# hongsukchoi/Pose2Mesh_RELEASE

Hardware: NVIDIA H100
Metric: SMPL meshes/sec (higher is better)
Workload: dtype f32 (wgmma fp16x3 split, fp32 accumulate)

## Files before the change

### include/p2m_b200.h

```cpp
#ifndef P2M_B200_H_
#define P2M_B200_H_

#include <stddef.h>
#include <stdint.h>

#ifdef __cplusplus
extern "C" {
#endif

typedef struct p2m_model p2m_model_t;
typedef void* p2m_stream_t;

enum p2m_status {
  P2M_OK = 0,
  P2M_ERR_INVALID = 1,
  P2M_ERR_CUDA = 2,
  P2M_ERR_WORKSPACE = 3,
  P2M_ERR_NOGPU = 4
};

enum p2m_precision {
  P2M_PREC_FP32_SIMT = 0,
  P2M_PREC_FP16X3_TC = 1
};

typedef struct {
  int32_t n_levels;
  const int32_t* level_size;
  const int32_t* const* rowptr;
  const int32_t* const* colidx;
  const float* const* values;
  int32_t n_blocks;
  const int32_t* block_len;
  const int32_t* block_chans;
  int32_t device;
} p2m_model_desc_t;

typedef struct {
  float* fc_w;
  float* fc_b;
  float* const* cl_w;
  float* const* cl_b;
  float* const* bn_w;
  float* const* bn_b;
  float* const* bn_rm;
  float* const* bn_rv;
  int64_t* const* bn_nbt;
} p2m_params_t;

int p2m_model_create(const p2m_model_desc_t* desc, p2m_model_t** out);
void p2m_model_destroy(p2m_model_t* m);
int p2m_model_num_layers(const p2m_model_t* m);
int p2m_model_layer_info(const p2m_model_t* m, int layer, int32_t out[6]);
int p2m_model_set_precision(p2m_model_t* m, int precision);
int p2m_model_set_profiling(p2m_model_t* m, int enable);
int p2m_model_layer_times_ms(p2m_model_t* m, float* out_ms, int n);
int p2m_debug_kernel_status(p2m_model_t* m, int32_t* out);
int p2m_debug_set_trace(p2m_model_t* m, void* dev_buf);
int p2m_debug_set_fuse_head(p2m_model_t* m, int enable);
int p2m_debug_set_elide_padding(p2m_model_t* m, int enable);
int p2m_debug_set_dedup_padding(p2m_model_t* m, int enable);
int p2m_debug_conv_path(const p2m_model_t* m, int level, int fin, int fout, int32_t out[9]);
int p2m_debug_conv_tiling(const p2m_model_t* m, int level, int fin, int fout, int32_t out[3]);
int p2m_debug_layer_route(const p2m_model_t* m, int layer, int batch, int need_dx, int32_t out[9]);

typedef struct {
  float* const* z;
  float* const* a;
  float* const* y;
  float* fc_out;
  float* const* g_a;
  float* const* g_z;
  float* const* dx;
  float* fc_dx;
} p2m_capture_t;
int p2m_debug_set_capture(p2m_model_t* m, const p2m_capture_t* capture);

#define P2M_BN_BATCH_UPDATE 0
#define P2M_BN_BATCH 1
#define P2M_BN_RUNNING 2
typedef struct {
  int32_t stats;
  int32_t cumulative;
  double momentum;
  double eps;
} p2m_bn_opts_t;

size_t p2m_meshnet_workspace_bytes(const p2m_model_t* m, int batch, int training);
size_t p2m_meshnet_backward_scratch_bytes(const p2m_model_t* m, int batch);

int p2m_meshnet_forward(p2m_model_t* m, const p2m_params_t* params, const float* x, float* y, int batch,
                        int training, void* workspace, size_t workspace_bytes, p2m_stream_t stream);

int p2m_model_set_output_gather(p2m_model_t* m, const int32_t* vertex_of_slot, int n_slots);
int p2m_meshnet_forward_vertices(p2m_model_t* m, const p2m_params_t* params, const float* x, float* y_vertices,
                                 int batch, void* workspace, size_t workspace_bytes, p2m_stream_t stream);

int p2m_meshnet_backward(p2m_model_t* m, const p2m_params_t* params, const p2m_params_t* grads, const float* x,
                         const float* dy, float* dx, int batch, void* workspace, size_t workspace_bytes,
                         void* scratch, size_t scratch_bytes, p2m_stream_t stream);

size_t p2m_meshnet_workspace_bytes_opts(const p2m_model_t* m, int batch, int training, const p2m_bn_opts_t* bn);
int p2m_meshnet_forward_opts(p2m_model_t* m, const p2m_params_t* params, const p2m_bn_opts_t* bn, const float* x,
                             float* y, int batch, int training, void* workspace, size_t workspace_bytes,
                             p2m_stream_t stream);
int p2m_meshnet_backward_opts(p2m_model_t* m, const p2m_params_t* params, const p2m_params_t* grads,
                              const p2m_bn_opts_t* bn, const float* x, const float* dy, float* dx, int batch,
                              void* workspace, size_t workspace_bytes, void* scratch, size_t scratch_bytes,
                              p2m_stream_t stream);

size_t p2m_meshnet_host_io_bytes(const p2m_model_t* m, int batch);
int p2m_meshnet_forward_host(p2m_model_t* m, const p2m_params_t* params, const float* x_host, float* y_host,
                             int batch, void* workspace, size_t workspace_bytes, p2m_stream_t stream);
int p2m_meshnet_forward_vertices_host(p2m_model_t* m, const p2m_params_t* params, const float* x_host,
                                      float* y_vertices_host, int batch, void* workspace, size_t workspace_bytes,
                                      p2m_stream_t stream);

typedef struct {
  int32_t level, batch, fin, fout;
  const float* x;
  const float* weight;
  const float* bias;
  int32_t bn_mode;
  const float* bn_weight;
  const float* bn_bias;
  float* bn_running_mean;
  float* bn_running_var;
  int64_t* bn_num_batches_tracked;
  float* save_mean;
  float* save_invstd;
  int32_t relu;
  float* y;
} p2m_conv_fwd_args_t;

size_t p2m_cheb_conv_workspace_bytes(const p2m_model_t* m, int level, int batch, int fin, int fout);
int p2m_cheb_conv_fwd(p2m_model_t* m, const p2m_conv_fwd_args_t* a, void* workspace, size_t workspace_bytes,
                      p2m_stream_t stream);

typedef struct {
  int32_t level, batch, fin, fout;
  const float* x;
  const float* weight;
  const float* dz;
  float* dx;
  float* dweight;
  float* dbias;
} p2m_conv_bwd_args_t;
int p2m_cheb_conv_bwd(p2m_model_t* m, const p2m_conv_bwd_args_t* a, void* workspace, size_t workspace_bytes,
                      p2m_stream_t stream);


typedef struct {
  const float* w1_w; const float* w1_b;
  const float* w2_w; const float* w2_b;
  const float* bn1_w; const float* bn1_b; const float* bn1_rm; const float* bn1_rv;
  const float* bn2_w; const float* bn2_b; const float* bn2_rm; const float* bn2_rv;
} p2m_posenet_stage_t;
typedef struct {
  int32_t num_joint, hidden, num_stage;
  const float* w1_w; const float* w1_b;
  const float* w2_w; const float* w2_b;
  const p2m_posenet_stage_t* stages;
} p2m_posenet_params_t;
size_t p2m_posenet_workspace_bytes(int batch, int hidden);
int p2m_posenet_forward(const p2m_posenet_params_t* params, const float* pose2d, float* pose3d, float* pose_combine,
                        int batch, void* workspace, size_t workspace_bytes, p2m_stream_t stream);

typedef struct {
  int64_t* bn1_nbt; int64_t* bn2_nbt;
} p2m_posenet_train_stage_t;
typedef struct {
  const p2m_posenet_train_stage_t* stages;
} p2m_posenet_train_t;
typedef struct {
  float* w1_w; float* w1_b; float* w2_w; float* w2_b;
  float* bn1_w; float* bn1_b; float* bn2_w; float* bn2_b;
} p2m_posenet_stage_grads_t;
typedef struct {
  float* w1_w; float* w1_b; float* w2_w; float* w2_b;
  const p2m_posenet_stage_grads_t* stages;
} p2m_posenet_grads_t;
size_t p2m_posenet_train_workspace_bytes(int batch, int num_joint, int hidden, int num_stage);
size_t p2m_posenet_train_saved_bytes(int batch, int num_joint, int hidden, int num_stage);
int p2m_posenet_train_forward(const p2m_posenet_params_t* params, const p2m_posenet_train_t* extra, const float* pose2d,
                              int batch, float p_dropout, const int64_t* seed, float* pose3d, float* pose_combine,
                              void* saved, size_t saved_bytes, void* workspace, size_t workspace_bytes,
                              p2m_stream_t stream);
int p2m_posenet_backward(const p2m_posenet_params_t* params, const float* pose2d, int batch, float p_dropout,
                         const int64_t* seed, const void* saved, size_t saved_bytes, const float* d_pose3d,
                         const p2m_posenet_grads_t* grads, float* d_pose2d, void* workspace, size_t workspace_bytes,
                         p2m_stream_t stream);

int p2m_posenet_forward_opts(const p2m_posenet_params_t* params, const p2m_bn_opts_t* bn, const float* pose2d,
                             float* pose3d, float* pose_combine, int batch, void* workspace, size_t workspace_bytes,
                             p2m_stream_t stream);
int p2m_posenet_train_forward_opts(const p2m_posenet_params_t* params, const p2m_posenet_train_t* extra,
                                   const p2m_bn_opts_t* bn, const float* p_dropout, const float* pose2d, int batch,
                                   const int64_t* seed, float* pose3d, float* pose_combine, void* saved,
                                   size_t saved_bytes, void* workspace, size_t workspace_bytes, p2m_stream_t stream);
int p2m_posenet_backward_opts(const p2m_posenet_params_t* params, const p2m_bn_opts_t* bn, const float* p_dropout,
                              const float* pose2d, int batch, const int64_t* seed, const void* saved,
                              size_t saved_bytes, const float* d_pose3d, const p2m_posenet_grads_t* grads,
                              float* d_pose2d, void* workspace, size_t workspace_bytes, p2m_stream_t stream);

typedef struct {
  float* const* g_y;
  float* const* a2;
  float* const* g_a2;
  float* const* g_z2;
  float* const* a1;
  float* const* g_a1;
  float* const* g_bn1;
  float* const* scale;
  float* g_y0;
} p2m_posenet_capture_t;
int p2m_debug_posenet_backward_capture(const p2m_posenet_params_t* params, const p2m_bn_opts_t* bn,
// ... 212 lines not shown
```

### pose2mesh_release_b200/_lib.py

```python
from __future__ import annotations

import ctypes as C
import os
import threading

import torch

_HERE = os.path.dirname(os.path.abspath(__file__))
LIB_PATH = os.path.join(_HERE, "libp2m_b200.so")

P2M_PREC_FP32_SIMT = 0
P2M_PREC_FP16X3_TC = 1
PRECISIONS = {"fp32": P2M_PREC_FP32_SIMT, "fp16x3": P2M_PREC_FP16X3_TC}


def default_precision() -> int:
    name = os.environ.get("P2M_PRECISION", "fp16x3").strip().lower()
    if name not in PRECISIONS:
        raise RuntimeError(f"P2M_PRECISION={name!r}: expected one of {sorted(PRECISIONS)}")
    return PRECISIONS[name]

c_float_p = C.POINTER(C.c_float)
c_int32_p = C.POINTER(C.c_int32)
c_int64_p = C.POINTER(C.c_int64)
# ... 14 lines not shown


class Params(C.Structure):
    _fields_ = [
        ("fc_w", C.c_void_p),
        ("fc_b", C.c_void_p),
        ("cl_w", C.POINTER(C.c_void_p)),
        ("cl_b", C.POINTER(C.c_void_p)),
        ("bn_w", C.POINTER(C.c_void_p)),
        ("bn_b", C.POINTER(C.c_void_p)),
        ("bn_rm", C.POINTER(C.c_void_p)),
        ("bn_rv", C.POINTER(C.c_void_p)),
        ("bn_nbt", C.POINTER(C.c_void_p)),
    ]


P2M_BN_BATCH_UPDATE = 0
P2M_BN_BATCH = 1
P2M_BN_RUNNING = 2


class BnOpts(C.Structure):
    _fields_ = [("stats", C.c_int32), ("cumulative", C.c_int32), ("momentum", C.c_double), ("eps", C.c_double)]


class ConvFwdArgs(C.Structure):
    _fields_ = [
        ("level", C.c_int32), ("batch", C.c_int32), ("fin", C.c_int32), ("fout", C.c_int32),
        ("x", C.c_void_p), ("weight", C.c_void_p), ("bias", C.c_void_p),
        ("bn_mode", C.c_int32),
        ("bn_weight", C.c_void_p), ("bn_bias", C.c_void_p),
        ("bn_running_mean", C.c_void_p), ("bn_running_var", C.c_void_p),
        ("bn_num_batches_tracked", C.c_void_p),
        ("save_mean", C.c_void_p), ("save_invstd", C.c_void_p),
        ("relu", C.c_int32),
        ("y", C.c_void_p),
    ]


class ConvBwdArgs(C.Structure):
    _fields_ = [
        ("level", C.c_int32), ("batch", C.c_int32), ("fin", C.c_int32), ("fout", C.c_int32),
        ("x", C.c_void_p), ("weight", C.c_void_p), ("dz", C.c_void_p),
        ("dx", C.c_void_p), ("dweight", C.c_void_p), ("dbias", C.c_void_p),
    ]


class Capture(C.Structure):
    _fields_ = [
        ("z", C.POINTER(C.c_void_p)), ("a", C.POINTER(C.c_void_p)), ("y", C.POINTER(C.c_void_p)),
        ("fc_out", C.c_void_p),
        ("g_a", C.POINTER(C.c_void_p)), ("g_z", C.POINTER(C.c_void_p)), ("dx", C.POINTER(C.c_void_p)),
        ("fc_dx", C.c_void_p),
    ]


class Pose2MeshLossArgs(C.Structure):
    _fields_ = [(n, C.c_int32) for n in ("batch", "n_padded", "n_vertex", "n_face", "n_reg_joint", "n_lift_joint")] + [
        (n, C.c_void_p) for n in ("cam_mesh", "lift_pose", "gt_mesh", "gt_reg3dpose", "gt_lift3dpose", "mesh_valid",
                                  "reg3dpose_valid", "lift3dpose_valid", "faces", "joint_regressor", "perm_reverse",
                                  "weights", "edge", "pred_pose", "scratch", "loss", "terms", "grad_loss",
                                  "d_cam_mesh", "d_lift_pose")]


P2M_POSE2MESH_MAX_REG_JOINT = 24


class PoseNetStage(C.Structure):
    _fields_ = [(n, C.c_void_p) for n in ("w1_w", "w1_b", "w2_w", "w2_b", "bn1_w", "bn1_b", "bn1_rm", "bn1_rv",
                                          "bn2_w", "bn2_b", "bn2_rm", "bn2_rv")]


class PoseNetParams(C.Structure):
    _fields_ = [("num_joint", C.c_int32), ("hidden", C.c_int32), ("num_stage", C.c_int32),
                ("w1_w", C.c_void_p), ("w1_b", C.c_void_p), ("w2_w", C.c_void_p), ("w2_b", C.c_void_p),
                ("stages", C.POINTER(PoseNetStage))]


class PoseNetTrainStage(C.Structure):
    _fields_ = [("bn1_nbt", C.c_void_p), ("bn2_nbt", C.c_void_p)]


class PoseNetTrain(C.Structure):
    _fields_ = [("stages", C.POINTER(PoseNetTrainStage))]


class PoseNetStageGrads(C.Structure):
    _fields_ = [(n, C.c_void_p) for n in ("w1_w", "w1_b", "w2_w", "w2_b", "bn1_w", "bn1_b", "bn2_w", "bn2_b")]


class PoseNetGrads(C.Structure):
    _fields_ = [("w1_w", C.c_void_p), ("w1_b", C.c_void_p), ("w2_w", C.c_void_p), ("w2_b", C.c_void_p),
                ("stages", C.POINTER(PoseNetStageGrads))]


class PoseNetCapture(C.Structure):
    _fields_ = [(n, C.POINTER(C.c_void_p)) for n in ("g_y", "a2", "g_a2", "g_z2", "a1", "g_a1", "g_bn1", "scale")] + [
        ("g_y0", C.c_void_p)]


class BodyModelDesc(C.Structure):
    _fields_ = [
        ("n_vertex", C.c_int32), ("n_joint", C.c_int32), ("n_betas", C.c_int32), ("n_out_joints", C.c_int32),
        ("v_template", c_float_p), ("shapedirs", c_float_p), ("posedirs", c_float_p), ("J_regressor", c_float_p),
        ("weights", c_float_p), ("parents", c_int32_p), ("model_betas", c_float_p), ("pose_mean", c_float_p),
        ("joint_map", c_int32_p), ("scale", C.c_float), ("device", C.c_int32),
    ]


P2M_BETAS_ZERO_MEANS_MODEL = 0
P2M_BETAS_AS_GIVEN = 1

P2M_FRAME_ROTATE_ROOT = 1
P2M_FRAME_CLAMP_BETAS = 2
P2M_FRAME_ZERO_BETAS_MODEL = 4
P2M_FRAME_LAYER_TRANS_T = 8
P2M_FRAME_LAYER_TRANS = 16
P2M_FRAME_H36M_COMPENSATE = 32
P2M_FRAME_ADD_T = 64
P2M_FRAME_TO_MM = 128

P2M_JOINTS_HUMAN36 = 0
P2M_JOINTS_COCO = 1
P2M_JOINTS_SMPL = 2
P2M_JOINTS_MANO = 3
P2M_DATASET_HUMAN36M = 0
P2M_DATASET_COCO = 1
P2M_DATASET_MUCO = 2
P2M_DATASET_AMASS = 3
P2M_DATASET_PW3D = 4
P2M_DATASET_SURREAL = 5
P2M_DATASET_FREIHAND = 6

P2M_CAM_INPUT_F64 = 0
P2M_CAM_INPUT_INT = 1
P2M_CAM_INPUT_F32 = 2

P2M_DTYPE_F32 = 0
P2M_DTYPE_F64 = 1

P2M_NOISE_NONE = 0
P2M_NOISE_COCO = 1
P2M_NOISE_H36M = 2
P2M_AREA_TIGHT = 0
P2M_AREA_CROP = 1


class H36MError(C.Structure):
    _fields_ = [("mean", C.c_double * 2), ("std", C.c_double * 2), ("weight", C.c_double)]


EXPORTS = [
    "p2m_model_create", "p2m_model_destroy", "p2m_model_num_layers", "p2m_model_layer_info",
    "p2m_model_set_precision", "p2m_debug_kernel_status", "p2m_debug_set_trace", "p2m_debug_set_fuse_head", "p2m_debug_set_elide_padding", "p2m_debug_set_dedup_padding", "p2m_debug_conv_path", "p2m_debug_conv_tiling", "p2m_debug_layer_route", "p2m_debug_set_capture", "p2m_model_set_profiling", "p2m_model_layer_times_ms", "p2m_meshnet_workspace_bytes", "p2m_meshnet_backward_scratch_bytes",
    "p2m_meshnet_forward", "p2m_meshnet_backward", "p2m_meshnet_workspace_bytes_opts", "p2m_meshnet_forward_opts",
    "p2m_meshnet_backward_opts", "p2m_model_set_output_gather", "p2m_meshnet_forward_vertices", "p2m_meshnet_host_io_bytes", "p2m_meshnet_forward_host", "p2m_meshnet_forward_vertices_host",
    "p2m_cheb_conv_workspace_bytes", "p2m_cheb_conv_fwd", "p2m_cheb_conv_bwd", "p2m_graph_match_level", "p2m_posenet_workspace_bytes", "p2m_posenet_forward",
    "p2m_posenet_train_workspace_bytes", "p2m_posenet_train_saved_bytes", "p2m_posenet_train_forward", "p2m_posenet_backward",
    "p2m_posenet_forward_opts", "p2m_posenet_train_forward_opts", "p2m_posenet_backward_opts",
    "p2m_debug_posenet_backward_capture",
    "p2m_regress_joints", "p2m_regress_joints_backward", "p2m_normalize_pose2d", "p2m_mesh_losses", "p2m_coord_loss",
    "p2m_pose2mesh_loss", "p2m_pose2mesh_loss_backward",
    "p2m_rigid_align", "p2m_point_errors", "p2m_fit_camera", "p2m_crop_cam_to_orig",
    "p2m_one_euro_smooth", "p2m_accel_error", "p2m_segment_mean",
    "p2m_nearest_distances", "p2m_align_w_scale", "p2m_pck_accumulate",
    "p2m_render_workspace_bytes", "p2m_render_meshes",
    "p2m_body_model_create", "p2m_body_model_destroy", "p2m_body_model_workspace_bytes", "p2m_body_model_forward",
    "p2m_body_model_backward_workspace_bytes", "p2m_body_model_backward",
    "p2m_camera_frame_workspace_bytes", "p2m_camera_frame_coords", "p2m_h36m_regressors_create",
    "p2m_h36m_regressors_destroy", "p2m_h36m_targets", "p2m_synthesize_pose", "p2m_h36m_syn_error",
    "p2m_training_pose2d", "p2m_augm_params", "p2m_training_pose2d_augmented", "p2m_sample_targets",
    "p2m_layer_joint_targets",
    "p2m_last_error", "p2m_version", "p2m_launch_count", "p2m_launch_count_reset",
]

_lib = None
_lock = threading.Lock()


def load() -> C.CDLL:
    global _lib
    if _lib is not None:
        return _lib
    with _lock:
        if _lib is not None:
            return _lib
        if not os.path.exists(LIB_PATH):
            raise RuntimeError(
                f"{LIB_PATH} not found: build it with `python -m pose2mesh_release_b200.build` "
                "(or __graft_entry__.build()).  pose2mesh_release_b200 has no CPU / eager fallback.")
        lib = C.CDLL(LIB_PATH)
        vp, i32, i64, sz = C.c_void_p, C.c_int32, C.c_int64, C.c_size_t
        lib.p2m_model_create.argtypes = [C.POINTER(ModelDesc), C.POINTER(vp)]
        lib.p2m_model_create.restype = C.c_int
        lib.p2m_model_destroy.argtypes = [vp]
        lib.p2m_model_destroy.restype = None
        lib.p2m_model_num_layers.argtypes = [vp]
        lib.p2m_model_num_layers.restype = C.c_int
        lib.p2m_model_layer_info.argtypes = [vp, C.c_int, c_int32_p]
        lib.p2m_model_layer_info.restype = C.c_int
        lib.p2m_model_set_precision.argtypes = [vp, C.c_int]
        lib.p2m_model_set_precision.restype = C.c_int
        lib.p2m_model_set_profiling.argtypes = [vp, C.c_int]
        lib.p2m_model_set_profiling.restype = C.c_int
        lib.p2m_model_layer_times_ms.argtypes = [vp, c_float_p, C.c_int]
        lib.p2m_model_layer_times_ms.restype = C.c_int
        lib.p2m_debug_set_fuse_head.argtypes = [vp, C.c_int]
        lib.p2m_debug_set_fuse_head.restype = C.c_int
        lib.p2m_debug_set_elide_padding.argtypes = [vp, C.c_int]
        lib.p2m_debug_set_elide_padding.restype = C.c_int
        lib.p2m_debug_set_dedup_padding.argtypes = [vp, C.c_int]
        lib.p2m_debug_set_dedup_padding.restype = C.c_int
        lib.p2m_debug_set_trace.argtypes = [vp, vp]
        lib.p2m_debug_set_trace.restype = C.c_int
        lib.p2m_debug_conv_path.argtypes = [vp, C.c_int, C.c_int, C.c_int, c_int32_p]
        lib.p2m_debug_conv_path.restype = C.c_int
        lib.p2m_debug_conv_tiling.argtypes = [vp, C.c_int, C.c_int, C.c_int, c_int32_p]
        lib.p2m_debug_conv_tiling.restype = C.c_int
        lib.p2m_debug_layer_route.argtypes = [vp, C.c_int, C.c_int, C.c_int, c_int32_p]
        lib.p2m_debug_layer_route.restype = C.c_int
        lib.p2m_debug_set_capture.argtypes = [vp, C.POINTER(Capture)]
        lib.p2m_debug_set_capture.restype = C.c_int
        lib.p2m_debug_kernel_status.argtypes = [vp, c_int32_p]
        lib.p2m_debug_kernel_status.restype = C.c_int
        lib.p2m_meshnet_workspace_bytes.argtypes = [vp, C.c_int, C.c_int]
        lib.p2m_meshnet_workspace_bytes.restype = sz
        lib.p2m_meshnet_backward_scratch_bytes.argtypes = [vp, C.c_int]
        lib.p2m_meshnet_backward_scratch_bytes.restype = sz
        lib.p2m_meshnet_host_io_bytes.argtypes = [vp, C.c_int]
        lib.p2m_meshnet_host_io_bytes.restype = sz
        lib.p2m_meshnet_forward.argtypes = [vp, C.POINTER(Params), vp, vp, C.c_int, C.c_int, vp, sz, vp]
        lib.p2m_meshnet_forward.restype = C.c_int
        lib.p2m_model_set_output_gather.argtypes = [vp, c_int32_p, C.c_int]
        lib.p2m_model_set_output_gather.restype = C.c_int
        lib.p2m_meshnet_forward_vertices.argtypes = [vp, C.POINTER(Params), vp, vp, C.c_int, vp, sz, vp]
        lib.p2m_meshnet_forward_vertices.restype = C.c_int
        lib.p2m_meshnet_forward_host.argtypes = [vp, C.POINTER(Params), vp, vp, C.c_int, vp, sz, vp]
        lib.p2m_meshnet_forward_host.restype = C.c_int
        lib.p2m_meshnet_forward_vertices_host.argtypes = [vp, C.POINTER(Params), vp, vp, C.c_int, vp, sz, vp]
        lib.p2m_meshnet_forward_vertices_host.restype = C.c_int
        lib.p2m_meshnet_backward.argtypes = [vp, C.POINTER(Params), C.POINTER(Params), vp, vp, vp, C.c_int, vp, sz,
                                             vp, sz, vp]
        lib.p2m_meshnet_backward.restype = C.c_int
        bn_p = C.POINTER(BnOpts)
        lib.p2m_meshnet_workspace_bytes_opts.argtypes = [vp, C.c_int, C.c_int, bn_p]
        lib.p2m_meshnet_workspace_bytes_opts.restype = sz
        lib.p2m_meshnet_forward_opts.argtypes = [vp, C.POINTER(Params), bn_p, vp, vp, C.c_int, C.c_int, vp, sz, vp]
        lib.p2m_meshnet_forward_opts.restype = C.c_int
        lib.p2m_meshnet_backward_opts.argtypes = [vp, C.POINTER(Params), C.POINTER(Params), bn_p, vp, vp, vp, C.c_int,
                                                  vp, sz, vp, sz, vp]
        lib.p2m_meshnet_backward_opts.restype = C.c_int
        lib.p2m_cheb_conv_workspace_bytes.argtypes = [vp, C.c_int, C.c_int, C.c_int, C.c_int]
        lib.p2m_cheb_conv_workspace_bytes.restype = sz
        lib.p2m_cheb_conv_fwd.argtypes = [vp, C.POINTER(ConvFwdArgs), vp, sz, vp]
        lib.p2m_cheb_conv_fwd.restype = C.c_int
        lib.p2m_cheb_conv_bwd.argtypes = [vp, C.POINTER(ConvBwdArgs), vp, sz, vp]
        lib.p2m_cheb_conv_bwd.restype = C.c_int
        lib.p2m_posenet_workspace_bytes.argtypes = [C.c_int, C.c_int]
        lib.p2m_posenet_workspace_bytes.restype = sz
        lib.p2m_posenet_forward.argtypes = [C.POINTER(PoseNetParams), vp, vp, vp, C.c_int, vp, sz, vp]
        lib.p2m_posenet_forward.restype = C.c_int
        for fn in (lib.p2m_posenet_train_workspace_bytes, lib.p2m_posenet_train_saved_bytes):
            fn.argtypes = [C.c_int] * 4
            fn.restype = sz
        lib.p2m_posenet_train_forward.argtypes = [C.POINTER(PoseNetParams), C.POINTER(PoseNetTrain), vp, C.c_int,
                                                  C.c_float, vp, vp, vp, vp, sz, vp, sz, vp]
        lib.p2m_posenet_train_forward.restype = C.c_int
        lib.p2m_posenet_backward.argtypes = [C.POINTER(PoseNetParams), vp, C.c_int, C.c_float, vp, vp, sz, vp,
                                             C.POINTER(PoseNetGrads), vp, vp, sz, vp]
        lib.p2m_posenet_backward.restype = C.c_int
        lib.p2m_posenet_forward_opts.argtypes = [C.POINTER(PoseNetParams), bn_p, vp, vp, vp, C.c_int, vp, sz, vp]
        lib.p2m_posenet_forward_opts.restype = C.c_int
        lib.p2m_posenet_train_forward_opts.argtypes = [C.POINTER(PoseNetParams), C.POINTER(PoseNetTrain), bn_p,
                                                       c_float_p, vp, C.c_int, vp, vp, vp, vp, sz, vp, sz, vp]
        lib.p2m_posenet_train_forward_opts.restype = C.c_int
        lib.p2m_posenet_backward_opts.argtypes = [C.POINTER(PoseNetParams), bn_p, c_float_p, vp, C.c_int, vp, vp, sz,
                                                  vp, C.POINTER(PoseNetGrads), vp, vp, sz, vp]
        lib.p2m_posenet_backward_opts.restype = C.c_int
        lib.p2m_debug_posenet_backward_capture.argtypes = (lib.p2m_posenet_backward_opts.argtypes[:-1]
                                                           + [C.POINTER(PoseNetCapture), vp])
        lib.p2m_debug_posenet_backward_capture.restype = C.c_int
        lib.p2m_regress_joints.argtypes = [vp, vp, vp, C.c_int, C.c_int, C.c_int, C.c_int, vp]
        lib.p2m_regress_joints.restype = C.c_int
        lib.p2m_regress_joints_backward.argtypes = [vp, vp, vp, C.c_int, C.c_int, C.c_int, C.c_int, vp]
        lib.p2m_regress_joints_backward.restype = C.c_int
        lib.p2m_normalize_pose2d.argtypes = [vp, vp, C.c_int, C.c_int, C.c_int, C.c_int, C.c_int, vp]
        lib.p2m_normalize_pose2d.restype = C.c_int
        lib.p2m_mesh_losses.argtypes = [vp, vp, vp, C.c_int, C.c_int, C.c_int, vp, vp, vp, vp]
        lib.p2m_mesh_losses.restype = C.c_int
        lib.p2m_coord_loss.argtypes = [vp, vp, vp, i64, vp, vp, vp, vp]
        lib.p2m_coord_loss.restype = C.c_int
        for fn in (lib.p2m_pose2mesh_loss, lib.p2m_pose2mesh_loss_backward):
            fn.argtypes = [C.POINTER(Pose2MeshLossArgs), vp]
            fn.restype = C.c_int
        lib.p2m_rigid_align.argtypes = [vp, vp, C.c_int, C.c_int, c_int32_p, C.c_int, vp, vp, vp, vp, vp]
        lib.p2m_rigid_align.restype = C.c_int
        lib.p2m_point_errors.argtypes = [vp, vp, vp, vp, C.c_int, C.c_int, c_int32_p, C.c_int, C.c_int, vp, vp, vp]
        lib.p2m_point_errors.restype = C.c_int
        lib.p2m_fit_camera.argtypes = [vp, C.c_int, C.c_int, C.c_int, vp, C.c_int, vp, C.c_int, C.c_int, C.c_int,
                                       c_int32_p, C.POINTER(C.c_double), C.c_int, vp, vp, vp, vp, vp, vp, vp]
        lib.p2m_fit_camera.restype = C.c_int
        lib.p2m_crop_cam_to_orig.argtypes = [vp, vp, vp, C.c_int, vp, vp]
        lib.p2m_crop_cam_to_orig.restype = C.c_int
        lib.p2m_one_euro_smooth.argtypes = [C.c_int, vp, vp, i64, c_int64_p, C.c_int, i64, C.c_double, C.c_double,
                                            C.c_double, vp]
        lib.p2m_one_euro_smooth.restype = C.c_int
        lib.p2m_accel_error.argtypes = [C.c_int, vp, vp, C.c_int, c_int64_p, C.c_int, i64, vp, vp, vp, vp, vp]
        lib.p2m_accel_error.restype = C.c_int
        lib.p2m_segment_mean.argtypes = [C.c_int, vp, i64, c_int64_p, C.c_int, i64, vp, vp, vp]
        lib.p2m_segment_mean.restype = C.c_int
        c_double_p = C.POINTER(C.c_double)
        lib.p2m_nearest_distances.argtypes = [C.c_int, vp, vp, C.c_int, C.c_int, C.c_int, c_double_p, C.c_int, vp, vp,
                                              vp, vp, vp, vp]
        lib.p2m_nearest_distances.restype = C.c_int
        lib.p2m_align_w_scale.argtypes = [vp, vp, C.c_int, C.c_int, C.c_int, vp, vp, vp]
        lib.p2m_align_w_scale.restype = C.c_int
        lib.p2m_pck_accumulate.argtypes = [vp, vp, vp, i64, c_double_p, C.c_int, vp, vp, vp]
        lib.p2m_pck_accumulate.restype = C.c_int
        lib.p2m_render_workspace_bytes.argtypes = [C.c_int, C.c_int, C.c_int]
        lib.p2m_render_workspace_bytes.restype = sz
        lib.p2m_render_meshes.argtypes = [vp, C.c_int, C.c_int, vp, C.c_int, vp, vp, vp, vp, C.c_int, C.c_int, C.c_int,
                                          vp, vp, vp, vp, vp, sz, vp]
        lib.p2m_render_meshes.restype = C.c_int
        lib.p2m_body_model_create.argtypes = [C.POINTER(BodyModelDesc), C.POINTER(vp)]
        lib.p2m_body_model_create.restype = C.c_int
        lib.p2m_body_model_destroy.argtypes = [vp]
        lib.p2m_body_model_destroy.restype = None
        lib.p2m_body_model_workspace_bytes.argtypes = [vp, C.c_int]
        lib.p2m_body_model_workspace_bytes.restype = sz
        lib.p2m_body_model_forward.argtypes = [vp, vp, vp, C.c_int, vp, C.c_int, vp, vp, C.c_int, vp, sz, vp]
        lib.p2m_body_model_forward.restype = C.c_int
        lib.p2m_body_model_backward_workspace_bytes.argtypes = [vp, C.c_int]
        lib.p2m_body_model_backward_workspace_bytes.restype = sz
        lib.p2m_body_model_backward.argtypes = [vp, vp, vp, C.c_int, vp, C.c_int, vp, vp, vp, vp, vp, C.c_int, vp, sz,
                                                vp]
        lib.p2m_body_model_backward.restype = C.c_int
        lib.p2m_camera_frame_workspace_bytes.argtypes = [vp, C.c_int]
        lib.p2m_camera_frame_workspace_bytes.restype = sz
        lib.p2m_camera_frame_coords.argtypes = [vp, C.c_int, vp, vp, vp, vp, vp, c_int32_p, C.c_int, vp, vp, C.c_int,
                                                vp, sz, vp]
        lib.p2m_camera_frame_coords.restype = C.c_int
        lib.p2m_h36m_regressors_create.argtypes = [C.POINTER(C.c_double), C.POINTER(C.c_double), C.c_int, C.c_int,
                                                   C.POINTER(vp)]
        lib.p2m_h36m_regressors_create.restype = C.c_int
        lib.p2m_h36m_regressors_destroy.argtypes = [vp]
        lib.p2m_h36m_regressors_destroy.restype = None
        lib.p2m_h36m_targets.argtypes = [vp, C.c_int, C.c_float, vp, vp, vp, vp, C.c_int, vp, vp, vp, vp, vp, vp, vp,
                                         vp, vp]
        lib.p2m_h36m_targets.restype = C.c_int
        lib.p2m_synthesize_pose.argtypes = [vp, vp, vp, C.c_int, vp, vp]
        lib.p2m_synthesize_pose.restype = C.c_int
        lib.p2m_h36m_syn_error.argtypes = [C.POINTER(H36MError), vp, C.c_int, vp, vp]
        lib.p2m_h36m_syn_error.restype = C.c_int
        lib.p2m_training_pose2d.argtypes = [vp, C.c_int, C.c_int, vp, C.c_int, C.c_int, C.c_int, C.POINTER(H36MError),
                                            vp, C.c_int, C.c_int, vp, vp]
        lib.p2m_training_pose2d.restype = C.c_int
        lib.p2m_augm_params.argtypes = [C.c_int, C.c_int, C.c_double, vp, vp, vp, vp]
        lib.p2m_augm_params.restype = C.c_int
        lib.p2m_training_pose2d_augmented.argtypes = [vp, C.c_int, C.c_int, vp, C.c_int, C.c_int, C.c_int,
                                                      C.POINTER(H36MError), vp, C.c_int, C.c_int, vp, vp, C.c_int,
                                                      C.c_int, vp, vp]
        lib.p2m_training_pose2d_augmented.restype = C.c_int
        lib.p2m_sample_targets.argtypes = [vp, C.c_int, C.c_int, C.c_float, vp, vp, vp, vp, vp, C.c_int, vp, vp, vp,
                                           vp, vp, C.c_int, vp, vp, vp, vp, vp, vp, vp, vp, vp, vp]
        lib.p2m_sample_targets.restype = C.c_int
        lib.p2m_layer_joint_targets.argtypes = [C.c_int, vp, vp, C.c_int, C.c_int, vp, vp, vp, vp, C.c_int, vp, vp,
                                                vp, vp, vp, vp, vp, vp, vp, vp]
        lib.p2m_layer_joint_targets.restype = C.c_int
        lib.p2m_graph_match_level.argtypes = [i64, c_int32_p, c_int32_p, C.POINTER(C.c_double), c_int64_p,
                                              C.POINTER(C.c_double), c_int32_p]
        lib.p2m_graph_match_level.restype = i32
# ... 50 lines not shown
```

### pose2mesh_release_b200/csrc/cheb_umma.cu

```cuda
#include <cuda.h>
#include <cuda_fp16.h>
#include <cuda_runtime.h>

#include <algorithm>
#include <climits>
#include <cstring>
#include <vector>

#include "p2m_internal.h"

namespace p2m {

namespace {

constexpr int TILE_M = 128;
constexpr int FC = 32;
constexpr int A_BLOCK_BYTES = TILE_M * 128;
constexpr float W_SCALE = 64.f;
constexpr float W_INV_SCALE = 1.f / 64.f;

struct TileHeader {
  int n_rows;
  int h1;
  int nnz;
// ... 176 lines not shown
  if (e < e1) {
    const uint2 a0 = lds_u2(ent + e * 8);
    fma4(acc0, __uint_as_float(a0.y), lds_f4(rows_q + a0.x));
  }
  return make_float4(acc0.x + acc1.x, acc0.y + acc1.y, acc0.z + acc1.z, acc0.w + acc1.w);
}

__device__ __forceinline__ void wg_fence() { asm volatile("wgmma.fence.sync.aligned;" ::: "memory"); }
__device__ __forceinline__ void wg_commit() { asm volatile("wgmma.commit_group.sync.aligned;" ::: "memory"); }
__device__ __forceinline__ void wg_wait0() { asm volatile("wgmma.wait_group.sync.aligned 0;" ::: "memory"); }
__device__ __forceinline__ void wgmma_m64n64(float (&d)[32], uint64_t desc_a, uint64_t desc_b) {
  asm volatile(
      "{\n\t.reg .pred p;\n\tsetp.ne.b32 p, 1, 0;\n\t"
      "wgmma.mma_async.sync.aligned.m64n64k16.f32.f16.f16 "
      "{%0, %1, %2, %3, %4, %5, %6, %7, %8, %9, %10, %11, %12, %13, %14, %15, "
      "%16, %17, %18, %19, %20, %21, %22, %23, %24, %25, %26, %27, %28, %29, %30, %31}, %32, %33, p, 1, 1, 0, 0;\n\t}"
      : "+f"(d[0]), "+f"(d[1]), "+f"(d[2]), "+f"(d[3]), "+f"(d[4]), "+f"(d[5]), "+f"(d[6]), "+f"(d[7]), "+f"(d[8]),
        "+f"(d[9]), "+f"(d[10]), "+f"(d[11]), "+f"(d[12]), "+f"(d[13]), "+f"(d[14]), "+f"(d[15]), "+f"(d[16]),
        "+f"(d[17]), "+f"(d[18]), "+f"(d[19]), "+f"(d[20]), "+f"(d[21]), "+f"(d[22]), "+f"(d[23]), "+f"(d[24]),
        "+f"(d[25]), "+f"(d[26]), "+f"(d[27]), "+f"(d[28]), "+f"(d[29]), "+f"(d[30]), "+f"(d[31])
      : "l"(desc_a), "l"(desc_b)
      : "memory");
}
__device__ __forceinline__ void wgmma_m64n128(float (&d)[2][32], uint64_t desc_a, uint64_t desc_b) {
  asm volatile(
      "{\n\t.reg .pred p;\n\tsetp.ne.b32 p, 1, 0;\n\t"
      "wgmma.mma_async.sync.aligned.m64n128k16.f32.f16.f16 "
      "{%0, %1, %2, %3, %4, %5, %6, %7, %8, %9, %10, %11, %12, %13, %14, %15, "
      "%16, %17, %18, %19, %20, %21, %22, %23, %24, %25, %26, %27, %28, %29, %30, %31, "
      "%32, %33, %34, %35, %36, %37, %38, %39, %40, %41, %42, %43, %44, %45, %46, %47, "
      "%48, %49, %50, %51, %52, %53, %54, %55, %56, %57, %58, %59, %60, %61, %62, %63}, %64, %65, p, 1, 1, 0, 0;\n\t}"
      : "+f"(d[0][0]), "+f"(d[0][1]), "+f"(d[0][2]), "+f"(d[0][3]), "+f"(d[0][4]), "+f"(d[0][5]), "+f"(d[0][6]),
        "+f"(d[0][7]), "+f"(d[0][8]), "+f"(d[0][9]), "+f"(d[0][10]), "+f"(d[0][11]), "+f"(d[0][12]), "+f"(d[0][13]),
        "+f"(d[0][14]), "+f"(d[0][15]), "+f"(d[0][16]), "+f"(d[0][17]), "+f"(d[0][18]), "+f"(d[0][19]), "+f"(d[0][20]),
        "+f"(d[0][21]), "+f"(d[0][22]), "+f"(d[0][23]), "+f"(d[0][24]), "+f"(d[0][25]), "+f"(d[0][26]), "+f"(d[0][27]),
        "+f"(d[0][28]), "+f"(d[0][29]), "+f"(d[0][30]), "+f"(d[0][31]), "+f"(d[1][0]), "+f"(d[1][1]), "+f"(d[1][2]),
        "+f"(d[1][3]), "+f"(d[1][4]), "+f"(d[1][5]), "+f"(d[1][6]), "+f"(d[1][7]), "+f"(d[1][8]), "+f"(d[1][9]),
        "+f"(d[1][10]), "+f"(d[1][11]), "+f"(d[1][12]), "+f"(d[1][13]), "+f"(d[1][14]), "+f"(d[1][15]), "+f"(d[1][16]),
        "+f"(d[1][17]), "+f"(d[1][18]), "+f"(d[1][19]), "+f"(d[1][20]), "+f"(d[1][21]), "+f"(d[1][22]), "+f"(d[1][23]),
        "+f"(d[1][24]), "+f"(d[1][25]), "+f"(d[1][26]), "+f"(d[1][27]), "+f"(d[1][28]), "+f"(d[1][29]), "+f"(d[1][30]),
        "+f"(d[1][31])
      : "l"(desc_a), "l"(desc_b)
      : "memory");
}
__device__ __forceinline__ void wgmma_m64n32(float (&d)[16], uint64_t desc_a, uint64_t desc_b) {
  asm volatile(
      "{\n\t.reg .pred p;\n\tsetp.ne.b32 p, 1, 0;\n\t"
      "wgmma.mma_async.sync.aligned.m64n32k16.f32.f16.f16 "
      "{%0, %1, %2, %3, %4, %5, %6, %7, %8, %9, %10, %11, %12, %13, %14, %15}, %16, %17, p, 1, 1, 1, 1;\n\t}"
      : "+f"(d[0]), "+f"(d[1]), "+f"(d[2]), "+f"(d[3]), "+f"(d[4]), "+f"(d[5]), "+f"(d[6]), "+f"(d[7]), "+f"(d[8]),
        "+f"(d[9]), "+f"(d[10]), "+f"(d[11]), "+f"(d[12]), "+f"(d[13]), "+f"(d[14]), "+f"(d[15])
      : "l"(desc_a), "l"(desc_b)
      : "memory");
}

__device__ __forceinline__ uint64_t make_desc_sw128(uint32_t saddr) {
  uint64_t d = 0;
  d |= (uint64_t)((saddr & 0x3FFFF) >> 4);
  d |= (uint64_t)1 << 16;
  d |= (uint64_t)(1024 >> 4) << 32;
  d |= (uint64_t)1 << 62;
  return d;
}

__host__ __device__ __forceinline__ uint32_t sw128_off(int row, int chunk) {
  return (uint32_t)row * 128u + (uint32_t)((chunk ^ (row & 7)) << 4);
}

struct Half4 {
  __half2 a, b;
};
__device__ __forceinline__ void split4(const float4& v, uint2& hi, uint2& lo) {
  __half2 h0 = __floats2half2_rn(v.x, v.y), h1 = __floats2half2_rn(v.z, v.w);
  float2 f0 = __half22float2(h0), f1 = __half22float2(h1);
  __half2 l0 = __floats2half2_rn(v.x - f0.x, v.y - f0.y), l1 = __floats2half2_rn(v.z - f1.x, v.w - f1.y);
  hi.x = *reinterpret_cast<uint32_t*>(&h0);
  hi.y = *reinterpret_cast<uint32_t*>(&h1);
  lo.x = *reinterpret_cast<uint32_t*>(&l0);
  lo.y = *reinterpret_cast<uint32_t*>(&l1);
}

struct KParams {
  const float* x;
  int in_unpool;
  int V, P, fin;
  int n_tiles;
  const unsigned char* meta;
  const int* meta_bytes;
  int meta_stride, max_h1;
  const unsigned char* wpack;
  const float* zero_row;
  EpiDev ep;
  int res_identity;
  const float* t1;
  const float* a_scale;
  const float* b_scale;
  long long ldy;
  int y_col0;
  float* y;
  int* status;
  long long* trace;
  int own_table;
  const float* head_wt;
  float* head_z;
  const unsigned char* apack;
  long long wslice_bytes;
  long long wblock_stride;
  int tma;
  CUtensorMap tm_x, tm_t1;
};

#ifdef P2M_UMMA_TRACE
__device__ __forceinline__ void trace_ev(const KParams& p, int role, int& n, int ev) {
  if (p.trace != nullptr && blockIdx.x == 0 && blockIdx.y == 0 && n < 512) {
    p.trace[role * 512 + n] = ((long long)ev << 48) | (clock64() & 0xFFFFFFFFFFFFll);
    ++n;
  }
}
#else
__device__ __forceinline__ void trace_ev(const KParams&, int, int&, int) {}
#endif

constexpr int W_PROD = 16;
constexpr int W_XLOAD = 16, N_XLOAD = 2, W_BLOAD = 18, W_EPI0 = 20;
constexpr int NUM_THREADS2 = 24 * 32;
constexpr int REGS_LAUNCH = 80, REGS_UTIL = 40, REGS_EPI = 120;
static_assert(128 * (REGS_EPI - REGS_LAUNCH) <= 128 * (REGS_LAUNCH - REGS_UTIL), "register pool balance");
static_assert(W_XLOAD % 4 == 0 && W_EPI0 % 4 == 0 && W_EPI0 - W_XLOAD == 4, "setmaxnreg works on aligned warpgroups");
constexpr int W_PROD_W = 8, W_EPI1_W = 8, W_XLOAD_W = 12, W_BLOAD_W = 14, W_EPI0_W = 16;
constexpr int NUM_THREADS_W = 20 * 32;
constexpr int REGS_LAUNCH_W = 96, REGS_UTIL_W = 40, REGS_PROD_W = 88, REGS_EPI_W = 128;
static_assert(2 * 128 * (REGS_EPI_W - REGS_LAUNCH_W) <=
                  128 * (REGS_LAUNCH_W - REGS_UTIL_W) + 2 * 128 * (REGS_LAUNCH_W - REGS_PROD_W),
              "register pool balance of the 64 x 128 layout");
static_assert(REGS_LAUNCH_W * NUM_THREADS_W <= 65536 && (REGS_LAUNCH_W + 8) * NUM_THREADS_W > 65536,
              "__launch_bounds__(NUM_THREADS_W, 1) gives REGS_LAUNCH_W registers per thread");
static_assert(W_EPI1_W == W_PROD_W && W_EPI1_W % 4 == 0 && W_XLOAD_W == W_EPI1_W + 4 && W_EPI0_W == W_XLOAD_W + 4 &&
                  (W_EPI0_W + 4) * 32 == NUM_THREADS_W,
              "setmaxnreg works on aligned warpgroups");
template <int N>
struct ConvRoles {
  static constexpr int threads = NUM_THREADS2, prod = W_PROD, xload = W_XLOAD, bload = W_BLOAD, epi0 = W_EPI0,
                       epi1 = -1;
  static constexpr int regs_launch = REGS_LAUNCH, regs_util = REGS_UTIL, regs_prod = REGS_LAUNCH, regs_epi = REGS_EPI;
};
template <>
struct ConvRoles<128> {
  static constexpr int threads = NUM_THREADS_W, prod = W_PROD_W, xload = W_XLOAD_W, bload = W_BLOAD_W,
                       epi0 = W_EPI0_W, epi1 = W_EPI1_W;
  static constexpr int regs_launch = REGS_LAUNCH_W, regs_util = REGS_UTIL_W, regs_prod = REGS_PROD_W,
                       regs_epi = REGS_EPI_W;
};

template <int N>
__host__ __device__ constexpr int tile_rows() { return N == 128 ? 64 : TILE_M; }


struct ConvSmem {
  size_t xs, xs_stage, t1s, t1_stage, meta, bars, flags, ep, stage, own, tail, bytes;
};
__host__ __device__ __forceinline__ ConvSmem conv_smem(int NC, int NS, int XS, int MODE, int max_h1, int meta_stride) {
  const int N = NC == 64 ? 64 : 128;
  const int tm = N == 128 ? 64 : TILE_M;
  size_t at = 0, sum = 0;
  auto take = [&](size_t bytes) { sum += bytes; at += bytes; return at - bytes; };
  ConvSmem L;
  take((size_t)NS * (tm + NC) * 128);
  L.xs_stage = (MODE == 1 && tm == 64) ? 0 : (size_t)tm * FC;
  L.xs = take(XS * L.xs_stage * 4);
  L.t1_stage = MODE == 1 ? (size_t)max_h1 * FC : 0;
  L.t1s = take(XS * L.t1_stage * 4);
  L.meta = take(2 * (size_t)meta_stride);
  L.bars = take(8 * (2 * NS + 2 * XS + 6));
  L.flags = take(16);
  L.ep = take(2 * 4 * NC);
  at = (at + 127) & ~(size_t)127;
  L.stage = take(4 * stg_warp_bytes(N));
  L.own = take(4 * 32 * 4);
  L.tail = take(N == 64 ? 64 * 12 * 4 : 4 * 8);
  L.bytes = sum + 128 + 1024 + 32;
  return L;
}

template <int N, int NC, int NS, int XS, int MODE>
__device__ __forceinline__ void cheb_conv_body(const KParams& p) {
  static_assert(N == 64 || N == 128, "one warpgroup holds the CTA's 128 x 64 or 64 x 128 accumulator in registers");
  static_assert(NC == N || (N == 128 && NC == 2 * N && MODE == 1),
                "64 x 256: both MMA warpgroups of the 64 x 128 layout, T1-given convs only (conv_cols)");
  static_assert(NS == 3 || NS == 6, "the producers fill a chunk's three slots back to back");
  using R = ConvRoles<N>;
  constexpr int TM = tile_rows<N>();
  constexpr int NPW = R::prod;
  constexpr int NRG = NPW * 4;
  constexpr int RPT = TM / NRG;
  constexpr int NWG = N == 128 ? 2 : 1;
  constexpr bool COLS = NC != N;
  static_assert(RPT == 2, "both configurations give a producer thread two tile rows");
  constexpr int H = TM / 64;
  constexpr int ER = 16 * H;
  constexpr bool KT1 = (MODE == 1);
  constexpr bool plain = !KT1;
  constexpr int A_BYTES = TM * 128;
  constexpr int B_BLOCK_BYTES = NC * 128;
  constexpr int SLOT_BYTES = A_BYTES + B_BLOCK_BYTES;
  static_assert(NWG * ER == 32 && SLOT_BYTES == (TM + NC) * 128, "conv_smem describes this configuration");

  extern __shared__ __align__(1024) unsigned char smem_raw[];
  const ConvSmem L = conv_smem(NC, NS, XS, MODE, p.max_h1, p.meta_stride);
  unsigned char* ring = smem_raw;
  float* Xs = reinterpret_cast<float*>(smem_raw + L.xs);
  float* T1s = reinterpret_cast<float*>(smem_raw + L.t1s);
  unsigned char* meta_s = smem_raw + L.meta;
  uint64_t* bars = reinterpret_cast<uint64_t*>(smem_raw + L.bars);
  uint64_t* b_ab_full = bars;
  uint64_t* b_ab_empty = b_ab_full + NS;
  uint64_t* b_x_full = b_ab_empty + NS;
  uint64_t* b_x_empty = b_x_full + XS;
  uint64_t* b_m_full = b_x_empty + XS;
  uint64_t* b_m_empty = b_m_full + 2;
  uint64_t* b_stg_free = b_m_empty + 2;
  uint64_t* b_turn = b_stg_free + 1;
  uint32_t* flags = reinterpret_cast<uint32_t*>(smem_raw + L.flags);
  volatile int* abort_flag = reinterpret_cast<volatile int*>(flags + 1);
  float* ep_mul = reinterpret_cast<float*>(smem_raw + L.ep);
  float* ep_add = ep_mul + NC;
  constexpr int EC = 32;
  constexpr int STG_WARP_BYTES = stg_warp_bytes(N);
  unsigned char* epi_stage = smem_raw + L.stage;
  int* own_s = reinterpret_cast<int*>(smem_raw + L.own);
  float* head_w_s = reinterpret_cast<float*>(smem_raw + L.tail);
  uint64_t* b_res = reinterpret_cast<uint64_t*>(head_w_s);

  const int tid = threadIdx.x;
  const int warp = tid >> 5;
  const int lane = tid & 31;
  const int n_chunk = p.fin / FC;
  const int n_use = 3 * n_chunk;

  if (tid == 0) {
    for (int s = 0; s < NS; ++s) {
      mbar_init(smem_u32(b_ab_full + s), p.apack != nullptr ? 1 : NPW + 1);
      mbar_init(smem_u32(b_ab_empty + s), COLS ? 8 : 4);
    }
    for (int s = 0; s < XS; ++s) {
      mbar_init(smem_u32(b_x_full + s), N_XLOAD * 32 + 1);
      mbar_init(smem_u32(b_x_empty + s), 1);
    }
    for (int s = 0; s < 2; ++s) {
      mbar_init(smem_u32(b_m_full + s), 1);
      mbar_init(smem_u32(b_m_empty + s), 1);
    }
    if (N == 128) {
      for (int w = 0; w < 4; ++w) mbar_init(smem_u32(b_res + w), 1);
      mbar_init(smem_u32(b_stg_free), 4);
      mbar_init(smem_u32(b_turn), 4);
    }
    *abort_flag = (smem_u32(ring) & 1023u) ? 1 : 0;
    if (*abort_flag) mbar_timeout(abort_flag, p.status, 100);
    fence_barrier_init();
  }
  const float a_scale = p.a_scale ? *p.a_scale : 1.f;
  const float b_inv = p.b_scale ? 1.f / *p.b_scale : W_INV_SCALE;
  const int ccol0 = (int)blockIdx.y * NC;
  for (int n = threadIdx.x; n < NC; n += R::threads) {
    const float sc = (p.ep.scale ? p.ep.scale[ccol0 + n] : 1.f) / a_scale;
    const float sh = p.ep.scale ? p.ep.shift[ccol0 + n] : 0.f;
    const float bi = p.ep.bias ? p.ep.bias[ccol0 + n] : 0.f;
    ep_mul[n] = b_inv * sc;
    ep_add[n] = fmaf(bi, p.ep.scale ? p.ep.scale[ccol0 + n] : 1.f, sh);
  }
  if (N == 64 && p.head_z != nullptr)
    for (int i = threadIdx.x; i < 64 * 12; i += R::threads) head_w_s[i] = p.head_wt[i];
  __syncthreads();

  const int mma_g = warp >= R::epi0 ? 0 : (NWG == 2 && warp >= R::epi1 && warp < R::epi1 + 4) ? 1 : -1;
  if (warp >= R::xload && warp < R::epi0) {
  asm volatile("setmaxnreg.dec.sync.aligned.u32 %0;" ::"n"(R::regs_util));
  if (warp >= R::xload && warp < R::xload + N_XLOAD) {
    if (p.apack == nullptr) {
      const int lt = tid - R::xload * 32;
      const int lq = lt & 7, lrg = lt >> 3;
      const int my_tiles = (p.n_tiles - (int)blockIdx.x + (int)gridDim.x - 1) / (int)gridDim.x;
      if (lt == 32 && p.tma) {
        if (plain) asm volatile("prefetch.tensormap [%0];" ::"l"(reinterpret_cast<uint64_t>(&p.tm_x)) : "memory");
        if (KT1) asm volatile("prefetch.tensormap [%0];" ::"l"(reinterpret_cast<uint64_t>(&p.tm_t1)) : "memory");
      }
      auto fetch_meta = [&](int itf) {
        const int pat = (blockIdx.x + itf * gridDim.x) % p.P;
        const int m = itf & 1;
        mbar_wait_relaxed(smem_u32(b_m_empty + m), ((itf >> 1) & 1) ^ 1, abort_flag, p.status, 1);
        const int mbytes = p.meta_bytes[pat];
        mbar_arrive_expect_tx(smem_u32(b_m_full + m), mbytes);
        bulk_g2s(smem_u32(meta_s + (size_t)m * p.meta_stride), p.meta + (size_t)pat * p.meta_stride, mbytes,
                 smem_u32(b_m_full + m));
      };
      if (lt == 0 && my_tiles > 0) fetch_meta(0);
      const uint32_t fin_bytes = (uint32_t)p.fin * 4u;
      const int sh = p.in_unpool ? 1 : 0;
      int g2 = 0;
      int ltn = 0;
      for (int it2 = 0; it2 < my_tiles; ++it2) {
        const int tile2 = blockIdx.x + it2 * gridDim.x;
        const long long mesh_row0 = (long long)(tile2 / p.P) * p.V;
        const int m2 = it2 & 1;
        mbar_wait_relaxed(smem_u32(b_m_full + m2), (it2 >> 1) & 1, abort_flag, p.status, 8);
        const unsigned char* mb2 = meta_s + (size_t)m2 * p.meta_stride;
        const TileHeader* hdr2 = reinterpret_cast<const TileHeader*>(mb2);
        const int* halo = reinterpret_cast<const int*>(mb2 + hdr2->off_halo);
        const int h1 = hdr2->h1;
        for (int c2 = 0; c2 < n_chunk; ++c2, ++g2) {
          const int xs2 = g2 % XS;
          mbar_wait_relaxed(smem_u32(b_x_empty + xs2), ((g2 / XS) & 1) ^ 1, abort_flag, p.status, 11);
          if (lt == 0) trace_ev(p, 4, ltn, 1);
          const uint32_t xbar = smem_u32(b_x_full + xs2);
          auto stage_rows = [&](uint32_t dbase, const char* sbase, int first, int n_rows, int shift) {
            for (int i0 = first + lrg; i0 < n_rows; i0 += 32) {
              int v[4];
#pragma unroll
              for (int u = 0; u < 4; ++u) v[u] = (i0 + 8 * u < n_rows) ? halo[i0 + 8 * u] : -2;
#pragma unroll
              for (int u = 0; u < 4; ++u) {
                if (v[u] != -2) {
                  const uint32_t srow = (uint32_t)max(v[u], 0) >> shift;
                  cp_async16_zfill(dbase + (i0 + 8 * u) * 128, sbase + (uint64_t)srow * (uint64_t)fin_bytes,
                                   v[u] >= 0 ? 16u : 0u);
                }
              }
            }
          };
          const char* t1_mesh =
              reinterpret_cast<const char*>(KT1 ? p.t1 + mesh_row0 * p.fin + c2 * FC + lq * 4 : nullptr);
          const char* x_mesh = reinterpret_cast<const char*>(p.x + (mesh_row0 >> sh) * p.fin + c2 * FC + lq * 4);
          const uint32_t t1_dst = smem_u32(T1s + xs2 * L.t1_stage) + lq * 16;
          const uint32_t x_dst = smem_u32(Xs + xs2 * L.xs_stage) + lq * 16;
          if (p.tma) {
            if (lt == 32) {
              const int own0 = tile2 * TM;
              mbar_arrive_expect_tx(xbar, KT1 ? TM * 128 : (p.in_unpool ? TM / 2 : TM) * 128);
              if (plain)
                tma_load_2d(smem_u32(Xs + xs2 * L.xs_stage), &p.tm_x, c2 * FC, p.in_unpool ? own0 >> 1 : own0, xbar);
              if (KT1) tma_load_2d(smem_u32(T1s + xs2 * L.t1_stage), &p.tm_t1, c2 * FC, own0, xbar);
            }
            if (KT1) stage_rows(t1_dst, t1_mesh, TM, h1, 0);
          } else {
            if (KT1) stage_rows(t1_dst, t1_mesh, 0, h1, 0);
            if (plain) stage_rows(x_dst, x_mesh, 0, TM, sh);
            if (lt == 32) mbar_arrive(xbar);
          }
          cp_async_arrive_noinc(xbar);
          if (lt == 0) trace_ev(p, 4, ltn, 2);
          if (lt == 0 && c2 == (n_chunk > 1 ? 1 : 0) && it2 + 1 < my_tiles) fetch_meta(it2 + 1);
        }
      }
    }
  } else if (warp == R::bload) {
    if (lane == 0) {
      uint32_t ucnt = 0;
      int tn = 0;
      const int uses = plain ? n_chunk : n_use;
      for (int tile = blockIdx.x; tile < p.n_tiles; tile += gridDim.x) {
        for (int u = 0; u < uses; ++u, ++ucnt) {
          const int s = ucnt % NS;
          const uint32_t par = (ucnt / NS) & 1;
          mbar_wait_relaxed(smem_u32(b_ab_empty + s), par ^ 1, abort_flag, p.status, 4);
          trace_ev(p, 1, tn, 10 + u);
          const unsigned char* wsl = p.wpack + (size_t)blockIdx.y * (size_t)p.wslice_bytes;
          if (p.apack != nullptr) {
            mbar_arrive_expect_tx(smem_u32(b_ab_full + s), B_BLOCK_BYTES + A_BYTES);
            bulk_g2s(smem_u32(ring + s * SLOT_BYTES), p.apack + ((size_t)tile * uses + u) * A_BYTES, A_BYTES,
                     smem_u32(b_ab_full + s));
          } else {
            mbar_arrive_expect_tx(smem_u32(b_ab_full + s), B_BLOCK_BYTES);
          }
          bulk_g2s(smem_u32(ring + s * SLOT_BYTES + A_BYTES), wsl + (size_t)u * (size_t)p.wblock_stride, B_BLOCK_BYTES,
                   smem_u32(b_ab_full + s));
        }
      }
    }
  }
  } else if (mma_g >= 0) {
    asm volatile("setmaxnreg.inc.sync.aligned.u32 %0;" ::"n"(R::regs_epi));
    const int g = mma_g;
    const int ecol0 = ccol0 + (COLS ? g * N : 0);
    const float* ep_mul_g = ep_mul + (COLS ? g * N : 0);
    const float* ep_add_g = ep_add + (COLS ? g * N : 0);
    const int wq = warp - (g == 0 ? R::epi0 : R::epi1);
    const int tr = 3 + 2 * g;
    constexpr int CPR = EC / 4;
    constexpr int RPI = 32 / CPR;
    const uint32_t stg = smem_u32(epi_stage) + (uint32_t)wq * STG_WARP_BYTES;
    const int prow = lane / CPR, pc = lane % CPR;
    constexpr int NP = ER / RPI;
    int colk[2];
#pragma unroll
    for (int k = 0; k < 2; ++k) colk[k] = (int)(((uint32_t)pc ^ (uint32_t)((k * RPI + prow) & 7)) << 2);
    const int trow = (lane >> 4) * 64 + wq * 16 + (lane & 15);
    const int uses = plain ? n_chunk : n_use;
    int etn = 0;
    for (int it = COLS ? 0 : g; (int)blockIdx.x + it * (int)gridDim.x < p.n_tiles; it += COLS ? 1 : NWG) {
      const int e = COLS ? 2 * it + g : it;
      const int tile = blockIdx.x + it * gridDim.x;
      const int b = tile / p.P, pat = tile - b * p.P;
      const long long mesh0 = (long long)b * p.V;
      int* own_w = own_s + (g * 4 + wq) * ER;
      {
        int v;
        if (lane >= ER) {
          v = -1;
        } else if (p.own_table) {
          v = __ldg(reinterpret_cast<const int*>(p.meta + (size_t)pat * p.meta_stride + 64) + trow);
        } else {
          v = pat * TM + trow;
          if (v >= p.V) v = -1;
        }
        __syncwarp();
        if (lane < ER) own_w[lane] = v;
        __syncwarp();
      }
      int own_v[NP];
#pragma unroll
      for (int i = 0; i < NP; ++i) own_v[i] = own_w[i * RPI + prow];
      if (p.ep.res != nullptr) {
        const bool own_cols = p.apack != nullptr || (N == 128 && p.res_identity);
        const int lpr = ((own_cols ? N : p.ep.res_F) * 4 + 127) >> 7;
        for (int j = lane; j < ER * lpr; j += 32) {
          const int rr = j / lpr, ln = j - rr * lpr;
          const int vtx = own_w[rr];
          if (vtx >= 0) {
            const long long r = mesh0 + vtx;
            prefetch_l2(p.ep.res + (p.ep.res_unpool ? (r >> 1) : r) * p.ep.res_F + (own_cols ? ecol0 : 0) + ln * 32);
          }
        }
      }
      float acc[2][32];
#pragma unroll
      for (int h = 0; h < 2; ++h)
#pragma unroll
        for (int j = 0; j < 32; ++j) acc[h][j] = 0.f;
      if (wq == 0 && lane == 0) trace_ev(p, tr, etn, 1);
      if (NWG == 2 && !COLS && it > 0) {
        mbar_wait(smem_u32(b_turn), (uint32_t)(it - 1) & 1u, abort_flag, p.status, 13);
        if (wq == 0 && lane == 0) trace_ev(p, tr, etn, 3);
      }
      uint32_t ucnt = (uint32_t)it * (uint32_t)uses;
      for (int u = 0; u < uses; ++u, ++ucnt) {
        const uint32_t s = ucnt % NS;
        if (wq == 0 && lane == 0) trace_ev(p, tr, etn, 4);
        mbar_wait(smem_u32(b_ab_full + s), (ucnt / NS) & 1, abort_flag, p.status, 6);
        if (wq == 0 && lane == 0) trace_ev(p, tr, etn, 5);
        const uint32_t a0 = smem_u32(ring + s * SLOT_BYTES);
        wg_fence();
        if constexpr (N == 128) {
          const uint64_t da = make_desc_sw128(a0);
          const uint64_t db = make_desc_sw128(a0 + A_BYTES + (COLS ? (uint32_t)g * (N * 128) : 0u));
          wgmma_m64n128(acc, da + 0, db + 0);
          wgmma_m64n128(acc, da + 2, db + 2);
          wgmma_m64n128(acc, da + 4, db + 0);
          wgmma_m64n128(acc, da + 6, db + 2);
          wgmma_m64n128(acc, da + 0, db + 4);
          wgmma_m64n128(acc, da + 2, db + 6);
        } else {
#pragma unroll
          for (int h = 0; h < 2; ++h) {
            const uint64_t da = make_desc_sw128(a0 + (uint32_t)h * (64 * 128));
            const uint64_t db = make_desc_sw128(a0 + A_BYTES);
            wgmma_m64n64(acc[h], da + 0, db + 0);
            wgmma_m64n64(acc[h], da + 2, db + 2);
            wgmma_m64n64(acc[h], da + 4, db + 0);
            wgmma_m64n64(acc[h], da + 6, db + 2);
            wgmma_m64n64(acc[h], da + 0, db + 4);
            wgmma_m64n64(acc[h], da + 2, db + 6);
          }
        }
        wg_commit();
        wg_wait0();
        __syncwarp();
        if (lane == 0) mbar_arrive(smem_u32(b_ab_empty + s));
      }
      if (NWG == 2 && !COLS && lane == 0) mbar_arrive(smem_u32(b_turn));
      if (wq == 0 && lane == 0) trace_ev(p, tr, etn, 2);
      auto stage_slab = [&](int cb) {
#pragma unroll
        for (int h = 0; h < H; ++h)
#pragma unroll
          for (int jj = 0; jj < 4; ++jj)
#pragma unroll
            for (int r = 0; r < 2; ++r) {
              const int lr = 16 * h + (lane >> 2) + 8 * r;
              const int cc = 8 * jj + 2 * (lane & 3);
              const int j = 4 * (cb / 8 + jj) + 2 * r;
              sts_f2(stg + lr * (EC * 4) + ((((uint32_t)(cc >> 2)) ^ (uint32_t)(lr & 7)) << 4) + (cc & 3) * 4,
                     acc[h][j], acc[h][j + 1]);
            }
        __syncwarp();
      };
      if (N == 64 && p.head_z != nullptr) {
        float z[12];
#pragma unroll
        for (int j = 0; j < 12; ++j) z[j] = 0.f;
#pragma unroll
        for (int cb = 0; cb < N; cb += 32) {
          stage_slab(cb);
#pragma unroll
          for (int c = 0; c < 8; ++c) {
            const float4 a = lds_f4(stg + lane * (EC * 4) + (((uint32_t)c ^ (uint32_t)(lane & 7)) << 4));
            const float av[4] = {a.x, a.y, a.z, a.w};
#pragma unroll
            for (int e = 0; e < 4; ++e) {
              const int n = cb + 4 * c + e;
              float t = fmaf(av[e], ep_mul[n], ep_add[n]);
              if (p.ep.relu) t = fmaxf(t, 0.f);
              const float4 w0 = *reinterpret_cast<const float4*>(head_w_s + n * 12);
              const float4 w1 = *reinterpret_cast<const float4*>(head_w_s + n * 12 + 4);
              const float4 w2 = *reinterpret_cast<const float4*>(head_w_s + n * 12 + 8);
              z[0] = fmaf(t, w0.x, z[0]); z[1] = fmaf(t, w0.y, z[1]); z[2] = fmaf(t, w0.z, z[2]); z[3] = fmaf(t, w0.w, z[3]);
              z[4] = fmaf(t, w1.x, z[4]); z[5] = fmaf(t, w1.y, z[5]); z[6] = fmaf(t, w1.z, z[6]); z[7] = fmaf(t, w1.w, z[7]);
              z[8] = fmaf(t, w2.x, z[8]); z[9] = fmaf(t, w2.y, z[9]); z[10] = fmaf(t, w2.z, z[10]); z[11] = fmaf(t, w2.w, z[11]);
            }
          }
          __syncwarp();
        }
        if (own_w[lane] >= 0) {
          float4* zr = reinterpret_cast<float4*>(p.head_z + (mesh0 + own_w[lane]) * 12);
          zr[0] = make_float4(z[0], z[1], z[2], z[3]);
          zr[1] = make_float4(z[4], z[5], z[6], z[7]);
          zr[2] = make_float4(z[8], z[9], z[10], z[11]);
        }
      } else if (N == 128) {
        if (e > 0) mbar_wait(smem_u32(b_stg_free), (uint32_t)(e - 1) & 1u, abort_flag, p.status, 14);
        if (wq == 0 && lane == 0) trace_ev(p, tr, etn, 20);
        const bool res_id = p.ep.res != nullptr && p.res_identity;
        if (res_id) {
          const uint32_t rbar = smem_u32(b_res + wq);
          const int n_valid = __popc(__ballot_sync(0xFFFFFFFFu, lane < ER && own_w[lane] >= 0));
          if (lane == 0) mbar_arrive_expect_tx(rbar, (uint32_t)n_valid * (N * 4));
          __syncwarp();
          if (lane < ER && own_w[lane] >= 0) {
            const long long r = mesh0 + own_w[lane];
            bulk_g2s(stg + lane * STG_ROW_BYTES, p.ep.res + (p.ep.res_unpool ? (r >> 1) : r) * p.ep.res_F + ecol0, N * 4,
                     rbar);
          }
          mbar_wait(rbar, (uint32_t)e & 1u, abort_flag, p.status, 12);
        }
        if (wq == 0 && lane == 0) trace_ev(p, tr, etn, 21);
#pragma unroll
        for (int h = 0; h < 2; ++h)
#pragma unroll
          for (int jg = 0; jg < 8; ++jg) {
            const int n = 64 * h + 8 * jg + 2 * (lane & 3);
            const float2 mu = *reinterpret_cast<const float2*>(ep_mul_g + n);
            const float2 ad = *reinterpret_cast<const float2*>(ep_add_g + n);
#pragma unroll
            for (int r = 0; r < 2; ++r) {
              const int j = 4 * jg + 2 * r;
              const uint32_t a = stg + ((lane >> 2) + 8 * r) * STG_ROW_BYTES + n * 4;
              float o0 = fmaf(acc[h][j], mu.x, ad.x), o1 = fmaf(acc[h][j + 1], mu.y, ad.y);
              if (p.ep.relu) {
                o0 = fmaxf(o0, 0.f);
                o1 = fmaxf(o1, 0.f);
              }
              if (res_id) {
                const float2 rv = lds_f2(a);
                o0 += rv.x;
                o1 += rv.y;
              }
              sts_f2(a, o0, o1);
            }
          }
        if (p.ep.res != nullptr && !p.res_identity) {
          __syncwarp();
          const int gn = ecol0 + 4 * lane;
          for (int rr = 0; rr < ER; ++rr) {
            const int vtx = own_w[rr];
            if (vtx >= 0) {
              const long long r = mesh0 + vtx;
              const float* res_row = p.ep.res + (p.ep.res_unpool ? (r >> 1) : r) * p.ep.res_F;
              const uint32_t a = stg + rr * STG_ROW_BYTES + lane * 16;
              const float4 v = lds_f4(a);
              float o[4] = {v.x, v.y, v.z, v.w};
#pragma unroll
              for (int e = 0; e < 4; ++e) {
                const float l = __ldg(p.ep.lam + gn + e);
                o[e] += (1.f - l) * __ldg(res_row + __ldg(p.ep.i0 + gn + e)) + l * __ldg(res_row + __ldg(p.ep.i1 + gn + e));
              }
              sts_f4(a, make_float4(o[0], o[1], o[2], o[3]));
            }
          }
        }
        if (wq == 0 && lane == 0) trace_ev(p, tr, etn, 22);
        fence_async_proxy();
        __syncwarp();
        if (lane < ER) {
          if (own_w[lane] >= 0)
            bulk_s2g(p.y + (mesh0 + own_w[lane]) * p.ldy + p.y_col0 + ecol0, stg + lane * STG_ROW_BYTES, N * 4);
          bulk_commit();
        }
        if (wq == 0 && lane == 0) trace_ev(p, tr, etn, 23);
        if (lane < ER) bulk_wait_read0();
        __syncwarp();
        if (lane == 0) mbar_arrive(smem_u32(b_stg_free));
        if (wq == 0 && lane == 0) trace_ev(p, tr, etn, 24);
      } else {
#pragma unroll
        for (int cb = 0; cb < N; cb += 32) {
          stage_slab(cb);
          float4 mu_k[2], ad_k[2];
#pragma unroll
          for (int k = 0; k < 2; ++k) {
            mu_k[k] = *reinterpret_cast<const float4*>(ep_mul + cb + colk[k]);
            ad_k[k] = *reinterpret_cast<const float4*>(ep_add + cb + colk[k]);
          }
#pragma unroll
          for (int i = 0; i < NP; ++i) {
            const int rr = i * RPI + prow;
            const int n = cb + colk[i & 1];
            const int gn = ecol0 + n;
            const float4 a = lds_f4(stg + rr * (EC * 4) + (pc << 4));
            const int vtx = own_v[i];
            if (vtx >= 0) {
              const float4 mu = mu_k[i & 1], ad = ad_k[i & 1];
              float o[4] = {fmaf(a.x, mu.x, ad.x), fmaf(a.y, mu.y, ad.y), fmaf(a.z, mu.z, ad.z), fmaf(a.w, mu.w, ad.w)};
              if (p.ep.relu) {
#pragma unroll
                for (int e = 0; e < 4; ++e) o[e] = fmaxf(o[e], 0.f);
              }
              const long long r = mesh0 + vtx;
              if (p.ep.res != nullptr) {
                const float* res_row = p.ep.res + (p.ep.res_unpool ? (r >> 1) : r) * p.ep.res_F;
                if (p.res_identity) {
                  const float4 rv = __ldg(reinterpret_cast<const float4*>(res_row + gn));
                  o[0] += rv.x; o[1] += rv.y; o[2] += rv.z; o[3] += rv.w;
                } else {
#pragma unroll
                  for (int e = 0; e < 4; ++e) {
                    const float l = __ldg(p.ep.lam + gn + e);
                    o[e] += (1.f - l) * __ldg(res_row + __ldg(p.ep.i0 + gn + e)) + l * __ldg(res_row + __ldg(p.ep.i1 + gn + e));
                  }
                }
              }
              *reinterpret_cast<float4*>(p.y + r * p.ldy + p.y_col0 + gn) = make_float4(o[0], o[1], o[2], o[3]);
            }
          }
          __syncwarp();
        }
      }
    }
    if (N == 128 && lane < ER) bulk_wait0();
  } else {
    if (R::regs_prod < R::regs_launch) asm volatile("setmaxnreg.dec.sync.aligned.u32 %0;" ::"n"(R::regs_prod));
    if (p.apack == nullptr) {
    const int q = tid & 7;
    const int rg = tid >> 3;
    const uint32_t t1s_a = smem_u32(T1s);
    const uint32_t ring_a = smem_u32(ring);
    const int my_tiles = (p.n_tiles - (int)blockIdx.x + (int)gridDim.x - 1) / (int)gridDim.x;
    const int n_stage = my_tiles * n_chunk;

    uint32_t row[RPT], re[RPT], ent_a = 0;
    int ptn = 0;
    uint32_t slot = 0, spar = 0;
    uint32_t so_f[RPT], so_s[RPT];
#pragma unroll
    for (int ps = 0; ps < RPT; ++ps) row[ps] = re[ps] = so_f[ps] = so_s[ps] = 0;
    const bool odd = (rg & 1) != 0;
    auto next_slot = [&]() {
      if (++slot == (uint32_t)NS) {
        slot = 0;
        spar ^= 1u;
      }
    };

    const int xsh = (p.tma && p.in_unpool) ? 1 : 0;
    const float* xp[RPT];
#pragma unroll
    for (int ps = 0; ps < RPT; ++ps) xp[ps] = nullptr;
    int it = 0, c = -1;
    for (int g = 0; g < n_stage; ++g) {
      if (++c == n_chunk) {
        c = 0;
        ++it;
      }
      const int m = it & 1;
      const int xs = g % XS;
      float4 xd[RPT];
#pragma unroll
      for (int ps = 0; ps < RPT; ++ps) {
        xd[ps] = make_float4(0.f, 0.f, 0.f, 0.f);
        if (KT1 && c != 0 && xp[ps]) xd[ps] = __ldg(reinterpret_cast<const float4*>(xp[ps] + c * FC));
      }
      if (tid == 0) trace_ev(p, 0, ptn, 1);
      mbar_wait(smem_u32(b_x_full + xs), (g / XS) & 1, abort_flag, p.status, 9);
      if (tid == 0) trace_ev(p, 0, ptn, 2);

      if (c == 0) {
        mbar_wait(smem_u32(b_m_full + m), (it >> 1) & 1, abort_flag, p.status, 8);
        const unsigned char* mb = meta_s + (size_t)m * p.meta_stride;
        const TileHeader* hdr = reinterpret_cast<const TileHeader*>(mb);
        const uint32_t mb_a = smem_u32(mb);
        const uint32_t rp_a = mb_a + hdr->off_rp, ord2_a = mb_a + hdr->off_ord2;
        ent_a = mb_a + hdr->off_ent;
#pragma unroll
        for (int ps = 0; ps < RPT; ++ps) {
          row[ps] = plain ? (uint32_t)(NRG * ps + rg) : lds_u16(ord2_a + 2 * (NRG * ps + rg));
          re[ps] = plain ? 0u : (lds_u16(rp_a + 2 * row[ps]) | (lds_u16(rp_a + 2 * row[ps] + 2) << 16));
          const uint32_t i = row[ps];
          const uint32_t a_hi = sw128_off(i, q >> 1) + (q & 1) * 8, a_lo = sw128_off(i, 4 + (q >> 1)) + (q & 1) * 8;
          so_f[ps] = odd ? a_lo : a_hi;
          so_s[ps] = odd ? a_hi : a_lo;
        }
        if (KT1) {
          const int* halo = reinterpret_cast<const int*>(mb + hdr->off_halo);
          const int sh = p.in_unpool ? 1 : 0;
          const long long mesh_row0 = (long long)((blockIdx.x + (unsigned)it * gridDim.x) / (unsigned)p.P) * p.V;
          const float* xm = p.x + (mesh_row0 >> sh) * p.fin + q * 4;
#pragma unroll
          for (int ps = 0; ps < RPT; ++ps) {
            const int v = halo[row[ps]];
            xp[ps] = (v >= 0) ? xm + (size_t)((uint32_t)v >> sh) * (uint32_t)p.fin : nullptr;
            if (xp[ps]) xd[ps] = __ldg(reinterpret_cast<const float4*>(xp[ps]));
          }
        }
      }
      const uint32_t xs_q = smem_u32(Xs + xs * L.xs_stage) + q * 16;
      const uint32_t t1s_q = t1s_a + (uint32_t)(xs * L.t1_stage * 4) + q * 16;
      if (plain) {
        const uint32_t s = slot;
        mbar_wait(smem_u32(b_ab_empty + s), spar ^ 1u, abort_flag, p.status, 10);
        const uint32_t ablk = ring_a + s * SLOT_BYTES;
#pragma unroll
        for (int ps = 0; ps < RPT; ++ps) {
          const uint32_t i = ps * NRG + rg;
          float4 v = lds_f4(xs_q + (i >> xsh) * 128);
          v.x *= a_scale; v.y *= a_scale; v.z *= a_scale; v.w *= a_scale;
          uint2 hi, lo;
          split4(v, hi, lo);
          sts_u2(ablk + so_f[ps], odd ? lo : hi);
          sts_u2(ablk + so_s[ps], odd ? hi : lo);
        }
        fence_async_proxy();
        __syncwarp();
        if ((tid & 31) == 0) mbar_arrive(smem_u32(b_ab_full + s));
        next_slot();
        producer_barrier<NPW * 32>();
        if (tid == 0) mbar_arrive(smem_u32(b_x_empty + xs));
        if (tid == 0 && c == n_chunk - 1) mbar_arrive(smem_u32(b_m_empty + m));
        continue;
      }
      const uint32_t slot0 = slot;
      auto emit = [&](const float4 (&vv)[RPT]) {
        const uint32_t ablk = ring_a + slot * SLOT_BYTES;
#pragma unroll
        for (int ps = 0; ps < RPT; ++ps) {
          uint2 hi, lo;
          float4 v = vv[ps];
          if (p.a_scale != nullptr) {
            v.x *= a_scale; v.y *= a_scale; v.z *= a_scale; v.w *= a_scale;
          }
          split4(v, hi, lo);
          sts_u2(ablk + so_f[ps], odd ? lo : hi);
          sts_u2(ablk + so_s[ps], odd ? hi : lo);
        }
        next_slot();
      };
      float4 t1v[RPT], t2[RPT];
#pragma unroll
      for (int ps = 0; ps < RPT; ++ps) t2[ps] = gather_row4(ent_a, re[ps] & 0xFFFFu, re[ps] >> 16, t1s_q);
#pragma unroll
      for (int ps = 0; ps < RPT; ++ps) t1v[ps] = lds_f4(t1s_q + row[ps] * 128);
      if (tid == 0) trace_ev(p, 0, ptn, 6);
      {
        uint32_t s2 = slot + 2, p2 = spar;
        if (s2 >= (uint32_t)NS) {
          s2 -= (uint32_t)NS;
          p2 ^= 1u;
        }
        mbar_wait(smem_u32(b_ab_empty + s2), p2 ^ 1u, abort_flag, p.status, 10);
      }
      emit(xd);
      emit(t1v);
#pragma unroll
      for (int ps = 0; ps < RPT; ++ps) t2[ps] = cheb_t2(t2[ps], xd[ps]);
      emit(t2);
      fence_async_proxy();
      __syncwarp();
      if ((tid & 31) == 0) {
#pragma unroll
        for (int k = 0; k < 3; ++k) mbar_arrive(smem_u32(b_ab_full + (slot0 + k) % NS));
      }
      if (tid == 0) trace_ev(p, 0, ptn, 7);
      producer_barrier<NPW * 32>();
      if (tid == 0) trace_ev(p, 0, ptn, 8);
      if (tid == 0) mbar_arrive(smem_u32(b_x_empty + xs));
      if (tid == 0 && c == n_chunk - 1) mbar_arrive(smem_u32(b_m_empty + m));
    }
    }
  }
}

template <int N, int NS, int XS, int MODE>
__global__ void __launch_bounds__(NUM_THREADS2, 1) k_cheb_conv_umma(const __grid_constant__ KParams p) {
  static_assert(N == 64, "the 64 x 128 configuration is k_cheb_conv_wide");
  cheb_conv_body<N, N, NS, XS, MODE>(p);
}
template <int NC, int NS, int XS, int MODE>
__global__ void __launch_bounds__(NUM_THREADS_W, 1) k_cheb_conv_wide(const __grid_constant__ KParams p) {
  cheb_conv_body<128, NC, NS, XS, MODE>(p);
}

struct DwParams {
  const float* x;
  int in_unpool;
  int V, P, fin;
  int n_tiles;
  const unsigned char* meta;
  const int* meta_bytes;
  int meta_stride, max_h1;
  const float* g;
  int fout_total, m_off, m_cols;
  int chunk0;
  const float* a_scale;
  float* dw;
  int* status;
  const float* t1;
  int g_unpool;
  int swap;
  int tma;
  CUtensorMap tm_x, tm_t1;
};

__device__ __forceinline__ uint64_t make_desc_sw128_mn(uint32_t saddr, uint32_t lbo_bytes) {
  uint64_t d = 0;
  d |= (uint64_t)((saddr & 0x3FFFF) >> 4);
  d |= (uint64_t)((lbo_bytes >> 4) & 0x3FFF) << 16;
  d |= (uint64_t)(1024 >> 4) << 32;
  d |= (uint64_t)1 << 62;
  return d;
}

constexpr int DW_NS = 3;
constexpr int DW_G_BYTES = 4 * A_BLOCK_BYTES;

struct DwSmem {
  size_t gblk, xs, t1s, t1_stage, meta, bars, flags, bytes;
};
__host__ __device__ __forceinline__ DwSmem dw_smem(int XS, int max_h1, int meta_stride) {
  size_t at = 0;
  auto take = [&](size_t bytes) { at += bytes; return at - bytes; };
  DwSmem L;
  take(DW_NS * A_BLOCK_BYTES);
  L.gblk = take(DW_G_BYTES);
  L.xs = take(XS * (size_t)TILE_M * FC * 4);
  L.t1_stage = (size_t)max_h1 * FC;
  L.t1s = take(XS * L.t1_stage * 4);
  L.meta = take(2 * (size_t)meta_stride);
  L.bars = take(8 * (2 * DW_NS + 2 * XS + 6));
  L.flags = take(16);
  L.bytes = at + 1024 + 32;
  return L;
}

template <int XS>
__global__ void __launch_bounds__(NUM_THREADS2, 1) k_cheb_dw_umma(const __grid_constant__ DwParams p) {
  extern __shared__ __align__(1024) unsigned char smem_raw[];
  const DwSmem L = dw_smem(XS, p.max_h1, p.meta_stride);
  unsigned char* ring = smem_raw;
  unsigned char* gblk = smem_raw + L.gblk;
  float* Xs = reinterpret_cast<float*>(smem_raw + L.xs);
  constexpr size_t xs_stage_floats = (size_t)TILE_M * FC;
  float* T1s = reinterpret_cast<float*>(smem_raw + L.t1s);
  const size_t t1_stage_floats = L.t1_stage;
  unsigned char* meta_s = smem_raw + L.meta;
  uint64_t* bars = reinterpret_cast<uint64_t*>(smem_raw + L.bars);
  uint64_t* b_t_full = bars;
  uint64_t* b_t_empty = b_t_full + DW_NS;
  uint64_t* b_x_full = b_t_empty + DW_NS;
  uint64_t* b_x_empty = b_x_full + XS;
  uint64_t* b_m_full = b_x_empty + XS;
  uint64_t* b_m_empty = b_m_full + 2;
  uint64_t* b_g_full = b_m_empty + 2;
  uint64_t* b_g_empty = b_g_full + 1;
  uint32_t* flags = reinterpret_cast<uint32_t*>(smem_raw + L.flags);
  volatile int* abort_flag = reinterpret_cast<volatile int*>(flags + 1);

  const int tid = threadIdx.x, warp = tid >> 5, lane = tid & 31;
  constexpr int n_chunk = 1;
  const int my_tiles = (p.n_tiles - (int)blockIdx.x + (int)gridDim.x - 1) / (int)gridDim.x;

  if (tid == 0) {
    for (int s = 0; s < DW_NS; ++s) {
      mbar_init(smem_u32(b_t_full + s), W_PROD);
      mbar_init(smem_u32(b_t_empty + s), 4);
    }
    for (int s = 0; s < XS; ++s) {
      mbar_init(smem_u32(b_x_full + s), N_XLOAD * 32 + 1);
      mbar_init(smem_u32(b_x_empty + s), 1);
    }
    for (int s = 0; s < 2; ++s) {
      mbar_init(smem_u32(b_m_full + s), 1);
      mbar_init(smem_u32(b_m_empty + s), 1);
    }
    mbar_init(smem_u32(b_g_full), W_PROD);
    mbar_init(smem_u32(b_g_empty), 4);
    *abort_flag = (smem_u32(ring) & 1023u) ? 1 : 0;
    if (*abort_flag) mbar_timeout(abort_flag, p.status, 100);
    fence_barrier_init();
  }
  const float a_scale = p.a_scale ? *p.a_scale : 1.f;
  __syncthreads();

  if (warp >= W_XLOAD && warp < W_XLOAD + N_XLOAD) {
    const int lt = tid - W_XLOAD * 32;
    const int q = lt & 7, rg = lt >> 3;
    auto fetch_meta = [&](int it2) {
      const int pat = (blockIdx.x + it2 * gridDim.x) % p.P;
      const int m2 = it2 & 1;
      mbar_wait_relaxed(smem_u32(b_m_empty + m2), ((it2 >> 1) & 1) ^ 1, abort_flag, p.status, 21);
      const int mbytes = p.meta_bytes[pat];
      mbar_arrive_expect_tx(smem_u32(b_m_full + m2), mbytes);
      bulk_g2s(smem_u32(meta_s + (size_t)m2 * p.meta_stride), p.meta + (size_t)pat * p.meta_stride, mbytes,
               smem_u32(b_m_full + m2));
    };
    if (lt == 0 && my_tiles > 0) fetch_meta(0);
    uint32_t g = 0;
    for (int it = 0; it < my_tiles; ++it) {
      const int tile = blockIdx.x + it * gridDim.x;
      const int b = tile / p.P;
      const int m = it & 1;
      mbar_wait_relaxed(smem_u32(b_m_full + m), (it >> 1) & 1, abort_flag, p.status, 22);
      const unsigned char* mb = meta_s + (size_t)m * p.meta_stride;
      const TileHeader* hdr = reinterpret_cast<const TileHeader*>(mb);
      const int h1 = hdr->h1;
      const int* halo = reinterpret_cast<const int*>(mb + hdr->off_halo);
      const long long mesh_row0 = (long long)b * p.V;
      if (it + 1 < my_tiles) {
        const int tile2 = blockIdx.x + (it + 1) * gridDim.x;
        const long long r2 = (long long)(tile2 / p.P) * p.V + (long long)(tile2 % p.P) * TILE_M;
        const int lpr = (p.m_cols * 4 + 127) >> 7;
        for (int j = lt; j < TILE_M * lpr; j += N_XLOAD * 32) {
          const long long rr = r2 + j / lpr;
          if (rr < (long long)(tile2 / p.P + 1) * p.V)
            prefetch_l2(p.g + (p.g_unpool ? (rr >> 1) : rr) * p.fout_total + p.m_off + (j % lpr) * 32);
        }
      }
      for (int c = 0; c < n_chunk; ++c, ++g) {
        const int xs = g % XS;
        mbar_wait_relaxed(smem_u32(b_x_empty + xs), ((g / XS) & 1) ^ 1, abort_flag, p.status, 23);
        const uint32_t dst0 = smem_u32(Xs + xs * xs_stage_floats) + q * 16;
        const float* src0 = p.x + (p.chunk0 + c) * FC + q * 4;
        const uint32_t xbar = smem_u32(b_x_full + xs);
        if (lt == 0) {
          if (p.tma) {
            const int own0 = tile * TILE_M;
            mbar_arrive_expect_tx(xbar, 2 * TILE_M * 128);
            tma_load_2d(smem_u32(Xs + xs * xs_stage_floats), &p.tm_x, (p.chunk0 + c) * FC, own0, xbar);
            tma_load_2d(smem_u32(T1s + xs * t1_stage_floats), &p.tm_t1, (p.chunk0 + c) * FC, own0, xbar);
          } else {
            mbar_arrive(xbar);
          }
        }
// ... 177 lines not shown
        fence_async_proxy();
        __syncwarp();
        if ((tid & 31) == 0) {
#pragma unroll
          for (int k = 0; k < 3; ++k) mbar_arrive(smem_u32(b_t_full + (u0 + k) % DW_NS));
        }
        producer_barrier<W_PROD * 32>();
        if (tid == 0) {
          mbar_arrive(smem_u32(b_x_empty + xs));
          if (c == n_chunk - 1) mbar_arrive(smem_u32(b_m_empty + m));
        }
      }
    }
  }
}

struct T1Params {
  const float* x;
  int in_unpool;
  int V, P, fin;
  const unsigned char* meta;
  const int* meta_bytes;
  int meta_stride, max_h1;
  float* t1;
};

struct T1Smem {
  size_t xs, stage, bytes;
};
__host__ __device__ __forceinline__ T1Smem t1_smem(int T1_STAGES, int max_h1, int meta_stride) {
  const size_t stage = (size_t)max_h1 * FC;
  return {(size_t)meta_stride, stage, meta_stride + T1_STAGES * stage * 4 + 16};
}

template <int T1_STAGES>
__global__ void __launch_bounds__(512, 2) k_cheb_t1(const T1Params p) {
  extern __shared__ __align__(16) unsigned char smem_t1[];
  const T1Smem L = t1_smem(T1_STAGES, p.max_h1, p.meta_stride);
  unsigned char* meta_s = smem_t1;
  float* Xs = reinterpret_cast<float*>(smem_t1 + L.xs);
  const size_t stage_floats = L.stage;
  const int tid = threadIdx.x, q = tid & 7, rg = tid >> 3;
  const int tile = blockIdx.x;
  const int b = tile / p.P, pat = tile - b * p.P;
  const long long mesh_row0 = (long long)b * p.V;
  {
    const uint4* src = reinterpret_cast<const uint4*>(p.meta + (size_t)pat * p.meta_stride);
    uint4* dst = reinterpret_cast<uint4*>(meta_s);
    const int n16 = p.meta_bytes[pat] >> 4;
    for (int i = tid; i < n16; i += 512) dst[i] = src[i];
  }
  __syncthreads();
  const TileHeader* hdr = reinterpret_cast<const TileHeader*>(meta_s);
  const int h1 = hdr->h1;
  const int* halo = reinterpret_cast<const int*>(meta_s + hdr->off_halo);
  const uint32_t mb_a = smem_u32(meta_s);
  const uint32_t rp_a = mb_a + hdr->off_rp, ent_a = mb_a + hdr->off_ent, ord2_a = mb_a + hdr->off_ord2;
  const int n_chunk = p.fin / FC;
  long long srow[4];
#pragma unroll
  for (int u = 0; u < 4; ++u) {
    const int i = rg + 64 * u;
    const int v = (i < h1) ? halo[i] : -2;
    long long r = mesh_row0 + v;
    if (p.in_unpool) r >>= 1;
    srow[u] = (v >= 0) ? r * p.fin : (long long)v;
  }
  auto stage = [&](int c) {
    if (c < n_chunk) {
      const uint32_t dst0 = smem_u32(Xs + (c % T1_STAGES) * stage_floats) + q * 16;
      const float* src0 = p.x + c * FC + q * 4;
#pragma unroll
      for (int u = 0; u < 4; ++u) {
        const int i = rg + 64 * u;
        if (srow[u] >= 0)
          cp_async16(dst0 + i * 128, src0 + srow[u]);
        else if (srow[u] == -1)
          sts_f4(dst0 + i * 128, make_float4(0.f, 0.f, 0.f, 0.f));
      }
    }
    asm volatile("cp.async.commit_group;" ::: "memory");
  };
  int vtx[2];
  uint32_t re[2];
#pragma unroll
  for (int ps = 0; ps < 2; ++ps) {
    const int i = lds_u16(ord2_a + 2 * (ps * 64 + rg));
    vtx[ps] = halo[i];
    re[ps] = lds_u16(rp_a + 2 * i) | (lds_u16(rp_a + 2 * i + 2) << 16);
  }
#pragma unroll
  for (int c = 0; c < T1_STAGES - 1; ++c) stage(c);
  for (int c = 0; c < n_chunk; ++c) {
    asm volatile("cp.async.wait_group %0;" ::"n"(T1_STAGES - 2) : "memory");
    __syncthreads();
    stage(c + T1_STAGES - 1);
    const uint32_t xs_q = smem_u32(Xs + (c % T1_STAGES) * stage_floats) + q * 16;
#pragma unroll
    for (int ps = 0; ps < 2; ++ps) {
      if (vtx[ps] >= 0) {
        const float4 acc = gather_row4(ent_a, re[ps] & 0xFFFFu, re[ps] >> 16, xs_q);
        *reinterpret_cast<float4*>(p.t1 + (mesh_row0 + vtx[ps]) * p.fin + c * FC + q * 4) = acc;
      }
    }
  }
}

struct PackSrc {
  const float* p;
  long long ld_row, ld_k;
  int rows, n_chunk, orders, n_real;
  float scale;
  int combined;
  float c;
  int k_real = INT_MAX;
  const float* dscale = nullptr;
};
__global__ void __launch_bounds__(256) k_pack(const PackSrc s, long long total, unsigned char* __restrict__ out) {
  const long long idx = (long long)blockIdx.x * blockDim.x + threadIdx.x;
  if (idx >= total) return;
  const int j = (int)(idx & 7);
  const int row = (int)((idx >> 3) % s.rows);
  const long long blk = (idx >> 3) / s.rows;
  const int per_tile = s.n_chunk * s.orders;
  const long long n = blk / per_tile * s.rows + row;
  const int u = (int)(blk % per_tile);
  const int k0 = (u / s.orders) * FC + (j & 3) * 8;
  const float* src = s.p + n * s.ld_row + (long long)k0 * s.ld_k + u % s.orders;
  const float c = s.c, c2 = 2.f * c * c - 1.f;
  const float scale = s.dscale ? s.scale * *s.dscale : s.scale;
  __align__(16) __half h[8];
#pragma unroll
  for (int e = 0; e < 8; ++e) {
    const float* wr = src + e * s.ld_k;
    float w = 0.f;
    if (n < s.n_real && k0 + e < s.k_real) w = s.combined ? (wr[0] + c * wr[1] + c2 * wr[2]) * scale : wr[0] * scale;
    const __half hi = __float2half_rn(w);
    h[e] = (j < 4) ? hi : __float2half_rn(w - __half2float(hi));
  }
  *reinterpret_cast<uint4*>(out + blk * s.rows * 128 + sw128_off(row, j)) = *reinterpret_cast<const uint4*>(h);
}
int launch_pack(const PackSrc& src, long long n_blocks, void* out, cudaStream_t s) {
  const long long total = n_blocks * src.rows * 8;
  k_pack<<<(unsigned)((total + 255) / 256), 256, 0, s>>>(src, total, static_cast<unsigned char*>(out));
  P2M_LAUNCH_OK();
  return P2M_OK;
}

constexpr size_t SMEM_LIMIT = 227 * 1024;
constexpr int CONV_N = 64;
constexpr int WIDE_N = 128;
constexpr int PAIR_N = 256;
inline int conv_n(int fout) { return fout % WIDE_N == 0 ? WIDE_N : CONV_N; }
const TileBlobs& conv_tiles(int N, const DevLevel& g, const TileSet* tiles) {
  if (tiles != nullptr) return N == WIDE_N ? tiles->m64 : *tiles;
  return N == WIDE_N ? g.meta64 : g.meta128;
}
struct ConvCfg {
  int ns, xs;
};
ConvCfg conv_cfg(int NC, const TileBlobs& t, bool t1_given) {
  for (int ns = NC == WIDE_N ? 6 : 3; ns >= 3; ns -= 3)
    for (int xs = 2; xs >= 1; --xs)
      if (conv_smem(NC, ns, xs, t1_given, t.max_h1, t.stride).bytes <= SMEM_LIMIT) return {ns, xs};
  return {0, 0};
}
int conv_cols(int fin, int fout, const TileBlobs& t, bool t1_given) {
  const bool pair = fout == PAIR_N && fin == PAIR_N && t1_given && conv_cfg(PAIR_N, t, true).ns > 0;
  return pair ? PAIR_N : conv_n(fout);
}

typedef CUresult (*TmapEncodeFn)(CUtensorMap*, CUtensorMapDataType, cuuint32_t, void*, const cuuint64_t*, const cuuint64_t*,
                                 const cuuint32_t*, const cuuint32_t*, CUtensorMapInterleave, CUtensorMapSwizzle,
                                 CUtensorMapL2promotion, CUtensorMapFloatOOBfill);
TmapEncodeFn tmap_encoder() {
  static TmapEncodeFn fn = [] {
    void* f = nullptr;
    cudaDriverEntryPointQueryResult q;
    if (cudaGetDriverEntryPoint("cuTensorMapEncodeTiled", &f, cudaEnableDefault, &q) != cudaSuccess ||
        q != cudaDriverEntryPointSuccess)
      f = nullptr;
    return reinterpret_cast<TmapEncodeFn>(f);
  }();
  return fn;
}
bool make_row_tmap(CUtensorMap* tm, const float* base, long long rows, int fin, int box_rows) {
  TmapEncodeFn enc = tmap_encoder();
  if (enc == nullptr || (reinterpret_cast<uintptr_t>(base) & 15u) != 0) return false;
  const cuuint64_t dims[2] = {(cuuint64_t)fin, (cuuint64_t)rows};
  const cuuint64_t strides[1] = {(cuuint64_t)fin * 4};
  const cuuint32_t box[2] = {(cuuint32_t)FC, (cuuint32_t)box_rows};
  const cuuint32_t estr[2] = {1, 1};
  return enc(tm, CU_TENSOR_MAP_DATA_TYPE_FLOAT32, 2, const_cast<float*>(base), dims, strides, box, estr,
             CU_TENSOR_MAP_INTERLEAVE_NONE, CU_TENSOR_MAP_SWIZZLE_NONE, CU_TENSOR_MAP_L2_PROMOTION_L2_128B,
             CU_TENSOR_MAP_FLOAT_OOB_FILL_NONE) == CUDA_SUCCESS;
}

template <int NC, int NS, int XS, int MODE>
constexpr auto conv_kernel() {
  if constexpr (NC != CONV_N) return k_cheb_conv_wide<NC, NS, XS, MODE>;
  else return k_cheb_conv_umma<NC, NS, XS, MODE>;
}
template <int NC, int NS, int XS, int MODE>
int check_launch_regs() {
  constexpr int N = NC == CONV_N ? CONV_N : WIDE_N;
  static int state = 0;
  if (state == 0) {
    cudaFuncAttributes fa;
    P2M_CUDA_OK(cudaFuncGetAttributes(&fa, conv_kernel<NC, NS, XS, MODE>()));
    state = (fa.numRegs == ConvRoles<N>::regs_launch) ? 1 : -1;
  }
  if (state < 0) {
    set_error(N == WIDE_N
                  ? "k_cheb_conv_wide was compiled with a register count other than the one its setmaxnreg split assumes"
                  : "k_cheb_conv_umma was compiled with a register count other than the one its setmaxnreg split assumes");
    return P2M_ERR_CUDA;
  }
  return P2M_OK;
}

template <int NC, int NS, int XS>
int launch_cfg(const UmmaConvArgs& a, int* status, const float* zero_row, int sm_count, cudaStream_t s) {
  constexpr int N = NC == CONV_N ? CONV_N : WIDE_N;
  constexpr int TM = tile_rows<N>();
  const DevLevel& g = *a.g;
  const TileBlobs& t = conv_tiles(N, g, a.tiles);
  const size_t smem = conv_smem(NC, NS, XS, !a.plain, t.max_h1, t.stride).bytes;
  constexpr int M0 = NC == PAIR_N ? 1 : 0;
  auto kern = a.plain ? conv_kernel<NC, NS, XS, M0>() : conv_kernel<NC, NS, XS, 1>();
  P2M_CUDA_OK(cudaFuncSetAttribute(kern, cudaFuncAttributeMaxDynamicSharedMemorySize, (int)smem));
  P2M_TRY((a.plain ? check_launch_regs<NC, NS, XS, M0>() : check_launch_regs<NC, NS, XS, 1>()));
  KParams p;
  p.x = a.x;
  p.in_unpool = a.in_unpool;
  p.V = g.V;
  p.P = t.n_pattern;
  p.fin = a.fin;
  p.meta = t.meta;
  p.meta_bytes = t.bytes;
  p.meta_stride = t.stride;
  p.max_h1 = t.max_h1;
  p.own_table = a.tiles != nullptr ? 1 : 0;
  p.n_tiles = a.batch * p.P;
  p.wpack = static_cast<const unsigned char*>(a.wpack);
  p.apack = nullptr;
  p.wslice_bytes = (long long)NC * 128;
  p.wblock_stride = (long long)a.fout * 128;
  p.zero_row = zero_row;
  p.ep = to_dev(a.ep);
  p.res_identity = (a.ep.res != nullptr && a.ep.res_F == a.fout) ? 1 : 0;
  p.y = a.y;
  p.t1 = a.t1;
  p.a_scale = a.a_scale;
  p.b_scale = nullptr;
  p.ldy = a.ldy > 0 ? a.ldy : a.fout;
  p.y_col0 = a.y_col0;
  p.status = status;
  p.trace = a.trace;
  p.head_wt = a.fout == 64 ? a.head_wt : nullptr;
  p.head_z = a.fout == 64 ? a.head_z : nullptr;
  if (N == WIDE_N) {
    const bool y_ok = (reinterpret_cast<uintptr_t>(p.y) & 15u) == 0 && (p.ldy * 4) % 16 == 0 && (p.y_col0 * 4) % 16 == 0;
    const bool res_ok = !p.res_identity || ((reinterpret_cast<uintptr_t>(p.ep.res) & 15u) == 0 && (p.ep.res_F * 4) % 16 == 0);
    if (!y_ok || !res_ok) {
      set_error("umma_conv: the 128-column epilogue needs 16-byte aligned output and identity-residual rows");
      return P2M_ERR_INVALID;
    }
  }
  p.tma = 0;
  std::memset(&p.tm_x, 0, sizeof(p.tm_x));
  std::memset(&p.tm_t1, 0, sizeof(p.tm_t1));
  if (a.tiles == nullptr && g.V % TILE_M == 0) {
    const long long rows = (long long)a.batch * g.V;
    bool ok = make_row_tmap(&p.tm_x, a.x, a.in_unpool ? rows / 2 : rows, a.fin, a.in_unpool ? TM / 2 : TM);
    if (ok && a.t1 != nullptr) ok = make_row_tmap(&p.tm_t1, a.t1, rows, a.fin, TM);
    p.tma = ok ? 1 : 0;
  }
  const int n_slices = a.fout / NC;
  const dim3 grid(std::min(p.n_tiles, std::max(1, sm_count / n_slices)), n_slices);
  kern<<<grid, ConvRoles<N>::threads, smem, s>>>(p);
  P2M_LAUNCH_OK();
  return P2M_OK;
}

int launch_n(const UmmaConvArgs& a, int* status, const float* zero_row, int sm_count, cudaStream_t s) {
  const int N = conv_n(a.fout);
  const TileBlobs& t = conv_tiles(N, *a.g, a.tiles);
  const int NC = conv_cols(a.fin, a.fout, t, !a.plain);
  const ConvCfg c = conv_cfg(NC, t, !a.plain);
  if (c.ns == 0) {
    set_error("umma_conv: tile family does not fit shared memory");
    return P2M_ERR_INVALID;
  }
  if (NC == PAIR_N)
    return c.xs == 2 ? launch_cfg<PAIR_N, 3, 2>(a, status, zero_row, sm_count, s)
                     : launch_cfg<PAIR_N, 3, 1>(a, status, zero_row, sm_count, s);
  if (N == CONV_N)
    return c.xs == 2 ? launch_cfg<CONV_N, 3, 2>(a, status, zero_row, sm_count, s)
                     : launch_cfg<CONV_N, 3, 1>(a, status, zero_row, sm_count, s);
  if (c.ns == 6)
    return c.xs == 2 ? launch_cfg<WIDE_N, 6, 2>(a, status, zero_row, sm_count, s)
                     : launch_cfg<WIDE_N, 6, 1>(a, status, zero_row, sm_count, s);
  return c.xs == 2 ? launch_cfg<WIDE_N, 3, 2>(a, status, zero_row, sm_count, s)
                   : launch_cfg<WIDE_N, 3, 1>(a, status, zero_row, sm_count, s);
}

}

namespace {
void balance_store_halves(std::vector<unsigned short>* ord) {
  std::vector<unsigned short> q0, q1;
  for (unsigned short r : *ord) ((r & 4) ? q1 : q0).push_back(r);
  if (q0.size() != q1.size() || (q0.size() & 1)) return;
  size_t o = 0;
  for (size_t g = 0; g + 1 < q0.size(); g += 2) {
    (*ord)[o++] = q0[g];
    (*ord)[o++] = q0[g + 1];
    (*ord)[o++] = q1[g];
    (*ord)[o++] = q1[g + 1];
  }
}

bool make_indexed_blob(const std::vector<int>& own, int tm, const int* rowptr, const int* colidx, const float* val,
                       std::vector<int>* slot_of, std::vector<unsigned char>* blob, int* h1_out) {
  std::vector<int> halo(own);
  int n_rows = 0;
  for (int i = 0; i < tm; ++i)
    if (own[i] >= 0) {
      (*slot_of)[own[i]] = i;
      ++n_rows;
    }
  for (int i = 0; i < tm; ++i) {
    if (own[i] < 0) continue;
    for (int e = rowptr[own[i]]; e < rowptr[own[i] + 1]; ++e) {
      const int v = colidx[e];
      if ((*slot_of)[v] < 0) {
        (*slot_of)[v] = (int)halo.size();
        halo.push_back(v);
      }
    }
  }
  const int h1 = (int)halo.size();
  std::vector<unsigned short> rp(tm + 1, 0);
  std::vector<unsigned int> ent;
  for (int i = 0; i < tm; ++i) {
    if (own[i] >= 0)
      for (int e = rowptr[own[i]]; e < rowptr[own[i] + 1]; ++e) {
        unsigned int bits;
        std::memcpy(&bits, &val[e], 4);
        ent.push_back((unsigned int)(*slot_of)[colidx[e]] * 128u);
        ent.push_back(bits);
      }
    rp[i + 1] = (unsigned short)(ent.size() / 2);
  }
  for (int v : halo)
    if (v >= 0) (*slot_of)[v] = -1;
  const int nnz = (int)(ent.size() / 2);
  if (h1 > 512 || nnz > 65535) return false;
  std::vector<unsigned short> ord2(tm);
  for (int i = 0; i < tm; ++i) ord2[i] = (unsigned short)i;
  std::stable_sort(ord2.begin(), ord2.end(), [&](unsigned short a, unsigned short b2) {
    return (int)rp[a + 1] - (int)rp[a] > (int)rp[b2 + 1] - (int)rp[b2];
  });
  balance_store_halves(&ord2);
  TileHeader t{};
  t.n_rows = n_rows;
  t.h1 = h1;
  t.nnz = nnz;
  int o1 = 64;
  t.off_halo = o1; o1 += up16(h1 * 4);
  t.off_rp = o1;   o1 += up16((tm + 1) * 2);
  t.off_ent = o1;  o1 += up16(nnz * 8);
  t.off_ord2 = o1; o1 += up16(tm * 2);
  t.bytes = o1;
  blob->assign(o1, 0);
  std::memcpy(blob->data(), &t, sizeof(t));
  std::memcpy(blob->data() + t.off_halo, halo.data(), (size_t)h1 * 4);
  std::memcpy(blob->data() + t.off_rp, rp.data(), (tm + 1) * 2);
  if (nnz) std::memcpy(blob->data() + t.off_ent, ent.data(), (size_t)nnz * 8);
  std::memcpy(blob->data() + t.off_ord2, ord2.data(), tm * 2);
  *h1_out = h1;
  return true;
}

int build_blobs(const std::vector<int>& rows, int tm, const int* rowptr, const int* colidx, const float* val, int V,
                TileBlobs* ts, std::vector<void*>* owned) {
  const int P = ((int)rows.size() + tm - 1) / tm;
  std::vector<std::vector<unsigned char>> blobs(P);
  std::vector<int> slot_of(V, -1);
  int stride = 0, max_h1 = 0;
  for (int pt = 0; pt < P; ++pt) {
    std::vector<int> own(tm, -1);
    for (int i = 0; i < tm && pt * tm + i < (int)rows.size(); ++i) own[i] = rows[pt * tm + i];
    int h1 = 0;
    if (!make_indexed_blob(own, tm, rowptr, colidx, val, &slot_of, &blobs[pt], &h1)) return P2M_ERR_INVALID;
    stride = std::max(stride, (int)blobs[pt].size());
    max_h1 = std::max(max_h1, h1);
  }
  stride = (stride + 127) & ~127;
  std::vector<unsigned char> all((size_t)P * stride, 0);
  std::vector<int> bytes(P);
  for (int pt = 0; pt < P; ++pt) {
    std::memcpy(all.data() + (size_t)pt * stride, blobs[pt].data(), blobs[pt].size());
    bytes[pt] = (int)blobs[pt].size();
  }
  unsigned char* d_meta = nullptr;
  int* d_bytes = nullptr;
  P2M_CUDA_OK(cudaMalloc(&d_meta, all.size()));
  owned->push_back(d_meta);
  P2M_CUDA_OK(cudaMalloc(&d_bytes, sizeof(int) * P));
  owned->push_back(d_bytes);
  P2M_CUDA_OK(cudaMemcpy(d_meta, all.data(), all.size(), cudaMemcpyHostToDevice));
  P2M_CUDA_OK(cudaMemcpy(d_bytes, bytes.data(), sizeof(int) * P, cudaMemcpyHostToDevice));
  ts->meta = d_meta;
  ts->bytes = d_bytes;
  ts->stride = stride;
  ts->n_pattern = P;
  ts->max_h1 = max_h1;
  return P2M_OK;
}
}

int build_tileset(const std::vector<int>& rows, const int* rowptr, const int* colidx, const float* val, int V,
                  TileSet* ts, std::vector<void*>* owned) {
  P2M_TRY(build_blobs(rows, TILE_M, rowptr, colidx, val, V, ts, owned));
  return build_blobs(rows, 64, rowptr, colidx, val, V, &ts->m64, owned);
}

int build_umma_level_meta(const int* rowptr, const int* colidx, const float* val, int V, DevLevel* out,
                          std::vector<void*>* owned) {
  std::vector<int> all_rows(V);
  for (int v = 0; v < V; ++v) all_rows[v] = v;
  int st = build_blobs(all_rows, TILE_M, rowptr, colidx, val, V, &out->meta128, owned);
  if (st == P2M_OK) st = build_blobs(all_rows, 64, rowptr, colidx, val, V, &out->meta64, owned);
  if (st == P2M_ERR_INVALID) return P2M_OK;
  if (st != P2M_OK) return st;
  {
    std::vector<int> real_rows, iso_rows;
    float c = 0.f;
    bool uniform = true;
    for (int v = 0; v < V; ++v) {
      const bool iso = (rowptr[v + 1] - rowptr[v] == 1) && colidx[rowptr[v]] == v;
      if (iso) {
        if (iso_rows.empty()) c = val[rowptr[v]];
        if (val[rowptr[v]] != c) uniform = false;
        iso_rows.push_back(v);
      } else {
        real_rows.push_back(v);
      }
    }
    out->n_iso = 0;
    if (uniform && (int)iso_rows.size() >= TILE_M && (int)real_rows.size() >= TILE_M) {
      TileSet rt, it;
      if (build_tileset(real_rows, rowptr, colidx, val, V, &rt, owned) == P2M_OK &&
          build_tileset(iso_rows, rowptr, colidx, val, V, &it, owned) == P2M_OK && rt.max_h1 <= 256) {
        out->real_tiles = rt;
        out->iso_tiles = it;
        out->n_iso = (int)iso_rows.size();
        out->iso_diag = c;
      }
    }
  }
  return P2M_OK;
}


bool umma_dw_supported(const DevLevel& g, int gathered_width, int plain_width) {
  if (g.meta128.n_pattern <= 0 || g.meta128.max_h1 > 256) return false;
  if (gathered_width % FC != 0 || gathered_width < FC || gathered_width > 256) return false;
  if (plain_width != 64 && plain_width != 128 && plain_width != 256) return false;
  return dw_smem(1, g.meta128.max_h1, g.meta128.stride).bytes <= SMEM_LIMIT;
}
int umma_dw_x_stages(const DevLevel& g) { return dw_smem(2, g.meta128.max_h1, g.meta128.stride).bytes <= SMEM_LIMIT ? 2 : 1; }

int launch_umma_dw(const DevLevel& g, int batch, const float* gathered, int in_unpool, int gathered_width,
                   const float* t1, const float* plain, int g_unpool, int plain_width, int swap, const float* a_scale,
                   float* dw_ref, int* status, int sm_count, cudaStream_t s) {
  if (!umma_dw_supported(g, gathered_width, plain_width) || t1 == nullptr) {
    set_error("umma_dw: unsupported shape");
    return P2M_ERR_INVALID;
  }
  const TileBlobs& t = g.meta128;
  DwParams p;
  p.x = gathered;
  p.in_unpool = in_unpool;
  p.V = g.V;
  p.P = t.n_pattern;
  p.fin = gathered_width;
  p.n_tiles = batch * t.n_pattern;
  p.meta = t.meta;
  p.meta_bytes = t.bytes;
  p.meta_stride = t.stride;
  p.max_h1 = t.max_h1;
  p.g = plain;
  p.fout_total = plain_width;
  p.a_scale = a_scale;
  p.dw = dw_ref;
  p.status = status;
  p.t1 = t1;
  p.g_unpool = g_unpool;
  p.swap = swap;
  p.tma = 0;
  std::memset(&p.tm_x, 0, sizeof(p.tm_x));
  std::memset(&p.tm_t1, 0, sizeof(p.tm_t1));
  if (g.V % TILE_M == 0 && !in_unpool) {
    const long long rows = (long long)batch * g.V;
    p.tma = (make_row_tmap(&p.tm_x, gathered, rows, gathered_width, TILE_M) &&
             make_row_tmap(&p.tm_t1, t1, rows, gathered_width, TILE_M)) ? 1 : 0;
  }
  const int xs = umma_dw_x_stages(g);
  const size_t smem = dw_smem(xs, t.max_h1, t.stride).bytes;
  auto kern = (xs == 2) ? k_cheb_dw_umma<2> : k_cheb_dw_umma<1>;
  P2M_CUDA_OK(cudaFuncSetAttribute(kern, cudaFuncAttributeMaxDynamicSharedMemorySize, (int)smem));
  const int grid = std::min(p.n_tiles, sm_count);
  for (int m_off = 0; m_off < plain_width; m_off += 64) {
    p.m_off = m_off;
    p.m_cols = std::min(64, plain_width - m_off);
    for (int c0 = 0; c0 < gathered_width / FC; ++c0) {
      p.chunk0 = c0;
      kern<<<grid, NUM_THREADS2, smem, s>>>(p);
      P2M_LAUNCH_OK();
    }
  }
  return P2M_OK;
}

int launch_cheb_t1(const DevLevel& g, const float* x, int in_unpool, int batch, int fin, float* t1, cudaStream_t s,
                   const TileSet* tiles) {
  const TileBlobs& t = tiles ? *tiles : g.meta128;
  if (t.n_pattern <= 0 || fin % FC != 0) {
    set_error("cheb_t1: unsupported shape");
    return P2M_ERR_INVALID;
  }
  if (t.max_h1 > 256) {
    set_error("cheb_t1: halo too large");
    return P2M_ERR_INVALID;
  }
  const size_t half_sm = (228 * 1024) / 2 - 1024;
  int stages = 4;
  while (stages > 2 && t1_smem(stages, t.max_h1, t.stride).bytes > half_sm) --stages;
  const size_t smem = t1_smem(stages, t.max_h1, t.stride).bytes;
  auto kern = stages == 4 ? k_cheb_t1<4> : (stages == 3 ? k_cheb_t1<3> : k_cheb_t1<2>);
  P2M_CUDA_OK(cudaFuncSetAttribute(kern, cudaFuncAttributeMaxDynamicSharedMemorySize, (int)smem));
  T1Params p;
  p.x = x;
  p.in_unpool = in_unpool;
  p.V = g.V;
  p.P = t.n_pattern;
  p.fin = fin;
  p.meta = t.meta;
  p.meta_bytes = t.bytes;
  p.meta_stride = t.stride;
  p.max_h1 = t.max_h1;
  p.t1 = t1;
  kern<<<batch * t.n_pattern, 512, smem, s>>>(p);
  P2M_LAUNCH_OK();
  return P2M_OK;
}

bool umma_conv_supported(const DevLevel& g, int fin, int fout) {
  if (g.meta128.n_pattern <= 0) return false;
  if (fin % FC != 0 || fin < FC || fin > 256) return false;
  if (g.meta128.max_h1 > 256) return false;
  if (fout != 64 && fout != 128 && fout != 256) return false;
  const int N = conv_n(fout);
  const TileBlobs& t = conv_tiles(N, g, nullptr);
  return t.n_pattern > 0 && conv_smem(N, 3, 1, 1, t.max_h1, t.stride).bytes <= SMEM_LIMIT &&
         conv_smem(N, 3, 1, 0, t.max_h1, t.stride).bytes <= SMEM_LIMIT;
}

int umma_conv_x_stages(const DevLevel& g, int fin, int fout, bool plain) {
  return umma_conv_tiling(g, fin, fout, plain).xs;
}
UmmaConvTiling umma_conv_tiling(const DevLevel& g, int fin, int fout, bool plain) {
  const int N = conv_n(fout);
  const TileBlobs& t = conv_tiles(N, g, nullptr);
  const int NC = conv_cols(fin, fout, t, !plain);
  const ConvCfg c = conv_cfg(NC, t, !plain);
  return {NC, c.ns, c.xs};
}
bool umma_tma_rows(const DevLevel& g) { return g.V % TILE_M == 0 && tmap_encoder() != nullptr; }

size_t umma_plain_pack_bytes(int N, int K) { return (size_t)(K / FC) * N * 128; }

static size_t gemm_x_image_bytes(int M, int K) { return (size_t)((M + TILE_M - 1) / TILE_M) * (K / FC) * A_BLOCK_BYTES; }
size_t umma_gemm_apack_bytes(int M, int K) { return gemm_x_image_bytes(M, K) + 128; }
size_t umma_gemm_wpack_bytes(int N, int K) { return (size_t)(K / FC) * N * 128; }
bool umma_gemm_supported(int M, int N, int K) { return M > 0 && K >= FC && K % FC == 0 && N >= 64 && N % 64 == 0; }

namespace {
template <int N>
int launch_gemm_cfg(KParams p, int n_slices, int sm_count, cudaStream_t s) {
  constexpr int NS = 3;
  const size_t smem = conv_smem(N, NS, 1, 0, 0, 0).bytes;
  auto kern = conv_kernel<N, NS, 1, 0>();
  P2M_TRY((check_launch_regs<N, NS, 1, 0>()));
  P2M_CUDA_OK(cudaFuncSetAttribute(kern, cudaFuncAttributeMaxDynamicSharedMemorySize, (int)smem));
  p.wslice_bytes = (long long)umma_gemm_wpack_bytes(N, p.fin);
  p.wblock_stride = (long long)N * 128;
  const dim3 grid(std::min(p.n_tiles, sm_count), n_slices);
  kern<<<grid, ConvRoles<N>::threads, smem, s>>>(p);
  P2M_LAUNCH_OK();
  return P2M_OK;
}
}

int launch_umma_gemm(GemmOperand X, GemmOperand W, int M, int N, int K, const Epilogue& ep, float* Y, void* apack,
                     void* wpack, int* status, int sm_count, cudaStream_t s, int n_real, int k_real,
                     const float* x_scale, const float* w_scale) {
  if (n_real <= 0 || n_real > N) n_real = N;
  if (k_real <= 0 || k_real > K) k_real = K;
  if (!umma_gemm_supported(M, N, K) || (ep.res != nullptr && ep.res_F != N)) {
    set_error("umma_gemm: unsupported shape");
    return P2M_ERR_INVALID;
  }
  const int tiles = (M + TILE_M - 1) / TILE_M;
  const int ns = CONV_N;
  if (x_scale == nullptr) {
    float* sc = reinterpret_cast<float*>(static_cast<unsigned char*>(apack) + gemm_x_image_bytes(M, K));
    P2M_TRY(launch_absmax_scale(X.p, (M - 1) * X.ld_row + (k_real - 1) * X.ld_k + 1, sc, s));
    x_scale = sc;
  }
  P2M_TRY(launch_pack(PackSrc{X.p, X.ld_row, X.ld_k, TILE_M, K / FC, 1, M, 1.f, 0, 0.f, k_real, x_scale},
                      (long long)tiles * (K / FC), apack, s));
  P2M_TRY(launch_pack(PackSrc{W.p, W.ld_row, W.ld_k, ns, K / FC, 1, n_real, w_scale ? 1.f : W_SCALE, 0, 0.f, k_real,
                              w_scale},
                      (long long)(N / ns) * (K / FC), wpack, s));
  KParams p;
  std::memset(&p, 0, sizeof(p));
  p.V = M;
  p.P = tiles;
  p.fin = K;
  p.n_tiles = tiles;
  p.wpack = static_cast<const unsigned char*>(wpack);
  p.apack = static_cast<const unsigned char*>(apack);
  p.a_scale = x_scale;
  p.b_scale = w_scale;
  p.ep = to_dev(ep);
  p.res_identity = (ep.res != nullptr) ? 1 : 0;
  p.ldy = N;
  p.y = Y;
  p.status = status;
  return launch_gemm_cfg<CONV_N>(p, N / ns, sm_count, s);
}

size_t umma_wpack_bytes(int fin, int fout) { return (size_t)(fin / FC) * 3 * fout * 128; }

int launch_umma_pack_weights(const float* W, int fin, int fout, bool transposed, int order, float c, void* wpack,
                             cudaStream_t s) {
  const int rows = transposed ? fin : fout, K = transposed ? fout : fin;
  PackSrc src{W, transposed ? 3 : 3LL * fin, transposed ? 3LL * fin : 3, rows, K / FC, 1, rows, W_SCALE, 0, c};
  if (order == WPACK_ALL) src.orders = 3;
  else if (order == WPACK_COMBINED) src.combined = 1;
  else src.p = W + order;
  return launch_pack(src, (long long)(K / FC) * src.orders, wpack, s);
}

int launch_umma_conv(const UmmaConvArgs& a, int* status, const float* zero_row, int sm_count, cudaStream_t s) {
  if (!umma_conv_supported(*a.g, a.fin, a.fout)) {
    set_error("umma_conv: unsupported shape");
    return P2M_ERR_INVALID;
  }
  if (a.head_z != nullptr && (a.fout != 64 || a.head_wt == nullptr || a.ep.res != nullptr)) {
    set_error("umma_conv: the fused head needs fout == 64 and no residual");
    return P2M_ERR_INVALID;
  }
  if (a.t1 == nullptr && !a.plain) {
    set_error("umma_conv: the conv needs T1 = L~x (launch_cheb_t1) unless it is a plain GEMM");
    return P2M_ERR_INVALID;
  }
  if (a.tiles != nullptr && (a.tiles->max_h1 > 256 || a.tiles->n_pattern <= 0 ||
                             (a.fout % WIDE_N == 0 && a.tiles->m64.n_pattern <= 0))) {
    set_error("umma_conv: index-list tiles need at most 256 staged rows");
    return P2M_ERR_INVALID;
  }
  return launch_n(a, status, zero_row, sm_count, s);
}

}
```

### pose2mesh_release_b200/csrc/p2m_api.cu

```cuda
#include <cuda_runtime.h>

#include <algorithm>
#include <cmath>
#include <cstring>
#include <memory>
#include <string>
#include <tuple>
#include <vector>

#include "p2m_internal.h"

namespace p2m {

static thread_local std::string g_error;
static thread_local int64_t g_launches = 0;
void set_error(const std::string& msg) { g_error = msg; }
void count_launch(int n) { g_launches += n; }

int arrays_device(const char* where, std::initializer_list<const void*> arrays, int* dev) {
  int found = -1;
  for (const void* p : arrays) {
    if (!p) continue;
    cudaPointerAttributes attr;
    if (cudaPointerGetAttributes(&attr, p) != cudaSuccess ||
        (attr.type != cudaMemoryTypeDevice && attr.type != cudaMemoryTypeManaged)) {
      cudaGetLastError();
      set_error(std::string(where) + ": the data arrays must be device memory");
      return P2M_ERR_INVALID;
    }
    if (found >= 0 && attr.device != found) {
      set_error(std::string(where) + ": the data arrays are on different devices");
      return P2M_ERR_INVALID;
    }
    found = attr.device;
  }
  if (found < 0) {
    set_error(std::string(where) + ": no data array given");
    return P2M_ERR_INVALID;
  }
  *dev = found;
  return P2M_OK;
}

struct Layer {
  int level, V, fin, fout;
  int bn, relu;
  int block_end;
};

struct Block {
  int first_layer, n_layers;
  int level;
  int has_residual;
  int out_unpool;
  int in_unpool;
  int cin, cout;
  InterpTable interp;
};

struct Capture {
  std::vector<float*> z, a, y, g_a, g_z, dx;
  float* fc_out = nullptr;
  float* fc_dx = nullptr;
};

}

using namespace p2m;

struct p2m_model {
  int device = 0;
  int sm_count = 132;
  int precision = P2M_PREC_FP32_SIMT;
  std::vector<DevLevel> levels;
  std::vector<Layer> layers;
  std::vector<Block> blocks;
  int n_joint = 0, cin = 0, cout = 0;
  int fc_in = 0, fc_out = 0;
  int* kernel_status = nullptr;
  volatile int* status_host = nullptr;
  long long* trace = nullptr;
  int trace_seen = 0;
  int* out_map = nullptr;
  int out_rows = 0;
  float* zero_row = nullptr;
  int elide_padding = 1;
  int dedup_padding = 1;
  int fuse_head = 1;
  int profiling = 0;
  std::unique_ptr<Capture> capture;
  std::vector<cudaEvent_t> ev_beg, ev_end;
  std::vector<void*> owned;
};

namespace {

int check_kernel_status(p2m_model* m, const char* where) {
  if (m->status_host == nullptr) return P2M_OK;
  const int code = *m->status_host;
  if (code == 0) return P2M_OK;
  *m->status_host = 0;
  set_error(std::string(where) + ": a tensor-core kernel of an earlier call on this handle timed out on mbarrier wait #" +
            std::to_string(code) + " (results of that call are invalid)");
  return P2M_ERR_CUDA;
}

template <class T>
int upload(p2m_model* m, const std::vector<T>& h, T** out) {
  T* d = nullptr;
  size_t bytes = std::max<size_t>(h.size(), 1) * sizeof(T);
  P2M_CUDA_OK(cudaMalloc(&d, bytes));
  m->owned.push_back(d);
  if (!h.empty()) P2M_CUDA_OK(cudaMemcpy(d, h.data(), h.size() * sizeof(T), cudaMemcpyHostToDevice));
  *out = d;
  return P2M_OK;
}

int build_interp(p2m_model* m, int fin, int fout, InterpTable* t) {
  t->fin = fin;
  t->fout = fout;
  std::vector<int> i0(fout), i1(fout);
  std::vector<float> lam(fout);
  const float scale = (float)fin / (float)fout;
  for (int j = 0; j < fout; ++j) {
    float src = scale * ((float)j + 0.5f) - 0.5f;
    if (src < 0.f) src = 0.f;
    int a = (int)src;
    if (a > fin - 1) a = fin - 1;
    int b = a + ((a < fin - 1) ? 1 : 0);
    i0[j] = a;
    i1[j] = b;
    lam[j] = src - (float)a;
  }
  std::vector<int> tp(fin + 1, 0), ti;
  std::vector<float> tw;
  for (int i = 0; i < fin; ++i) {
    for (int j = 0; j < fout; ++j) {
      float w = 0.f;
      if (i0[j] == i) w += 1.f - lam[j];
      if (i1[j] == i) w += lam[j];
      if (w != 0.f) {
        ti.push_back(j);
        tw.push_back(w);
      }
    }
    tp[i + 1] = (int)ti.size();
  }
  P2M_TRY(upload(m, i0, &t->i0));
  P2M_TRY(upload(m, i1, &t->i1));
  P2M_TRY(upload(m, lam, &t->lam));
  P2M_TRY(upload(m, tp, &t->t_ptr));
  P2M_TRY(upload(m, ti, &t->t_idx));
  P2M_TRY(upload(m, tw, &t->t_w));
  return P2M_OK;
}

struct Sizes {
  size_t max_act = 0;
  size_t max_T = 0;
  size_t max_U = 0;
  size_t max_w = 0;
  size_t max_wpack = 0;
  size_t max_thin = 1;
  int max_f = 0;
};

Sizes model_sizes(const p2m_model* m, int B) {
  Sizes s;
  for (const Layer& L : m->layers) {
    size_t rows = (size_t)B * L.V;
    s.max_act = std::max(s.max_act, rows * L.fout);
    s.max_act = std::max(s.max_act, rows * L.fin);
    s.max_T = std::max(s.max_T, rows * 3 * L.fin);
    s.max_U = std::max(s.max_U, rows * L.fin);
    s.max_w = std::max(s.max_w, (size_t)L.fout * 3 * L.fin);
    if (umma_conv_supported(m->levels[L.level], L.fin, L.fout))
      s.max_wpack = std::max(s.max_wpack, umma_wpack_bytes(L.fin, L.fout));
    s.max_f = std::max(s.max_f, std::max(L.fin, L.fout));
    if (thin_conv_bwd_supported(L.fin, L.fout)) s.max_thin = std::max(s.max_thin, thin_conv_bwd_scratch_floats(rows, L.fin));
  }
  s.max_act = std::max(s.max_act, (size_t)B * m->fc_out);
  s.max_act = std::max(s.max_act, (size_t)B * m->fc_in);
  return s;
}

struct WsCommon {
  Sizes s;
  Bump b;
  float* T;
  float* wp_scratch;
  unsigned char* wpack;
  float* scale_scratch;
  double* sums;
  unsigned char* fc_apack = nullptr;
  unsigned char* fc_wpack = nullptr;
  WsCommon(const p2m_model* m, int B, void* base) : s(model_sizes(m, B)), b(base) {
    T = b.take<float>(s.max_T);
    wp_scratch = b.take<float>(s.max_w);
    wpack = b.take<unsigned char>(std::max(s.max_wpack, (size_t)16));
    scale_scratch = b.take<float>(2 * (size_t)s.max_f);
    sums = b.take<double>(2 * (size_t)s.max_f);
    if (umma_gemm_supported(B, m->fc_out, m->fc_in)) {
      fc_apack = b.take<unsigned char>(umma_gemm_apack_bytes(B, m->fc_in));
      fc_wpack = b.take<unsigned char>(umma_gemm_wpack_bytes(m->fc_out, m->fc_in));
    }
  }
  size_t bytes() const { return b.off; }
};
struct EvalWs : WsCommon {
  float* rot[3];
  EvalWs(const p2m_model* m, int B, void* base) : WsCommon(m, B, base) {
    for (int i = 0; i < 3; ++i) rot[i] = b.take<float>(s.max_act);
  }
};
struct TrainWs : WsCommon {
  std::vector<float*> z, a, mean, invstd, scale, shift, wp;
  float* fc_out;
  TrainWs(const p2m_model* m, int B, void* base) : WsCommon(m, B, base) {
    const size_t nl = m->layers.size();
    for (std::vector<float*>* v : {&z, &a, &mean, &invstd, &scale, &shift, &wp}) v->assign(nl, nullptr);
    for (size_t i = 0; i < nl; ++i) {
      const Layer& L = m->layers[i];
      size_t n = (size_t)B * L.V * L.fout;
      wp[i] = b.take<float>((size_t)L.fout * 3 * L.fin);
      if (L.bn) {
        z[i] = b.take<float>(n);
        a[i] = b.take<float>(n);
        mean[i] = b.take<float>(L.fout);
        invstd[i] = b.take<float>(L.fout);
        scale[i] = b.take<float>(L.fout);
        shift[i] = b.take<float>(L.fout);
      }
    }
    fc_out = b.take<float>((size_t)B * m->fc_out);
  }
};

struct HostIo {
  float *x, *y;
  size_t bytes;
  HostIo(const p2m_model* m, int B, void* base) {
    Bump b(base);
    x = b.take<float>((size_t)B * m->n_joint * m->cin);
    y = b.take<float>((size_t)B * m->levels[0].V * m->cout);
    bytes = b.off;
  }
};

size_t wpack_capacity(bool network, int fin, int fout) {
  return network ? umma_wpack_bytes(256, 256) : umma_wpack_bytes(((fin + 31) / 32) * 32, fout);
}

struct BwdMap {
  float* G[4];
  float* U;
  float* dwp;
  double* sums;
  unsigned char* wpack;
  unsigned char* wpack_iso;
  float* thin;
  float* a_scale;
  size_t bytes;
};
BwdMap map_scratch(const p2m_model* m, int B, void* base) {
  BwdMap w;
  Sizes s = model_sizes(m, B);
  Bump b(base);
  for (int i = 0; i < 4; ++i) w.G[i] = b.take<float>(s.max_act);
  w.U = b.take<float>(s.max_U);
  w.dwp = b.take<float>(std::max(s.max_w, (size_t)1));
  w.sums = b.take<double>(2 * (size_t)s.max_f + 2 * (size_t)m->fc_out);
  w.wpack = b.take<unsigned char>(wpack_capacity(true, 0, 0));
  w.wpack_iso = b.take<unsigned char>(umma_plain_pack_bytes(256, 256));
  w.thin = b.take<float>(s.max_thin);
  w.a_scale = b.take<float>(4);
  w.bytes = b.off;
  return w;
}

bool elided(int mode, const DevLevel& g, long long rows, int width) {
  return mode > 0 && g.n_iso > 0 && rows >= 2LL * width && (mode >= 2 || 5LL * g.n_iso >= 2LL * g.V);
}

struct ConvRoute {
  bool tc = false;
  bool elide = false;
  bool thin = false;
  bool tc_dw = false;
  bool dw_dz_basis = false;
  bool tc_dx = false;
  bool dx_elide = false;
  bool tc_dt = false;
};
ConvRoute conv_route(const p2m_model* m, int level, int fin, int fout, int batch, bool network, bool thin_ok = false,
                     bool need_dx = true) {
  const DevLevel& g = m->levels[level];
  const long long rows = (long long)batch * g.V;
  const bool tc = m->precision == P2M_PREC_FP16X3_TC;
  const size_t cap = wpack_capacity(network, fin, fout);
  ConvRoute r;
  r.tc = tc && umma_conv_supported(g, fin, fout);
  r.elide = network && r.tc && elided(m->elide_padding, g, rows, fout);
  r.thin = network && thin_ok && thin_conv_bwd_supported(fin, fout);
  r.tc_dw = tc && !r.thin && umma_dw_supported(g, fin, fout);
  const bool dx_tc = tc && !r.thin && need_dx && umma_conv_supported(g, fout, fin);
  r.tc_dx = network && dx_tc && umma_wpack_bytes(fout, fin) <= cap && fout <= 3LL * fin;
  r.dw_dz_basis = r.tc_dx && umma_dw_supported(g, fout, fin);
  r.dx_elide = r.tc_dx && elided(m->elide_padding, g, rows, fin);
  r.tc_dt = dx_tc && !r.tc_dx && umma_plain_pack_bytes(fin, fout) <= cap;
  return r;
}

UmmaConvArgs umma_args(const DevLevel& g, int batch, const float* x, int in_unpool, int fin, int fout, const Epilogue& ep,
                       float* y, const float* a_scale) {
  UmmaConvArgs a;
  a.g = &g;
  a.x = x;
  a.in_unpool = in_unpool;
  a.batch = batch;
  a.fin = fin;
  a.fout = fout;
  a.wpack = nullptr;
  a.ep = ep;
  a.y = y;
  a.a_scale = a_scale;
  return a;
}

int run_tc_conv(p2m_model* m, UmmaConvArgs a, const float* W, bool transposed, bool elide, int iso_mode, bool t1_given,
                float* T, unsigned char* wpack, unsigned char* w_iso, cudaStream_t s) {
  const DevLevel& g = *a.g;
  const int fin = transposed ? a.fout : a.fin, fout = transposed ? a.fin : a.fout;
  if (m->trace != nullptr && !transposed) {
    const char* tv = getenv("P2M_TRACE_V");
    const char* tu = getenv("P2M_TRACE_UNPOOL");
    const char* tf = getenv("P2M_TRACE_FOUT");
    a.trace = m->trace;
    if ((tv && atoi(tv) != g.V) || (tu && atoi(tu) != a.in_unpool) || (tf && atoi(tf) != a.fout)) a.trace = nullptr;
    const char* tn = getenv("P2M_TRACE_NTH");
    if (a.trace != nullptr && tn && m->trace_seen++ != atoi(tn)) a.trace = nullptr;
  }
  P2M_TRY(launch_umma_pack_weights(W, fin, fout, transposed, WPACK_ALL, 0.f, wpack, s));
  if (!t1_given) P2M_TRY(launch_cheb_t1(g, a.x, a.in_unpool, a.batch, a.fin, T, s, elide ? &g.real_tiles : nullptr));
  a.t1 = T;
  a.wpack = wpack;
  if (elide) a.tiles = &g.real_tiles;
  P2M_TRY(launch_umma_conv(a, m->kernel_status, m->zero_row, m->sm_count, s));
  if (!elide || iso_mode == 2) return P2M_OK;
  P2M_TRY(launch_umma_pack_weights(W, fin, fout, transposed, WPACK_COMBINED, g.iso_diag, w_iso, s));
  a.t1 = nullptr;
  a.plain = 1;
  a.trace = nullptr;
  a.tiles = (iso_mode == 1 && g.n_rep > 0) ? &g.rep_tiles : &g.iso_tiles;
  a.wpack = w_iso;
  return launch_umma_conv(a, m->kernel_status, m->zero_row, m->sm_count, s);
}

int run_tc_dt(p2m_model* m, const DevLevel& g, int batch, const float* dz, int fin, int fout, const float* W,
              const Epilogue& ep, const float* a_scale, unsigned char* wpack, float* T, cudaStream_t s) {
  for (int k = 0; k < 3; ++k) {
    P2M_TRY(launch_umma_pack_weights(W, fin, fout, true, k, 0.f, wpack, s));
    UmmaConvArgs a = umma_args(g, batch, dz, 0, fout, fin, ep, T, a_scale);
    a.wpack = wpack;
    a.plain = 1;
    a.ldy = 3LL * fin;
    a.y_col0 = k * fin;
    P2M_TRY(launch_umma_conv(a, m->kernel_status, m->zero_row, m->sm_count, s));
  }
  return P2M_OK;
}

int conv_linear(p2m_model* m, const ConvRoute& r, const Layer& L, int B, const float* x, int in_unpool,
                const float* w_ref, float* T, float* wp, unsigned char* wpack, const Epilogue& ep, float* y,
                cudaStream_t s, bool keep_wp, int iso_mode = 0, const float* head_wt = nullptr,
                float* head_z = nullptr) {
  const int rows = B * L.V;
  const DevLevel& g = m->levels[L.level];
  if (keep_wp || !r.tc) P2M_TRY(launch_permute_w(w_ref, wp, L.fout, L.fin, s));
  if (r.tc) {
    UmmaConvArgs a = umma_args(g, B, x, in_unpool, L.fin, L.fout, ep, y, nullptr);
    a.head_wt = head_wt;
    a.head_z = head_z;
    return run_tc_conv(m, a, w_ref, false, r.elide, iso_mode, false, T, wpack,
                       reinterpret_cast<unsigned char*>(T + (size_t)rows * L.fin), s);
  }
  if (head_z != nullptr) {
    set_error("conv_linear: fused head requested off the tensor-core path");
    return P2M_ERR_INVALID;
  }
  if (thin_conv_supported(L.fin, L.fout) && ep.res == nullptr &&
      thin_conv_scratch_floats(rows, L.fin) <= (size_t)rows * 3 * L.fin) {
    return launch_thin_conv(g, x, in_unpool, rows, L.fin, L.fout, w_ref, ep, T, y, s);
  }
  P2M_TRY(launch_cheb_basis(g, x, in_unpool, rows, L.fin, T, s));
  P2M_TRY(launch_gemm(T, 3 * L.fin, wp, 3 * L.fin, 0, y, L.fout, rows, L.fout, 3 * L.fin, ep, s));
  return P2M_OK;
}

int bn_train_tail(const float* z, int rows, int F, const float* gamma, const float* beta, float* rm, float* rv,
                  int64_t* nbt, const p2m_bn_opts_t& o, double* sums, float* mean, float* invstd, float* scale,
                  float* shift, int relu, const float* res, int res_F, int res_unpool, const InterpTable* it, float* a,
                  cudaStream_t s) {
  P2M_TRY(launch_bn_stats(z, rows, F, gamma, beta, rm, rv, nbt, o, sums, mean, invstd, scale, shift, s));
  return launch_affine_act(z, rows, F, scale, shift, relu, res, res_F, res_unpool, it, a, s);
}

int simt_dw(const DevLevel& g, const float* x, int in_unpool, int rows, int fin, int fout, const float* dz, float* T,
            float* dwp, float* dw, cudaStream_t s) {
  P2M_TRY(launch_cheb_basis(g, x, in_unpool, rows, fin, T, s));
  P2M_TRY(launch_fill_zero(dwp, sizeof(float) * fout * 3 * fin, s));
  P2M_TRY(launch_gemm_tn_atomic(dz, fout, T, 3 * fin, dwp, 3 * fin, rows, fout, 3 * fin, s));
  return launch_unpermute_w(dwp, dw, fout, fin, s);
}

int tc_dw(p2m_model* m, const DevLevel& g, int batch, const float* x, int in_unpool, int fin, const float* dz, int fout,
          bool basis_of_dz, const float* a_scale, float* T, float* dw, cudaStream_t s) {
  P2M_TRY(basis_of_dz ? launch_cheb_t1(g, dz, 0, batch, fout, T, s, nullptr)
                      : launch_cheb_t1(g, x, in_unpool, batch, fin, T, s, nullptr));
  P2M_TRY(launch_fill_zero(dw, sizeof(float) * fout * 3 * fin, s));
  return basis_of_dz ? launch_umma_dw(g, batch, dz, 0, fout, T, x, in_unpool, fin, 1, a_scale, dw, m->kernel_status,
                                      m->sm_count, s)
                     : launch_umma_dw(g, batch, x, in_unpool, fin, T, dz, 0, fout, 0, a_scale, dw, m->kernel_status,
                                      m->sm_count, s);
}

int run_fc(const p2m_model* m, const p2m_params_t* P, const WsCommon& w, int B, const float* x, float* out, cudaStream_t s) {
  Epilogue ep;
  ep.bias = P->fc_b;
  if (m->precision == P2M_PREC_FP16X3_TC && w.fc_apack != nullptr)
    return launch_umma_gemm({x, m->fc_in, 1}, {P->fc_w, m->fc_in, 1}, B, m->fc_out, m->fc_in, ep, out, w.fc_apack,
                            w.fc_wpack, m->kernel_status, m->sm_count, s);
  return launch_gemm(x, m->fc_in, P->fc_w, m->fc_in, 0, out, m->fc_out, B, m->fc_out, m->fc_in, ep, s);
}

bool fuses_head(const p2m_model* m, const Block& blk, int li, int B, const ConvRoute& r) {
  const Layer& L = m->layers[li];
  if (!m->fuse_head || !r.tc || li + 2 != (int)m->layers.size() || li + 1 >= blk.first_layer + blk.n_layers ||
      blk.has_residual || L.fout != 64 || B * L.V < 64)
    return false;
  const Layer& H = m->layers[li + 1];
  return thin_conv_supported(H.fin, H.fout) && H.fin == L.fout && H.V == L.V;
}

ConvRoute backward_route(const p2m_model* m, int li, int B, bool need_dx) {
  const Layer& L = m->layers[li];
  int b = 0;
  while (m->blocks[b].first_layer + m->blocks[b].n_layers <= li) ++b;
  const Block& blk = m->blocks[b];
  const bool first = (li == blk.first_layer);
  const bool in_unpool = first && blk.in_unpool;
  const bool res_here = first && blk.has_residual;
  return conv_route(m, L.level, L.fin, L.fout, B, true, !in_unpool && !res_here && li > 0, need_dx);
}

int capture_copy(float* dst, const float* src, size_t n, cudaStream_t s) {
  if (dst == nullptr) return P2M_OK;
  P2M_CUDA_OK(cudaMemcpyAsync(dst, src, n * sizeof(float), cudaMemcpyDeviceToDevice, s));
  return P2M_OK;
}
int capture_copy(const std::vector<float*>& v, int li, const float* src, size_t n, cudaStream_t s) {
  return capture_copy(v.empty() ? nullptr : v[li], src, n, s);
}

inline bool policy_elided(const DevLevel& g) { return elided(1, g, g.V, 0); }

int build_padding_classes(p2m_model* m, const p2m_model_desc_t* d) {
  const int n_mesh = d->n_levels - 1;
  std::vector<std::vector<char>> iso(n_mesh);
  for (int k = 0; k < n_mesh; ++k) {
    const int V = d->level_size[k];
    const int32_t* rp = d->rowptr[k];
    iso[k].assign(V, 0);
    for (int v = 0; v < V; ++v) iso[k][v] = (rp[v + 1] - rp[v] == 1 && d->colidx[k][rp[v]] == v) ? 1 : 0;
  }
  std::vector<std::vector<int>> rep_of(n_mesh);
  for (int k = n_mesh - 1; k >= 0; --k) {
    DevLevel& g = m->levels[k];
    if (!policy_elided(g)) continue;
    const int V = g.V;
    const bool has_parent = (k + 1 < n_mesh) && (d->level_size[k + 1] * 2 == V);
    const bool parent_elided = has_parent && policy_elided(m->levels[k + 1]);
    std::vector<int>& ro = rep_of[k];
    ro.assign(V, -1);
    std::vector<int> reps, cdst, csrc;
    bool ok = true;
    for (int r = 0; r < V && ok; ++r) {
      if (!iso[k][r]) continue;
      const int p = r >> 1;
      if (!has_parent || !iso[k + 1][p]) {
        ro[r] = r;
      } else {
        if (!iso[k][r ^ 1]) ok = false;
        const bool parent_computed = !parent_elided || rep_of[k + 1][p] == p;
        if (parent_computed) ro[r] = r & ~1;
        else ro[r] = 2 * rep_of[k + 1][p];
// ... 169 lines not shown
      p2m_model_destroy(m);
      return st;
    }
    m->status_host = static_cast<volatile int*>(hp);
    *m->status_host = 0;
  }
  const int nb = d->n_blocks;
  int off = 0, li = 0;
  for (int b = 0; b < nb; ++b) {
    const int32_t* ch = d->block_chans + off;
    const int len = d->block_len[b];
    if (len < 2) {
      set_error("model_create: block with < 2 channel entries");
      p2m_model_destroy(m);
      return P2M_ERR_INVALID;
    }
    Block blk{};
    blk.first_layer = li;
    blk.n_layers = len - 1;
    blk.level = (b == nb - 1) ? 0 : d->n_levels - 1 - b;
    blk.has_residual = (b >= 1 && b <= nb - 2);
    blk.out_unpool = (b >= 1 && b < nb - 2);
    blk.in_unpool = (b >= 2 && b <= nb - 2);
    blk.cin = ch[0];
    blk.cout = ch[len - 1];
    for (int j = 0; j < len - 1; ++j) {
      const bool last = (b == nb - 1) && (j == len - 2);
      m->layers.push_back(Layer{blk.level, m->levels[blk.level].V, ch[j], ch[j + 1], !last, !last, j == len - 2});
      ++li;
    }
    if (blk.has_residual) {
      int st = build_interp(m, blk.cin, blk.cout, &blk.interp);
      if (st) {
        p2m_model_destroy(m);
        return st;
      }
    }
    m->blocks.push_back(blk);
    off += len;
  }
  for (int b = 1; b < nb; ++b) {
    const Block& p = m->blocks[b - 1];
    const Block& c = m->blocks[b];
    bool ok = (c.cin == p.cout);
    if (b >= 2) {
      int vp = m->levels[p.level].V, vc = m->levels[c.level].V;
      ok = ok && (p.out_unpool ? (vc == 2 * vp) : (vc == vp));
    }
    if (!ok) {
      set_error("model_create: inconsistent hierarchy / channel plan at block " + std::to_string(b));
      p2m_model_destroy(m);
      return P2M_ERR_INVALID;
    }
  }
  if (nb == 0) {
    *out = m;
    return P2M_OK;
  }
  m->n_joint = m->levels.back().V;
  m->cin = m->blocks[0].cin;
  m->cout = m->blocks[nb - 1].cout;
  m->fc_in = m->n_joint * m->blocks[0].cout;
  m->fc_out = m->levels[m->blocks[1].level].V * m->blocks[1].cin;
  *out = m;
  return P2M_OK;
}

void p2m_model_destroy(p2m_model_t* m) {
  if (!m) return;
  DeviceGuard guard(m->device);
  for (void* p : m->owned) cudaFree(p);
  if (m->status_host) cudaFreeHost(const_cast<int*>(m->status_host));
  for (cudaEvent_t e : m->ev_beg) cudaEventDestroy(e);
  for (cudaEvent_t e : m->ev_end) cudaEventDestroy(e);
  delete m;
}

int p2m_model_num_layers(const p2m_model_t* m) { return m ? (int)m->layers.size() : 0; }

int p2m_model_layer_info(const p2m_model_t* m, int layer, int32_t out[6]) {
  if (!m || layer < 0 || layer >= (int)m->layers.size()) {
    set_error("layer_info: bad layer");
    return P2M_ERR_INVALID;
  }
  const Layer& L = m->layers[layer];
  out[0] = L.level; out[1] = L.V; out[2] = L.fin; out[3] = L.fout; out[4] = L.bn; out[5] = L.relu;
  return P2M_OK;
}

int p2m_debug_kernel_status(p2m_model_t* m, int32_t* out) {
  if (!m || !out) {
    set_error("debug_kernel_status: bad argument");
    return P2M_ERR_INVALID;
  }
  DeviceGuard guard(m->device);
  P2M_CUDA_OK(cudaDeviceSynchronize());
  *out = m->status_host ? *m->status_host : 0;
  return P2M_OK;
}

int p2m_debug_set_trace(p2m_model_t* m, void* dev_buf) {
  if (!m) return P2M_ERR_INVALID;
#ifdef P2M_UMMA_TRACE
  m->trace = static_cast<long long*>(dev_buf);
  m->trace_seen = 0;
  return P2M_OK;
#else
  if (dev_buf == nullptr) return P2M_OK;
  set_error("debug_set_trace: this library was built without P2M_UMMA_TRACE");
  return P2M_ERR_INVALID;
#endif
}

int p2m_debug_set_elide_padding(p2m_model_t* m, int enable) {
  if (!m) return P2M_ERR_INVALID;
  m->elide_padding = enable < 0 ? 0 : (enable > 2 ? 2 : enable);
  return P2M_OK;
}
int p2m_debug_set_dedup_padding(p2m_model_t* m, int enable) {
  if (!m) return P2M_ERR_INVALID;
  m->dedup_padding = enable ? 1 : 0;
  return P2M_OK;
}
int p2m_debug_conv_path(const p2m_model_t* m, int level, int fin, int fout, int32_t out[9]) {
  if (!m || !out || level < 0 || level >= (int)m->levels.size() || fin <= 0 || fout <= 0) {
    set_error("debug_conv_path: bad argument");
    return P2M_ERR_INVALID;
  }
  const DevLevel& g = m->levels[level];
  const ConvRoute r = conv_route(m, level, fin, fout, 1, false);
  out[0] = r.tc;
  out[1] = r.tc ? umma_conv_x_stages(g, fin, fout, false) : 0;
  out[2] = r.tc_dw;
  out[3] = r.tc_dw ? umma_dw_x_stages(g) : 0;
  out[4] = r.tc_dt;
  out[5] = r.tc_dt ? umma_conv_x_stages(g, fout, fin, true) : 0;
  out[6] = (g.meta128.n_pattern > 0 && umma_tma_rows(g)) ? 1 : 0;
  out[7] = g.meta128.max_h1;
  out[8] = g.n_iso;
  return P2M_OK;
}

int p2m_debug_conv_tiling(const p2m_model_t* m, int level, int fin, int fout, int32_t out[3]) {
  if (!m || !out || level < 0 || level >= (int)m->levels.size() || fin <= 0 || fout <= 0) {
    set_error("debug_conv_tiling: bad argument");
    return P2M_ERR_INVALID;
  }
  const DevLevel& g = m->levels[level];
  const UmmaConvTiling t = conv_route(m, level, fin, fout, 1, false).tc ? umma_conv_tiling(g, fin, fout, false)
                                                                        : UmmaConvTiling{0, 0, 0};
  out[0] = t.cols;
  out[1] = t.ns;
  out[2] = t.xs;
  return P2M_OK;
}

int p2m_debug_layer_route(const p2m_model_t* m, int layer, int batch, int need_dx, int32_t out[9]) {
  if (!m || !out || layer < 0 || layer >= (int)m->layers.size() || batch <= 0) {
    set_error("debug_layer_route: bad argument");
    return P2M_ERR_INVALID;
  }
  const Layer& L = m->layers[layer];
  int b = 0;
  while (m->blocks[b].first_layer + m->blocks[b].n_layers <= layer) ++b;
  const ConvRoute f = conv_route(m, L.level, L.fin, L.fout, batch, true);
  const ConvRoute r = backward_route(m, layer, batch, layer > 0 || need_dx);
  out[0] = f.tc;
  out[1] = f.elide;
  out[2] = r.thin;
  out[3] = r.tc_dw;
  out[4] = r.dw_dz_basis;
  out[5] = r.tc_dx;
  out[6] = r.dx_elide;
  out[7] = r.tc_dt;
  out[8] = fuses_head(m, m->blocks[b], layer, batch, f);
  return P2M_OK;
}

int p2m_debug_set_capture(p2m_model_t* m, const p2m_capture_t* c) {
  if (!m) {
    set_error("debug_set_capture: bad argument");
    return P2M_ERR_INVALID;
  }
  if (!c) {
    m->capture.reset();
    return P2M_OK;
  }
  const size_t nl = m->layers.size();
  auto take = [nl](float* const* p) { return p ? std::vector<float*>(p, p + nl) : std::vector<float*>(); };
  std::unique_ptr<Capture> cap(new Capture());
  cap->z = take(c->z);
  cap->a = take(c->a);
  cap->y = take(c->y);
  cap->g_a = take(c->g_a);
  cap->g_z = take(c->g_z);
  cap->dx = take(c->dx);
  cap->fc_out = c->fc_out;
  cap->fc_dx = c->fc_dx;
  m->capture = std::move(cap);
  return P2M_OK;
}

int p2m_debug_set_fuse_head(p2m_model_t* m, int enable) {
  if (!m) return P2M_ERR_INVALID;
  m->fuse_head = enable ? 1 : 0;
  return P2M_OK;
}

int p2m_model_set_profiling(p2m_model_t* m, int enable) {
  if (!m) {
    set_error("set_profiling: bad argument");
    return P2M_ERR_INVALID;
  }
  DeviceGuard guard(m->device);
  if (enable && m->ev_beg.empty()) {
    m->ev_beg.resize(m->layers.size());
    m->ev_end.resize(m->layers.size());
    for (size_t i = 0; i < m->layers.size(); ++i) {
      P2M_CUDA_OK(cudaEventCreate(&m->ev_beg[i]));
      P2M_CUDA_OK(cudaEventCreate(&m->ev_end[i]));
    }
  }
  m->profiling = enable ? 1 : 0;
  return P2M_OK;
}

int p2m_model_layer_times_ms(p2m_model_t* m, float* out, int n) {
  if (!m || !out || n < (int)m->layers.size() || m->ev_beg.empty()) {
    set_error("layer_times_ms: profiling was not enabled or buffer too small");
    return P2M_ERR_INVALID;
  }
  DeviceGuard guard(m->device);
  for (size_t i = 0; i < m->layers.size(); ++i) {
    P2M_CUDA_OK(cudaEventSynchronize(m->ev_end[i]));
    P2M_CUDA_OK(cudaEventElapsedTime(&out[i], m->ev_beg[i], m->ev_end[i]));
  }
  return P2M_OK;
}

int p2m_model_set_precision(p2m_model_t* m, int precision) {
  if (!m || (precision != P2M_PREC_FP32_SIMT && precision != P2M_PREC_FP16X3_TC)) {
    set_error("set_precision: bad argument");
    return P2M_ERR_INVALID;
  }
  m->precision = precision;
  return P2M_OK;
}

size_t p2m_meshnet_workspace_bytes_opts(const p2m_model_t* m, int batch, int training, const p2m_bn_opts_t* bn) {
  if (!m || batch <= 0 || m->layers.empty()) return 0;
  return eval_schedule(m, training, resolve_bn_opts(m, training, bn)) ? EvalWs(m, batch, nullptr).bytes()
                                                                      : TrainWs(m, batch, nullptr).bytes();
}
size_t p2m_meshnet_workspace_bytes(const p2m_model_t* m, int batch, int training) {
  return p2m_meshnet_workspace_bytes_opts(m, batch, training, nullptr);
}
size_t p2m_meshnet_backward_scratch_bytes(const p2m_model_t* m, int batch) {
  if (!m || batch <= 0 || m->layers.empty()) return 0;
  return map_scratch(m, batch, nullptr).bytes;
}
size_t p2m_meshnet_host_io_bytes(const p2m_model_t* m, int batch) {
  if (!m || batch <= 0 || m->layers.empty()) return 0;
  return HostIo(m, batch, nullptr).bytes;
}

static int forward_eval(p2m_model_t* m, const p2m_params_t* P, const std::vector<p2m_bn_opts_t>& bn, const float* x,
                        float* y, int B, void* workspace, cudaStream_t s, int gathered) {
  const EvalWs w(m, B, workspace);
  const int nl = (int)m->layers.size();
  const int iso_mode = (!m->dedup_padding || m->elide_padding < 1) ? 0 : (gathered ? 2 : 1);
  const float* cur = x;
  int cur_unpool = 0;
  int cur_buf = -1;
  auto free_rot = [](int a, int b) { return a != 0 && b != 0 ? 0 : (a != 1 && b != 1 ? 1 : 2); };
  float* head_z = nullptr;
  for (int b = 0; b < (int)m->blocks.size(); ++b) {
    const Block& blk = m->blocks[b];
    const float* block_in = cur;
    const int block_in_unpool = cur_unpool;
    const int block_in_buf = cur_buf;
    for (int j = 0; j < blk.n_layers; ++j) {
      const int li = blk.first_layer + j;
      const Layer& L = m->layers[li];
      const int rows = B * L.V;
      const bool last = (li == nl - 1);
      const bool with_res = L.block_end && blk.has_residual;
      const ConvRoute r = conv_route(m, L.level, L.fin, L.fout, B, true);
      Epilogue ep;
      float* scale = w.scale_scratch;
      float* shift = w.scale_scratch + L.fout;
      if (L.bn) {
        P2M_TRY(launch_bn_fold_eval(P->bn_w[li], P->bn_b[li], P->bn_rm[li], P->bn_rv[li], P->cl_b[li], bn[li].eps,
                                    scale, shift, L.fout, s));
        ep.scale = scale;
        ep.shift = shift;
      } else {
        ep.bias = P->cl_b[li];
      }
      ep.relu = L.relu;
      if (with_res) {
        ep.res = block_in;
        ep.res_F = blk.cin;
        ep.res_unpool = block_in_unpool;
        ep.res_i0 = blk.interp.i0;
        ep.res_i1 = blk.interp.i1;
        ep.res_lam = blk.interp.lam;
// ... 523 lines not shown
```

### pose2mesh_release_b200/csrc/p2m_internal.h

```cpp
#pragma once
#include <cuda_runtime.h>
#include <stdint.h>

#include <initializer_list>
#include <string>
#include <vector>

#include "../../include/p2m_b200.h"

namespace p2m {

void set_error(const std::string& msg);
void count_launch(int n = 1);

#define P2M_CUDA_OK(expr)                                                                     \
  do {                                                                                        \
    cudaError_t _e = (expr);                                                                  \
    if (_e != cudaSuccess) {                                                                  \
      p2m::set_error(std::string(#expr) + " failed: " + cudaGetErrorString(_e) + " (" +        \
                     __FILE__ + ":" + std::to_string(__LINE__) + ")");                        \
      return P2M_ERR_CUDA;                                                                    \
    }                                                                                         \
  } while (0)

// ... 188 lines not shown
                      ((double)y - (double)c.ccy) * c.sc + (double)in_h * 0.5);
}
__device__ __forceinline__ float2 crop_point(const PoseCrop& c, float x, float y, int in_h, int in_w, int truncate) {
  double2 t = crop_point_d(c, x, y, in_h, in_w);
  if (truncate) {
    t.x = trunc(t.x);
    t.y = trunc(t.y);
  }
  return make_float2((float)t.x, (float)t.y);
}
__device__ __forceinline__ int flip_partner(int joint_set, int j) {
  if (joint_set == P2M_JOINTS_COCO) return (j >= 1 && j <= 16) ? ((j & 1) ? j + 1 : j - 1) : j;
  if (joint_set == P2M_JOINTS_MANO || j <= 0 || j >= 24) return j;
  if (joint_set == P2M_JOINTS_SMPL) {
    if (j >= 18) return (j & 1) ? j - 1 : j + 1;
    return j % 3 == 1 ? j + 1 : (j % 3 == 2 ? j - 1 : j);
  }
  if ((j >= 1 && j <= 3) || (j >= 11 && j <= 13)) return j + 3;
  if ((j >= 4 && j <= 6) || (j >= 14 && j <= 16)) return j - 3;
  return j;
}
__device__ __forceinline__ void normalize_crop(float cx, float cy, bool on, int n_joint, int in_h, int in_w,
                                               float* __restrict__ out) {
  const int lane = threadIdx.x & 31;
  float u = cx / (float)in_w, v = cy / (float)in_h;
  float su = on ? u : 0.f, sv = on ? v : 0.f;
  for (int o = 16; o > 0; o >>= 1) {
    su += __shfl_xor_sync(0xffffffffu, su, o);
    sv += __shfl_xor_sync(0xffffffffu, sv, o);
  }
  const float mu = su / n_joint, mv = sv / n_joint;
  float qu = on ? (u - mu) * (u - mu) : 0.f, qv = on ? (v - mv) * (v - mv) : 0.f;
  for (int o = 16; o > 0; o >>= 1) {
    qu += __shfl_xor_sync(0xffffffffu, qu, o);
    qv += __shfl_xor_sync(0xffffffffu, qv, o);
  }
  if (on) {
    out[lane * 2 + 0] = (u - mu) / sqrtf(qu / n_joint);
    out[lane * 2 + 1] = (v - mv) / sqrtf(qv / n_joint);
  }
}

struct EpiDev {
  const float* bias;
  const float* scale;
  const float* shift;
  int relu;
  const float* res;
  int res_F;
  int res_unpool;
  const int* i0;
  const int* i1;
  const float* lam;
  const int* out_map;
  int out_rows;
  int level_V;
};
inline EpiDev to_dev(const Epilogue& e) {
  return EpiDev{e.bias, e.scale, e.shift, e.relu, e.res, e.res_F, e.res_unpool, e.res_i0, e.res_i1, e.res_lam,
                e.out_map, e.out_rows, e.level_V};
}
__device__ __forceinline__ float apply_epilogue(float v, long long r, int n, const EpiDev& ep) {
  if (ep.bias) v += ep.bias[n];
  if (ep.scale) v = fmaf(v, ep.scale[n], ep.shift[n]);
  if (ep.relu) v = fmaxf(v, 0.f);
  if (ep.res) {
    long long pr = ep.res_unpool ? (r >> 1) : r;
    const float* rr = ep.res + pr * ep.res_F;
    if (ep.lam == nullptr) {
      v += rr[n];
    } else {
      float l = ep.lam[n];
      v += (1.f - l) * rr[ep.i0[n]] + l * rr[ep.i1[n]];
    }
  }
  return v;
}
#endif

int launch_gemm(const float* A, int lda, const float* B, int ldb, int b_is_kn, float* C, int ldc, int M, int N, int K,
                const Epilogue& ep, cudaStream_t s);
int launch_gemm_tn_atomic(const float* A, int lda, const float* B, int ldb, float* C, int ldc, int M, int N1, int N2,
                          cudaStream_t s);

bool thin_conv_supported(int fin, int fout);
size_t thin_conv_scratch_floats(long long rows, int fin);
int launch_thin_conv(const DevLevel& g, const float* x, int in_unpool, int rows, int fin, int fout, const float* W,
                     const Epilogue& e, float* scratch, float* y, cudaStream_t s);
bool thin_conv_bwd_supported(int fin, int fout);
size_t thin_conv_bwd_scratch_floats(long long rows, int fin);
int launch_thin_conv_bwd(const DevLevel& g, const float* x, int rows, int fin, int fout, const float* W, const float* dz,
                         float* scratch, float* dx, float* dw, int sm_count, cudaStream_t s);
int launch_thin_prep(const float* W, int fin, int fout, float* wt, cudaStream_t s);
int launch_thin_tail(const DevLevel& g, int rows, int fout, const float* Z, float* U, const Epilogue& e, float* y,
                     cudaStream_t s);

int launch_permute_w(const float* W, float* Wp, int fout, int fin, cudaStream_t s);
int launch_unpermute_w(const float* Wp, float* W, int fout, int fin, cudaStream_t s);
int launch_fill_zero(void* p, size_t bytes, cudaStream_t s);
int launch_copy_rows(float* y, int batch, int V, int F, const int* dst, const int* src, int n, cudaStream_t s);

inline p2m_bn_opts_t bn_opts_default(int stats) {
  p2m_bn_opts_t o;
  o.stats = stats;
  o.cumulative = 0;
  o.momentum = 0.1;
  o.eps = 1e-5;
  return o;
}
int check_bn_opts(const p2m_bn_opts_t& o, const void* rm, const void* rv, const void* nbt, const char* where);
int launch_bn_fold_eval(const float* gamma, const float* beta, const float* rm, const float* rv, const float* bias,
                        double eps, float* scale, float* shift, int F, cudaStream_t s, float* save_mean = nullptr,
                        float* save_invstd = nullptr);
int launch_col_stats(const float* z, int rows, int F, double* sums , cudaStream_t s);
int launch_bn_finalize(const double* sums, const float* z, int rows, int F, const float* gamma, const float* beta,
                       float* rm, float* rv, int64_t* nbt, const p2m_bn_opts_t& o, float* save_mean,
                       float* save_invstd, float* scale, float* shift, cudaStream_t s);
int launch_bn_stats(const float* z, int rows, int F, const float* gamma, const float* beta, float* rm, float* rv,
                    int64_t* nbt, const p2m_bn_opts_t& o, double* sums , float* mean, float* invstd,
                    float* scale, float* shift, cudaStream_t s);
int launch_affine_act(const float* z, int rows, int F, const float* scale, const float* shift, int relu,
                      const float* res, int res_F, int res_unpool, const InterpTable* it, float* a, cudaStream_t s);
int launch_bn_relu_bwd(const float* z, const float* g_a, int rows, int F, const float* gamma, const float* scale,
                       const float* shift, const float* mean, const float* invstd, int relu,
                       double* sums , float* dgamma, float* dbeta,
                       float* g_z, cudaStream_t s,
                       float* gz_scale_out = nullptr ,
                       int frozen = 0 ,
                       float* dbias = nullptr );
int launch_col_sum(const float* g, int rows, int F, double* scratch , float* out, cudaStream_t s);

int launch_cheb_basis_bwd(const DevLevel& g, const float* dT, int rows, int F, float* U ,
                          const float* g_res, int res_Fout, const InterpTable* it, int out_pairsum, float* dx,
                          cudaStream_t s);

struct UmmaConvArgs {
  const DevLevel* g;
  const float* x;
  int in_unpool;
  int batch;
  int fin, fout;
  const void* wpack;
  Epilogue ep;
  float* y;
  const float* t1 = nullptr;
  int plain = 0;
  const float* a_scale = nullptr;
  long long ldy = 0;
  int y_col0 = 0;
  const float* head_wt = nullptr;
  float* head_z = nullptr;
  const TileSet* tiles = nullptr;
  long long* trace = nullptr;
};
int build_umma_level_meta(const int* rowptr, const int* colidx, const float* val, int V, DevLevel* out,
                          std::vector<void*>* owned);
int build_tileset(const std::vector<int>& rows, const int* rowptr, const int* colidx, const float* val, int V,
                  TileSet* ts, std::vector<void*>* owned);
bool umma_conv_supported(const DevLevel& g, int fin, int fout);
int umma_conv_x_stages(const DevLevel& g, int fin, int fout, bool plain);
struct UmmaConvTiling {
  int cols, ns, xs;
};
UmmaConvTiling umma_conv_tiling(const DevLevel& g, int fin, int fout, bool plain);
int umma_dw_x_stages(const DevLevel& g);
bool umma_tma_rows(const DevLevel& g);
constexpr int WPACK_ALL = -1, WPACK_COMBINED = -2;
size_t umma_wpack_bytes(int fin, int fout);
size_t umma_plain_pack_bytes(int N, int K);
int launch_umma_pack_weights(const float* W, int fin, int fout, bool transposed, int order, float c, void* wpack,
                             cudaStream_t s);
int launch_absmax_scale(const float* x, long long n, float* scale_out, cudaStream_t s, int headroom_log2 = 0);
int launch_absmax_finish(unsigned int* amax, float* scale_out, cudaStream_t s, int headroom_log2 = 0);
int launch_scale_by(const float* x, long long n, const float* scale, int invert, float mul, float* y, cudaStream_t s);
int launch_rescaled_epilogue(const Epilogue& ep, const float* w_scale, float w_packed, int n, float* out_scale,
                             float* out_shift, cudaStream_t s);
bool umma_dw_supported(const DevLevel& g, int gathered_width, int plain_width);
int launch_umma_dw(const DevLevel& g, int batch, const float* gathered, int in_unpool, int gathered_width,
                   const float* t1, const float* plain, int g_unpool, int plain_width, int swap, const float* a_scale,
                   float* dw_ref, int* status, int sm_count, cudaStream_t s);
int launch_cheb_t1(const DevLevel& g, const float* x, int in_unpool, int batch, int fin, float* t1, cudaStream_t s,
                   const TileSet* tiles = nullptr);
int launch_umma_conv(const UmmaConvArgs& a, int* status_flag, const float* zero_row, int sm_count, cudaStream_t s);
struct GemmOperand {
  const float* p;
  long long ld_row, ld_k;
};
bool umma_gemm_supported(int M, int N, int K);
size_t umma_gemm_apack_bytes(int M, int K);
size_t umma_gemm_wpack_bytes(int N, int K);
int launch_umma_gemm(GemmOperand X, GemmOperand W, int M, int N, int K, const Epilogue& ep, float* Y, void* apack,
                     void* wpack, int* status, int sm_count, cudaStream_t s, int n_real = 0 ,
                     int k_real = 0 ,
                     const float* x_scale = nullptr ,
                     const float* w_scale = nullptr );
int launch_dx_finish(const float* dxl, int rows, int F, const float* g_res, int res_Fout, const InterpTable* it,
                     int out_pairsum, float* out, cudaStream_t s);

}
```

### pose2mesh_release_b200/meshnet.py

```python
from __future__ import annotations

import ctypes as C
import threading
from typing import List, Optional, Sequence

import numpy as np
import torch
import torch.nn as nn

from . import _lib

CHEB_K = 3


def channel_plan(num_joint_input_chan: int, num_mesh_output_chan: int, mano: bool):
    if mano:
        return [(num_joint_input_chan, 32, 64, 64), (64, 128, 256), (256, 256, 256), (256, 256, 256),
                (256, 256, 256), (256, 128, 128), (128, 64, num_mesh_output_chan)]
    return [(num_joint_input_chan, 32, 64, 64), (64, 128, 256), (256, 256, 256), (256, 256, 256),
            (256, 256, 256), (256, 256, 256), (256, 128, 128), (128, 128, 128), (128, 128, 128),
            (128, 64, num_mesh_output_chan)]


def _is_mano(graph_L) -> bool:
    try:
        from core.config import cfg

        return cfg.DATASET.target_joint_set == "mano"
    except Exception:
        return len(graph_L) == 7


class BakedHierarchy:

    def __init__(self, laplacians: Sequence, plan):
        self.level_size = np.array([m.shape[0] for m in laplacians], dtype=np.int32)
        self.rowptr, self.colidx, self.values = [], [], []
        for i, m in enumerate(laplacians):
            c = m.tocsr().astype(np.float32)
            c.sort_indices()
            if (c != c.T).nnz:
                raise ValueError(f"Laplacian {i} is not symmetric: MeshNet's kernels need L~ == L~^T")
            self.rowptr.append(np.ascontiguousarray(c.indptr, dtype=np.int32))
            self.colidx.append(np.ascontiguousarray(c.indices, dtype=np.int32))
            self.values.append(np.ascontiguousarray(c.data, dtype=np.float32))
        self.block_len = np.array([len(p) for p in plan], dtype=np.int32)
        self.block_chans = np.array([c for p in plan for c in p], dtype=np.int32)
        self._handles = {}
        self._lock = threading.Lock()
        self.precision = _lib.default_precision()

    def handle(self, device_index: int) -> int:
        with self._lock:
            h = self._handles.get(device_index)
            if h is None:
                lib = _lib.load()
                n = len(self.level_size)
                desc = _lib.ModelDesc()
                desc.n_levels = n
                desc.level_size = self.level_size.ctypes.data_as(_lib.c_int32_p)
                rp = (_lib.c_int32_p * n)(*[a.ctypes.data_as(_lib.c_int32_p) for a in self.rowptr])
                ci = (_lib.c_int32_p * n)(*[a.ctypes.data_as(_lib.c_int32_p) for a in self.colidx])
                va = (_lib.c_float_p * n)(*[a.ctypes.data_as(_lib.c_float_p) for a in self.values])
                desc.rowptr, desc.colidx, desc.values = rp, ci, va
                desc.n_blocks = len(self.block_len)
                desc.block_len = self.block_len.ctypes.data_as(_lib.c_int32_p)
                desc.block_chans = self.block_chans.ctypes.data_as(_lib.c_int32_p)
                desc.device = device_index
                out = C.c_void_p()
                _lib.check(lib.p2m_model_create(C.byref(desc), C.byref(out)), "p2m_model_create")
                _lib.check(lib.p2m_model_set_precision(out, self.precision), "p2m_model_set_precision")
                h = out.value
                self._handles[device_index] = h
            return h

    def set_precision(self, precision: int):
        with self._lock:
            self.precision = precision
            for h in self._handles.values():
                _lib.check(_lib.load().p2m_model_set_precision(h, precision), "p2m_model_set_precision")

    def set_profiling(self, device_index: int, enable: bool):
        _lib.check(_lib.load().p2m_model_set_profiling(self.handle(device_index), int(enable)), "set_profiling")

    def set_debug(self, device_index: int, fuse_head: Optional[bool] = None, elide_padding: Optional[int] = None,
                  dedup_padding: Optional[bool] = None):
        lib, h = _lib.load(), self.handle(device_index)
        if fuse_head is not None:
            _lib.check(lib.p2m_debug_set_fuse_head(h, int(fuse_head)), "set_fuse_head")
        if elide_padding is not None:
            _lib.check(lib.p2m_debug_set_elide_padding(h, int(elide_padding)), "set_elide_padding")
        if dedup_padding is not None:
            _lib.check(lib.p2m_debug_set_dedup_padding(h, int(dedup_padding)), "set_dedup_padding")

    def set_capture(self, device_index: int, capture: Optional[dict] = None):
        lib, h = _lib.load(), self.handle(device_index)
        if capture is None:
            _lib.check(lib.p2m_debug_set_capture(h, None), "set_capture")
            return
        c = _lib.Capture()
        keep = []
        for name in ("z", "a", "y", "g_a", "g_z", "dx"):
            if capture.get(name) is not None:
                arr = _ptr_array(capture[name])
                keep.append(arr)
                setattr(c, name, arr)
        for name in ("fc_out", "fc_dx"):
            if capture.get(name) is not None:
                setattr(c, name, capture[name].data_ptr())
        _lib.check(lib.p2m_debug_set_capture(h, C.byref(c)), "set_capture")

    def layer_route(self, device_index: int, layer: int, batch: int, need_dx: bool = True) -> dict:
        out = (C.c_int32 * 9)()
        _lib.check(_lib.load().p2m_debug_layer_route(self.handle(device_index), layer, batch, int(need_dx), out),
                   "layer_route")
        return dict(zip(("tc", "elide", "thin", "tc_dw", "dw_dz_basis", "tc_dx", "dx_elide", "tc_dt", "fuse_head"),
                        (bool(v) for v in out)))

    def layer_info(self, device_index: int):
        lib = _lib.load()
        h = self.handle(device_index)
        out = []
        for i in range(lib.p2m_model_num_layers(h)):
            buf = (C.c_int32 * 6)()
            _lib.check(lib.p2m_model_layer_info(h, i, buf), "layer_info")
            out.append(dict(level=buf[0], V=buf[1], fin=buf[2], fout=buf[3], bn=buf[4], relu=buf[5]))
        return out

    def layer_times_ms(self, device_index: int):
        lib = _lib.load()
        h = self.handle(device_index)
        n = lib.p2m_model_num_layers(h)
        buf = (C.c_float * n)()
        _lib.check(lib.p2m_model_layer_times_ms(h, buf, n), "layer_times_ms")
        return list(buf)

    def kernel_status(self, device_index: int) -> int:
        out = C.c_int32(0)
        _lib.check(_lib.load().p2m_debug_kernel_status(self.handle(device_index), C.byref(out)), "kernel_status")
        return out.value

    def __deepcopy__(self, memo):
        return self

    def __del__(self):
        try:
            lib = _lib.load()
            for h in self._handles.values():
                lib.p2m_model_destroy(h)
        except Exception:
            pass


def _ptr_array(tensors):
    arr = (C.c_void_p * len(tensors))()
    for i, t in enumerate(tensors):
        arr[i] = None if t is None else t.data_ptr()
    return arr


def _param_table(fc_w, fc_b, cl_w, cl_b, bn_w, bn_b, bn_rm=None, bn_rv=None, bn_nbt=None):
    n = len(cl_w)
    none = [None] * n
    keep = [_ptr_array(cl_w), _ptr_array(cl_b), _ptr_array(bn_w), _ptr_array(bn_b),
            _ptr_array(bn_rm or none), _ptr_array(bn_rv or none), _ptr_array(bn_nbt or none)]
    p = _lib.Params()
    p.fc_w, p.fc_b = fc_w.data_ptr(), fc_b.data_ptr()
    p.cl_w, p.cl_b, p.bn_w, p.bn_b, p.bn_rm, p.bn_rv, p.bn_nbt = keep
    p._keep = keep
    return p


class _MeshNetFunction(torch.autograd.Function):

    @staticmethod
    def forward(ctx, x, hier: BakedHierarchy, training: bool, buffers, n_layers, *params):
        lib = _lib.load()
        dev = x.device
        h = hier.handle(dev.index)
        fc_w, fc_b = params[0], params[1]
        cl_w = list(params[2:2 + n_layers])
        cl_b = list(params[2 + n_layers:2 + 2 * n_layers])
        n_bn = n_layers - 1
        bn_w = list(params[2 + 2 * n_layers:2 + 2 * n_layers + n_bn]) + [None]
        bn_b = list(params[2 + 2 * n_layers + n_bn:2 + 2 * n_layers + 2 * n_bn]) + [None]
        bn_rm, bn_rv, bn_nbt, *rest = buffers
        opts = rest[0] if rest else None
        B = x.shape[0]
        v0 = int(hier.level_size[0])
        cout = int(hier.block_chans[-1])
        y = torch.empty((B, v0, cout), device=dev, dtype=torch.float32)
        ws_bytes = lib.p2m_meshnet_workspace_bytes_opts(h, B, int(training), opts)
        ws = torch.empty(ws_bytes, device=dev, dtype=torch.uint8)
        table = _param_table(fc_w, fc_b, cl_w, cl_b, bn_w, bn_b, bn_rm, bn_rv, bn_nbt)
        _lib.call("p2m_meshnet_forward_opts", dev, h, C.byref(table), opts, x, y, B, int(training), ws, ws_bytes)
        needs_grad = training and any(ctx.needs_input_grad)
        if needs_grad:
            ctx.hier, ctx.n_layers, ctx.ws, ctx.ws_bytes, ctx.bn_opts = hier, n_layers, ws, ws_bytes, opts
            ctx.save_for_backward(x, *params)
        ctx.differentiable = needs_grad
        ctx.training = training
        return y

    @staticmethod
    def backward(ctx, dy):
        if not ctx.differentiable:
            raise RuntimeError("pose2mesh_release_b200: backward through an eval-mode MeshNet forward is not "
                               "supported (BatchNorm was folded into the conv epilogues and no activations were "
                               "kept); call .train() first")
        if ctx.ws is None:
            raise RuntimeError("pose2mesh_release_b200: the saved activations of this forward were already released "
                               "by an earlier backward (retain_graph is not supported: run the forward again)")
        lib = _lib.load()
        x, *params = ctx.saved_tensors
        n_layers, hier = ctx.n_layers, ctx.hier
        dev = x.device
        h = hier.handle(dev.index)
        n_bn = n_layers - 1
        fc_w, fc_b = params[0], params[1]
        cl_w = list(params[2:2 + n_layers])
        cl_b = list(params[2 + n_layers:2 + 2 * n_layers])
        bn_w = list(params[2 + 2 * n_layers:2 + 2 * n_layers + n_bn]) + [None]
        bn_b = list(params[2 + 2 * n_layers + n_bn:2 + 2 * n_layers + 2 * n_bn]) + [None]
        sizes = [p.numel() for p in params]
        flat = torch.empty(sum(sizes), device=dev, dtype=torch.float32)
        grads, off = [], 0
        for p_, n in zip(params, sizes):
            grads.append(flat[off:off + n].view_as(p_))
            off += n
        g_fc_w, g_fc_b = grads[0], grads[1]
        g_cl_w = grads[2:2 + n_layers]
        g_cl_b = grads[2 + n_layers:2 + 2 * n_layers]
        g_bn_w = grads[2 + 2 * n_layers:2 + 2 * n_layers + n_bn] + [None]
        g_bn_b = grads[2 + 2 * n_layers + n_bn:2 + 2 * n_layers + 2 * n_bn] + [None]
        ptab = _param_table(fc_w, fc_b, cl_w, cl_b, bn_w, bn_b)
        gtab = _param_table(g_fc_w, g_fc_b, g_cl_w, g_cl_b, g_bn_w, g_bn_b)
        B = x.shape[0]
        dy = dy.contiguous().float()
        dx = torch.empty_like(x) if ctx.needs_input_grad[0] else None
        sc_bytes = lib.p2m_meshnet_backward_scratch_bytes(h, B)
# ... 177 lines not shown
```

Baseline: 13130.

## Add 128-row tile variant for 128-wide Chebyshev conv using both MMA warpgroups

Adds a 128x128 tile configuration for the wide (N=128) Chebyshev conv kernel. Both MMA warpgroups now work on the same tile, each taking a 64-row half, and the epilogue is staged in two passes per warp with per-warp residual barriers. A heuristic (conv_rows) picks between 64-row and 128-row tiles, with a debug override. The aim is to halve B-operand (weight) smem traffic per output row and improve reuse, in exchange for more producer work per thread and a more complex epilogue and barrier scheme.

```diff
diff --git a/include/p2m_b200.h b/include/p2m_b200.h
--- a/include/p2m_b200.h
+++ b/include/p2m_b200.h
@@ -62,6 +62,8 @@
 int p2m_debug_set_dedup_padding(p2m_model_t* m, int enable);
 int p2m_debug_conv_path(const p2m_model_t* m, int level, int fin, int fout, int32_t out[9]);
 int p2m_debug_conv_tiling(const p2m_model_t* m, int level, int fin, int fout, int32_t out[3]);
+int p2m_debug_set_conv_rows(p2m_model_t* m, int rows);
+int p2m_debug_conv_rows(const p2m_model_t* m, int level, int fin, int fout, int res_identity, int32_t* out);
 int p2m_debug_layer_route(const p2m_model_t* m, int layer, int batch, int need_dx, int32_t out[9]);
 
 typedef struct {
diff --git a/pose2mesh_release_b200/_lib.py b/pose2mesh_release_b200/_lib.py
--- a/pose2mesh_release_b200/_lib.py
+++ b/pose2mesh_release_b200/_lib.py
@@ -190,7 +190,7 @@
 
 EXPORTS = [
     "p2m_model_create", "p2m_model_destroy", "p2m_model_num_layers", "p2m_model_layer_info",
-    "p2m_model_set_precision", "p2m_debug_kernel_status", "p2m_debug_set_trace", "p2m_debug_set_fuse_head", "p2m_debug_set_elide_padding", "p2m_debug_set_dedup_padding", "p2m_debug_conv_path", "p2m_debug_conv_tiling", "p2m_debug_layer_route", "p2m_debug_set_capture", "p2m_model_set_profiling", "p2m_model_layer_times_ms", "p2m_meshnet_workspace_bytes", "p2m_meshnet_backward_scratch_bytes",
+    "p2m_model_set_precision", "p2m_debug_kernel_status", "p2m_debug_set_trace", "p2m_debug_set_fuse_head", "p2m_debug_set_elide_padding", "p2m_debug_set_dedup_padding", "p2m_debug_conv_path", "p2m_debug_conv_tiling", "p2m_debug_set_conv_rows", "p2m_debug_conv_rows", "p2m_debug_layer_route", "p2m_debug_set_capture", "p2m_model_set_profiling", "p2m_model_layer_times_ms", "p2m_meshnet_workspace_bytes", "p2m_meshnet_backward_scratch_bytes",
     "p2m_meshnet_forward", "p2m_meshnet_backward", "p2m_meshnet_workspace_bytes_opts", "p2m_meshnet_forward_opts",
     "p2m_meshnet_backward_opts", "p2m_model_set_output_gather", "p2m_meshnet_forward_vertices", "p2m_meshnet_host_io_bytes", "p2m_meshnet_forward_host", "p2m_meshnet_forward_vertices_host",
     "p2m_cheb_conv_workspace_bytes", "p2m_cheb_conv_fwd", "p2m_cheb_conv_bwd", "p2m_graph_match_level", "p2m_posenet_workspace_bytes", "p2m_posenet_forward",
@@ -255,6 +255,10 @@
         lib.p2m_debug_conv_path.restype = C.c_int
         lib.p2m_debug_conv_tiling.argtypes = [vp, C.c_int, C.c_int, C.c_int, c_int32_p]
         lib.p2m_debug_conv_tiling.restype = C.c_int
+        lib.p2m_debug_set_conv_rows.argtypes = [vp, C.c_int]
+        lib.p2m_debug_set_conv_rows.restype = C.c_int
+        lib.p2m_debug_conv_rows.argtypes = [vp, C.c_int, C.c_int, C.c_int, C.c_int, c_int32_p]
+        lib.p2m_debug_conv_rows.restype = C.c_int
         lib.p2m_debug_layer_route.argtypes = [vp, C.c_int, C.c_int, C.c_int, c_int32_p]
         lib.p2m_debug_layer_route.restype = C.c_int
         lib.p2m_debug_set_capture.argtypes = [vp, C.POINTER(Capture)]
diff --git a/pose2mesh_release_b200/csrc/cheb_umma.cu b/pose2mesh_release_b200/csrc/cheb_umma.cu
--- a/pose2mesh_release_b200/csrc/cheb_umma.cu
+++ b/pose2mesh_release_b200/csrc/cheb_umma.cu
@@ -352,21 +352,19 @@
                        regs_epi = REGS_EPI_W;
 };
 
-template <int N>
-__host__ __device__ constexpr int tile_rows() { return N == 128 ? 64 : TILE_M; }
 
 
 struct ConvSmem {
   size_t xs, xs_stage, t1s, t1_stage, meta, bars, flags, ep, stage, own, tail, bytes;
 };
-__host__ __device__ __forceinline__ ConvSmem conv_smem(int NC, int NS, int XS, int MODE, int max_h1, int meta_stride) {
+__host__ __device__ __forceinline__ ConvSmem conv_smem(int NC, int tm, int NS, int XS, int MODE, int max_h1,
+                                                       int meta_stride) {
   const int N = NC == 64 ? 64 : 128;
-  const int tm = N == 128 ? 64 : TILE_M;
   size_t at = 0, sum = 0;
   auto take = [&](size_t bytes) { sum += bytes; at += bytes; return at - bytes; };
   ConvSmem L;
   take((size_t)NS * (tm + NC) * 128);
-  L.xs_stage = (MODE == 1 && tm == 64) ? 0 : (size_t)tm * FC;
+  L.xs_stage = (MODE == 1 && N == 128) ? 0 : (size_t)tm * FC;
   L.xs = take(XS * L.xs_stage * 4);
   L.t1_stage = MODE == 1 ? (size_t)max_h1 * FC : 0;
   L.t1s = take(XS * L.t1_stage * 4);
@@ -377,26 +375,29 @@
   at = (at + 127) & ~(size_t)127;
   L.stage = take(4 * stg_warp_bytes(N));
   L.own = take(4 * 32 * 4);
-  L.tail = take(N == 64 ? 64 * 12 * 4 : 4 * 8);
+  L.tail = take(N == 64 ? 64 * 12 * 4 : (tm == TILE_M ? 8 : 4) * 8);
   L.bytes = sum + 128 + 1024 + 32;
   return L;
 }
 
-template <int N, int NC, int NS, int XS, int MODE>
+template <int N, int NC, int TM, int NS, int XS, int MODE>
 __device__ __forceinline__ void cheb_conv_body(const KParams& p) {
   static_assert(N == 64 || N == 128, "one warpgroup holds the CTA's 128 x 64 or 64 x 128 accumulator in registers");
-  static_assert(NC == N || (N == 128 && NC == 2 * N && MODE == 1),
+  static_assert(NC == N || (N == 128 && NC == 2 * N && TM == 64 && MODE == 1),
                 "64 x 256: both MMA warpgroups of the 64 x 128 layout, T1-given convs only (conv_cols)");
+  static_assert(TM == (N == 64 ? TILE_M : 64) || (N == 128 && NC == N && TM == TILE_M && MODE == 1),
+                "128 x 128: both MMA warpgroups of the 64 x 128 layout, T1-given convs only (conv_rows)");
   static_assert(NS == 3 || NS == 6, "the producers fill a chunk's three slots back to back");
   using R = ConvRoles<N>;
-  constexpr int TM = tile_rows<N>();
   constexpr int NPW = R::prod;
   constexpr int NRG = NPW * 4;
   constexpr int RPT = TM / NRG;
   constexpr int NWG = N == 128 ? 2 : 1;
   constexpr bool COLS = NC != N;
-  static_assert(RPT == 2, "both configurations give a producer thread two tile rows");
-  constexpr int H = TM / 64;
+  constexpr bool ROWS = N == 128 && TM == TILE_M;
+  constexpr bool BOTH = COLS || ROWS;
+  static_assert(RPT == (ROWS ? 4 : 2), "a producer thread builds two tile rows (128 x 128: four)");
+  constexpr int H = N == 64 ? 2 : 1;
   constexpr int ER = 16 * H;
   constexpr bool KT1 = (MODE == 1);
   constexpr bool plain = !KT1;
@@ -406,7 +407,7 @@
   static_assert(NWG * ER == 32 && SLOT_BYTES == (TM + NC) * 128, "conv_smem describes this configuration");
 
   extern __shared__ __align__(1024) unsigned char smem_raw[];
-  const ConvSmem L = conv_smem(NC, NS, XS, MODE, p.max_h1, p.meta_stride);
+  const ConvSmem L = conv_smem(NC, TM, NS, XS, MODE, p.max_h1, p.meta_stride);
   unsigned char* ring = smem_raw;
   float* Xs = reinterpret_cast<float*>(smem_raw + L.xs);
   float* T1s = reinterpret_cast<float*>(smem_raw + L.t1s);
@@ -440,7 +441,7 @@
   if (tid == 0) {
     for (int s = 0; s < NS; ++s) {
       mbar_init(smem_u32(b_ab_full + s), p.apack != nullptr ? 1 : NPW + 1);
-      mbar_init(smem_u32(b_ab_empty + s), COLS ? 8 : 4);
+      mbar_init(smem_u32(b_ab_empty + s), BOTH ? 8 : 4);
     }
     for (int s = 0; s < XS; ++s) {
       mbar_init(smem_u32(b_x_full + s), N_XLOAD * 32 + 1);
@@ -451,7 +452,7 @@
       mbar_init(smem_u32(b_m_empty + s), 1);
     }
     if (N == 128) {
-      for (int w = 0; w < 4; ++w) mbar_init(smem_u32(b_res + w), 1);
+      for (int w = 0; w < (ROWS ? 8 : 4); ++w) mbar_init(smem_u32(b_res + w), 1);
       mbar_init(smem_u32(b_stg_free), 4);
       mbar_init(smem_u32(b_turn), 4);
     }
@@ -594,11 +595,11 @@
     int colk[2];
 #pragma unroll
     for (int k = 0; k < 2; ++k) colk[k] = (int)(((uint32_t)pc ^ (uint32_t)((k * RPI + prow) & 7)) << 2);
-    const int trow = (lane >> 4) * 64 + wq * 16 + (lane & 15);
+    const int trow = (ROWS ? 64 * g : (lane >> 4) * 64) + wq * 16 + (lane & 15);
     const int uses = plain ? n_chunk : n_use;
     int etn = 0;
-    for (int it = COLS ? 0 : g; (int)blockIdx.x + it * (int)gridDim.x < p.n_tiles; it += COLS ? 1 : NWG) {
-      const int e = COLS ? 2 * it + g : it;
+    for (int it = BOTH ? 0 : g; (int)blockIdx.x + it * (int)gridDim.x < p.n_tiles; it += BOTH ? 1 : NWG) {
+      const int e = BOTH ? 2 * it + g : it;
       const int tile = blockIdx.x + it * gridDim.x;
       const int b = tile / p.P, pat = tile - b * p.P;
       const long long mesh0 = (long long)b * p.V;
@@ -638,7 +639,7 @@
 #pragma unroll
         for (int j = 0; j < 32; ++j) acc[h][j] = 0.f;
       if (wq == 0 && lane == 0) trace_ev(p, tr, etn, 1);
-      if (NWG == 2 && !COLS && it > 0) {
+      if (NWG == 2 && !BOTH && it > 0) {
         mbar_wait(smem_u32(b_turn), (uint32_t)(it - 1) & 1u, abort_flag, p.status, 13);
         if (wq == 0 && lane == 0) trace_ev(p, tr, etn, 3);
       }
@@ -651,7 +652,7 @@
         const uint32_t a0 = smem_u32(ring + s * SLOT_BYTES);
         wg_fence();
         if constexpr (N == 128) {
-          const uint64_t da = make_desc_sw128(a0);
+          const uint64_t da = make_desc_sw128(a0 + (ROWS ? (uint32_t)g * (64 * 128) : 0u));
           const uint64_t db = make_desc_sw128(a0 + A_BYTES + (COLS ? (uint32_t)g * (N * 128) : 0u));
           wgmma_m64n128(acc, da + 0, db + 0);
           wgmma_m64n128(acc, da + 2, db + 2);
@@ -677,7 +678,7 @@
         __syncwarp();
         if (lane == 0) mbar_arrive(smem_u32(b_ab_empty + s));
       }
-      if (NWG == 2 && !COLS && lane == 0) mbar_arrive(smem_u32(b_turn));
+      if (NWG == 2 && !BOTH && lane == 0) mbar_arrive(smem_u32(b_turn));
       if (wq == 0 && lane == 0) trace_ev(p, tr, etn, 2);
       auto stage_slab = [&](int cb) {
 #pragma unroll
@@ -727,78 +728,92 @@
           zr[2] = make_float4(z[8], z[9], z[10], z[11]);
         }
       } else if (N == 128) {
-        if (e > 0) mbar_wait(smem_u32(b_stg_free), (uint32_t)(e - 1) & 1u, abort_flag, p.status, 14);
+        constexpr int NPASS = ROWS ? 2 : 1;
+        constexpr int PR = ER / NPASS;
+        const uint32_t stg_e = ROWS ? smem_u32(epi_stage) + (uint32_t)(g * 4 + wq) * (PR * STG_ROW_BYTES) : stg;
+        if (!ROWS && e > 0) mbar_wait(smem_u32(b_stg_free), (uint32_t)(e - 1) & 1u, abort_flag, p.status, 14);
         if (wq == 0 && lane == 0) trace_ev(p, tr, etn, 20);
         const bool res_id = p.ep.res != nullptr && p.res_identity;
-        if (res_id) {
-          const uint32_t rbar = smem_u32(b_res + wq);
-          const int n_valid = __popc(__ballot_sync(0xFFFFFFFFu, lane < ER && own_w[lane] >= 0));
-          if (lane == 0) mbar_arrive_expect_tx(rbar, (uint32_t)n_valid * (N * 4));
-          __syncwarp();
-          if (lane < ER && own_w[lane] >= 0) {
-            const long long r = mesh0 + own_w[lane];
-            bulk_g2s(stg + lane * STG_ROW_BYTES, p.ep.res + (p.ep.res_unpool ? (r >> 1) : r) * p.ep.res_F + ecol0, N * 4,
-                     rbar);
+#pragma unroll
+        for (int ps = 0; ps < NPASS; ++ps) {
+          const int* own_p = own_w + ps * PR;
+          if (ROWS) {
+            if (lane < PR) bulk_wait_read0();
+            __syncwarp();
           }
-          mbar_wait(rbar, (uint32_t)e & 1u, abort_flag, p.status, 12);
-        }
-        if (wq == 0 && lane == 0) trace_ev(p, tr, etn, 21);
-#pragma unroll
-        for (int h = 0; h < 2; ++h)
-#pragma unroll
-          for (int jg = 0; jg < 8; ++jg) {
-            const int n = 64 * h + 8 * jg + 2 * (lane & 3);
-            const float2 mu = *reinterpret_cast<const float2*>(ep_mul_g + n);
-            const float2 ad = *reinterpret_cast<const float2*>(ep_add_g + n);
-#pragma unroll
-            for (int r = 0; r < 2; ++r) {
-              const int j = 4 * jg + 2 * r;
-              const uint32_t a = stg + ((lane >> 2) + 8 * r) * STG_ROW_BYTES + n * 4;
-              float o0 = fmaf(acc[h][j], mu.x, ad.x), o1 = fmaf(acc[h][j + 1], mu.y, ad.y);
-              if (p.ep.relu) {
-                o0 = fmaxf(o0, 0.f);
-                o1 = fmaxf(o1, 0.f);
+          if (res_id) {
+            const uint32_t rbar = smem_u32(b_res + (ROWS ? g * 4 + wq : wq));
+            const int n_valid = __popc(__ballot_sync(0xFFFFFFFFu, lane < PR && own_p[lane] >= 0));
+            if (lane == 0) mbar_arrive_expect_tx(rbar, (uint32_t)n_valid * (N * 4));
+            __syncwarp();
+            if (lane < PR && own_p[lane] >= 0) {
+              const long long r = mesh0 + own_p[lane];
+              bulk_g2s(stg_e + lane * STG_ROW_BYTES, p.ep.res + (p.ep.res_unpool ? (r >> 1) : r) * p.ep.res_F + ecol0,
+                       N * 4, rbar);
+            }
+            mbar_wait(rbar, (uint32_t)(ROWS ? ps : e) & 1u, abort_flag, p.status, ROWS ? 15 : 12);
+          }
+          if (wq == 0 && lane == 0) trace_ev(p, tr, etn, 21);
+#pragma unroll
+          for (int h = 0; h < 2; ++h)
+#pragma unroll
+            for (int jg = 0; jg < 8; ++jg) {
+              const int n = 64 * h + 8 * jg + 2 * (lane & 3);
+              const float2 mu = *reinterpret_cast<const float2*>(ep_mul_g + n);
+              const float2 ad = *reinterpret_cast<const float2*>(ep_add_g + n);
+#pragma unroll
+              for (int r = 0; r < 2; ++r) {
+                if (ROWS && r != ps) continue;
+                const int j = 4 * jg + 2 * r;
+                const uint32_t a = stg_e + ((lane >> 2) + (ROWS ? 0 : 8 * r)) * STG_ROW_BYTES + n * 4;
+                float o0 = fmaf(acc[h][j], mu.x, ad.x), o1 = fmaf(acc[h][j + 1], mu.y, ad.y);
+                if (p.ep.relu) {
+                  o0 = fmaxf(o0, 0.f);
+                  o1 = fmaxf(o1, 0.f);
+                }
+                if (res_id) {
+                  const float2 rv = lds_f2(a);
+                  o0 += rv.x;
+                  o1 += rv.y;
+                }
+                sts_f2(a, o0, o1);
               }
-              if (res_id) {
-                const float2 rv = lds_f2(a);
-                o0 += rv.x;
-                o1 += rv.y;
+            }
+          if (p.ep.res != nullptr && !p.res_identity) {
+            __syncwarp();
+            const int gn = ecol0 + 4 * lane;
+            for (int rr = 0; rr < PR; ++rr) {
+              const int vtx = own_p[rr];
+              if (vtx >= 0) {
+                const long long r = mesh0 + vtx;
+                const float* res_row = p.ep.res + (p.ep.res_unpool ? (r >> 1) : r) * p.ep.res_F;
+                const uint32_t a = stg_e + rr * STG_ROW_BYTES + lane * 16;
+                const float4 v = lds_f4(a);
+                float o[4] = {v.x, v.y, v.z, v.w};
+#pragma unroll
+                for (int e = 0; e < 4; ++e) {
+                  const float l = __ldg(p.ep.lam + gn + e);
+                  o[e] += (1.f - l) * __ldg(res_row + __ldg(p.ep.i0 + gn + e)) + l * __ldg(res_row + __ldg(p.ep.i1 + gn + e));
+                }
+                sts_f4(a, make_float4(o[0], o[1], o[2], o[3]));
               }
-              sts_f2(a, o0, o1);
             }
           }
-        if (p.ep.res != nullptr && !p.res_identity) {
+          if (wq == 0 && lane == 0) trace_ev(p, tr, etn, 22);
+          fence_async_proxy();
           __syncwarp();
-          const int gn = ecol0 + 4 * lane;
-          for (int rr = 0; rr < ER; ++rr) {
-            const int vtx = own_w[rr];
-            if (vtx >= 0) {
-              const long long r = mesh0 + vtx;
-              const float* res_row = p.ep.res + (p.ep.res_unpool ? (r >> 1) : r) * p.ep.res_F;
-              const uint32_t a = stg + rr * STG_ROW_BYTES + lane * 16;
-              const float4 v = lds_f4(a);
-              float o[4] = {v.x, v.y, v.z, v.w};
-#pragma unroll
-              for (int e = 0; e < 4; ++e) {
-                const float l = __ldg(p.ep.lam + gn + e);
-                o[e] += (1.f - l) * __ldg(res_row + __ldg(p.ep.i0 + gn + e)) + l * __ldg(res_row + __ldg(p.ep.i1 + gn + e));
-              }
-              sts_f4(a, make_float4(o[0], o[1], o[2], o[3]));
-            }
+          if (lane < PR) {
+            if (own_p[lane] >= 0)
+              bulk_s2g(p.y + (mesh0 + own_p[lane]) * p.ldy + p.y_col0 + ecol0, stg_e + lane * STG_ROW_BYTES, N * 4);
+            bulk_commit();
           }
         }
-        if (wq == 0 && lane == 0) trace_ev(p, tr, etn, 22);
-        fence_async_proxy();
-        __syncwarp();
-        if (lane < ER) {
-          if (own_w[lane] >= 0)
-            bulk_s2g(p.y + (mesh0 + own_w[lane]) * p.ldy + p.y_col0 + ecol0, stg + lane * STG_ROW_BYTES, N * 4);
-          bulk_commit();
-        }
         if (wq == 0 && lane == 0) trace_ev(p, tr, etn, 23);
-        if (lane < ER) bulk_wait_read0();
-        __syncwarp();
-        if (lane == 0) mbar_arrive(smem_u32(b_stg_free));
+        if (!ROWS) {
+          if (lane < ER) bulk_wait_read0();
+          __syncwarp();
+          if (lane == 0) mbar_arrive(smem_u32(b_stg_free));
+        }
         if (wq == 0 && lane == 0) trace_ev(p, tr, etn, 24);
       } else {
 #pragma unroll
@@ -1000,11 +1015,11 @@
 template <int N, int NS, int XS, int MODE>
 __global__ void __launch_bounds__(NUM_THREADS2, 1) k_cheb_conv_umma(const __grid_constant__ KParams p) {
   static_assert(N == 64, "the 64 x 128 configuration is k_cheb_conv_wide");
-  cheb_conv_body<N, N, NS, XS, MODE>(p);
-}
-template <int NC, int NS, int XS, int MODE>
+  cheb_conv_body<N, N, TILE_M, NS, XS, MODE>(p);
+}
+template <int NC, int TM, int NS, int XS, int MODE>
 __global__ void __launch_bounds__(NUM_THREADS_W, 1) k_cheb_conv_wide(const __grid_constant__ KParams p) {
-  cheb_conv_body<128, NC, NS, XS, MODE>(p);
+  cheb_conv_body<128, NC, TM, NS, XS, MODE>(p);
 }
 
 struct DwParams {
@@ -1488,22 +1503,28 @@
 constexpr int WIDE_N = 128;
 constexpr int PAIR_N = 256;
 inline int conv_n(int fout) { return fout % WIDE_N == 0 ? WIDE_N : CONV_N; }
-const TileBlobs& conv_tiles(int N, const DevLevel& g, const TileSet* tiles) {
-  if (tiles != nullptr) return N == WIDE_N ? tiles->m64 : *tiles;
-  return N == WIDE_N ? g.meta64 : g.meta128;
+inline int conv_tm(int N) { return N == WIDE_N ? 64 : TILE_M; }
+const TileBlobs& conv_tiles(int tm, const DevLevel& g, const TileSet* tiles) {
+  if (tiles != nullptr) return tm == 64 ? tiles->m64 : *tiles;
+  return tm == 64 ? g.meta64 : g.meta128;
 }
 struct ConvCfg {
   int ns, xs;
 };
-ConvCfg conv_cfg(int NC, const TileBlobs& t, bool t1_given) {
-  for (int ns = NC == WIDE_N ? 6 : 3; ns >= 3; ns -= 3)
+ConvCfg conv_cfg(int NC, int tm, const TileBlobs& t, bool t1_given) {
+  for (int ns = (NC == WIDE_N && tm == 64) ? 6 : 3; ns >= 3; ns -= 3)
     for (int xs = 2; xs >= 1; --xs)
-      if (conv_smem(NC, ns, xs, t1_given, t.max_h1, t.stride).bytes <= SMEM_LIMIT) return {ns, xs};
+      if (conv_smem(NC, tm, ns, xs, t1_given, t.max_h1, t.stride).bytes <= SMEM_LIMIT) return {ns, xs};
   return {0, 0};
 }
 int conv_cols(int fin, int fout, const TileBlobs& t, bool t1_given) {
-  const bool pair = fout == PAIR_N && fin == PAIR_N && t1_given && conv_cfg(PAIR_N, t, true).ns > 0;
+  const bool pair = fout == PAIR_N && fin == PAIR_N && t1_given && conv_cfg(PAIR_N, 64, t, true).ns > 0;
   return pair ? PAIR_N : conv_n(fout);
+}
+int conv_rows(int fin, int fout, const TileBlobs& t128, bool t1_given, bool res_identity, int force) {
+  const bool fits = fout == WIDE_N && t1_given && t128.n_pattern > 0 && conv_cfg(WIDE_N, TILE_M, t128, true).ns > 0;
+  if (!fits || force == 64) return 64;
+  return (force == TILE_M || (fin >= WIDE_N && !res_identity)) ? TILE_M : 64;
 }
 
 typedef CUresult (*TmapEncodeFn)(CUtensorMap*, CUtensorMapDataType, cuuint32_t, void*, const cuuint64_t*, const cuuint64_t*,
@@ -1532,18 +1553,18 @@
              CU_TENSOR_MAP_FLOAT_OOB_FILL_NONE) == CUDA_SUCCESS;
 }
 
-template <int NC, int NS, int XS, int MODE>
+template <int NC, int TM, int NS, int XS, int MODE>
 constexpr auto conv_kernel() {
-  if constexpr (NC != CONV_N) return k_cheb_conv_wide<NC, NS, XS, MODE>;
+  if constexpr (NC != CONV_N) return k_cheb_conv_wide<NC, TM, NS, XS, MODE>;
   else return k_cheb_conv_umma<NC, NS, XS, MODE>;
 }
-template <int NC, int NS, int XS, int MODE>
+template <int NC, int TM, int NS, int XS, int MODE>
 int check_launch_regs() {
   constexpr int N = NC == CONV_N ? CONV_N : WIDE_N;
   static int state = 0;
   if (state == 0) {
     cudaFuncAttributes fa;
-    P2M_CUDA_OK(cudaFuncGetAttributes(&fa, conv_kernel<NC, NS, XS, MODE>()));
+    P2M_CUDA_OK(cudaFuncGetAttributes(&fa, conv_kernel<NC, TM, NS, XS, MODE>()));
     state = (fa.numRegs == ConvRoles<N>::regs_launch) ? 1 : -1;
   }
   if (state < 0) {
@@ -1555,17 +1576,16 @@
   return P2M_OK;
 }
 
-template <int NC, int NS, int XS>
+template <int NC, int TM, int NS, int XS>
 int launch_cfg(const UmmaConvArgs& a, int* status, const float* zero_row, int sm_count, cudaStream_t s) {
   constexpr int N = NC == CONV_N ? CONV_N : WIDE_N;
-  constexpr int TM = tile_rows<N>();
   const DevLevel& g = *a.g;
-  const TileBlobs& t = conv_tiles(N, g, a.tiles);
-  const size_t smem = conv_smem(NC, NS, XS, !a.plain, t.max_h1, t.stride).bytes;
-  constexpr int M0 = NC == PAIR_N ? 1 : 0;
-  auto kern = a.plain ? conv_kernel<NC, NS, XS, M0>() : conv_kernel<NC, NS, XS, 1>();
+  const TileBlobs& t = conv_tiles(TM, g, a.tiles);
+  const size_t smem = conv_smem(NC, TM, NS, XS, !a.plain, t.max_h1, t.stride).bytes;
+  constexpr int M0 = (NC == PAIR_N || (N == WIDE_N && TM == TILE_M)) ? 1 : 0;
+  auto kern = a.plain ? conv_kernel<NC, TM, NS, XS, M0>() : conv_kernel<NC, TM, NS, XS, 1>();
   P2M_CUDA_OK(cudaFuncSetAttribute(kern, cudaFuncAttributeMaxDynamicSharedMemorySize, (int)smem));
-  P2M_TRY((a.plain ? check_launch_regs<NC, NS, XS, M0>() : check_launch_regs<NC, NS, XS, 1>()));
+  P2M_TRY((a.plain ? check_launch_regs<NC, TM, NS, XS, M0>() : check_launch_regs<NC, TM, NS, XS, 1>()));
   KParams p;
   p.x = a.x;
   p.in_unpool = a.in_unpool;
@@ -1619,26 +1639,37 @@
   return P2M_OK;
 }
 
+UmmaConvTiling conv_tiling(int fin, int fout, const DevLevel& g, const TileSet* tiles, bool plain, bool res_identity,
+                           int force_rows) {
+  const int N = conv_n(fout);
+  const int NC = conv_cols(fin, fout, conv_tiles(conv_tm(N), g, tiles), !plain);
+  const int tm =
+      NC == WIDE_N ? conv_rows(fin, fout, conv_tiles(TILE_M, g, tiles), !plain, res_identity, force_rows) : conv_tm(N);
+  const ConvCfg c = conv_cfg(NC, tm, conv_tiles(tm, g, tiles), !plain);
+  return {NC, c.ns, c.xs, tm};
+}
+
 int launch_n(const UmmaConvArgs& a, int* status, const float* zero_row, int sm_count, cudaStream_t s) {
-  const int N = conv_n(a.fout);
-  const TileBlobs& t = conv_tiles(N, *a.g, a.tiles);
-  const int NC = conv_cols(a.fin, a.fout, t, !a.plain);
-  const ConvCfg c = conv_cfg(NC, t, !a.plain);
+  const bool res_identity = a.ep.res != nullptr && a.ep.res_F == a.fout;
+  const UmmaConvTiling c = conv_tiling(a.fin, a.fout, *a.g, a.tiles, a.plain != 0, res_identity, a.conv_rows);
   if (c.ns == 0) {
     set_error("umma_conv: tile family does not fit shared memory");
     return P2M_ERR_INVALID;
   }
-  if (NC == PAIR_N)
-    return c.xs == 2 ? launch_cfg<PAIR_N, 3, 2>(a, status, zero_row, sm_count, s)
-                     : launch_cfg<PAIR_N, 3, 1>(a, status, zero_row, sm_count, s);
-  if (N == CONV_N)
-    return c.xs == 2 ? launch_cfg<CONV_N, 3, 2>(a, status, zero_row, sm_count, s)
-                     : launch_cfg<CONV_N, 3, 1>(a, status, zero_row, sm_count, s);
+  if (c.cols == PAIR_N)
+    return c.xs == 2 ? launch_cfg<PAIR_N, 64, 3, 2>(a, status, zero_row, sm_count, s)
+                     : launch_cfg<PAIR_N, 64, 3, 1>(a, status, zero_row, sm_count, s);
+  if (c.cols == CONV_N)
+    return c.xs == 2 ? launch_cfg<CONV_N, TILE_M, 3, 2>(a, status, zero_row, sm_count, s)
+                     : launch_cfg<CONV_N, TILE_M, 3, 1>(a, status, zero_row, sm_count, s);
+  if (c.rows == TILE_M)
+    return c.xs == 2 ? launch_cfg<WIDE_N, TILE_M, 3, 2>(a, status, zero_row, sm_count, s)
+                     : launch_cfg<WIDE_N, TILE_M, 3, 1>(a, status, zero_row, sm_count, s);
   if (c.ns == 6)
-    return c.xs == 2 ? launch_cfg<WIDE_N, 6, 2>(a, status, zero_row, sm_count, s)
-                     : launch_cfg<WIDE_N, 6, 1>(a, status, zero_row, sm_count, s);
-  return c.xs == 2 ? launch_cfg<WIDE_N, 3, 2>(a, status, zero_row, sm_count, s)
-                   : launch_cfg<WIDE_N, 3, 1>(a, status, zero_row, sm_count, s);
+    return c.xs == 2 ? launch_cfg<WIDE_N, 64, 6, 2>(a, status, zero_row, sm_count, s)
+                     : launch_cfg<WIDE_N, 64, 6, 1>(a, status, zero_row, sm_count, s);
+  return c.xs == 2 ? launch_cfg<WIDE_N, 64, 3, 2>(a, status, zero_row, sm_count, s)
+                   : launch_cfg<WIDE_N, 64, 3, 1>(a, status, zero_row, sm_count, s);
 }
 
 }
@@ -1900,20 +1931,16 @@
   if (g.meta128.max_h1 > 256) return false;
   if (fout != 64 && fout != 128 && fout != 256) return false;
   const int N = conv_n(fout);
-  const TileBlobs& t = conv_tiles(N, g, nullptr);
-  return t.n_pattern > 0 && conv_smem(N, 3, 1, 1, t.max_h1, t.stride).bytes <= SMEM_LIMIT &&
-         conv_smem(N, 3, 1, 0, t.max_h1, t.stride).bytes <= SMEM_LIMIT;
+  const TileBlobs& t = conv_tiles(conv_tm(N), g, nullptr);
+  return t.n_pattern > 0 && conv_smem(N, conv_tm(N), 3, 1, 1, t.max_h1, t.stride).bytes <= SMEM_LIMIT &&
+         conv_smem(N, conv_tm(N), 3, 1, 0, t.max_h1, t.stride).bytes <= SMEM_LIMIT;
 }
 
 int umma_conv_x_stages(const DevLevel& g, int fin, int fout, bool plain) {
   return umma_conv_tiling(g, fin, fout, plain).xs;
 }
-UmmaConvTiling umma_conv_tiling(const DevLevel& g, int fin, int fout, bool plain) {
-  const int N = conv_n(fout);
-  const TileBlobs& t = conv_tiles(N, g, nullptr);
-  const int NC = conv_cols(fin, fout, t, !plain);
-  const ConvCfg c = conv_cfg(NC, t, !plain);
-  return {NC, c.ns, c.xs};
+UmmaConvTiling umma_conv_tiling(const DevLevel& g, int fin, int fout, bool plain, bool res_identity, int force_rows) {
+  return conv_tiling(fin, fout, g, nullptr, plain, res_identity, force_rows);
 }
 bool umma_tma_rows(const DevLevel& g) { return g.V % TILE_M == 0 && tmap_encoder() != nullptr; }
 
@@ -1928,9 +1955,9 @@
 template <int N>
 int launch_gemm_cfg(KParams p, int n_slices, int sm_count, cudaStream_t s) {
   constexpr int NS = 3;
-  const size_t smem = conv_smem(N, NS, 1, 0, 0, 0).bytes;
-  auto kern = conv_kernel<N, NS, 1, 0>();
-  P2M_TRY((check_launch_regs<N, NS, 1, 0>()));
+  const size_t smem = conv_smem(N, TILE_M, NS, 1, 0, 0, 0).bytes;
+  auto kern = conv_kernel<N, TILE_M, NS, 1, 0>();
+  P2M_TRY((check_launch_regs<N, TILE_M, NS, 1, 0>()));
   P2M_CUDA_OK(cudaFuncSetAttribute(kern, cudaFuncAttributeMaxDynamicSharedMemorySize, (int)smem));
   p.wslice_bytes = (long long)umma_gemm_wpack_bytes(N, p.fin);
   p.wblock_stride = (long long)N * 128;
diff --git a/pose2mesh_release_b200/csrc/p2m_api.cu b/pose2mesh_release_b200/csrc/p2m_api.cu
--- a/pose2mesh_release_b200/csrc/p2m_api.cu
+++ b/pose2mesh_release_b200/csrc/p2m_api.cu
@@ -87,6 +87,7 @@
   int elide_padding = 1;
   int dedup_padding = 1;
   int fuse_head = 1;
+  int conv_rows = 0;
   int profiling = 0;
   std::unique_ptr<Capture> capture;
   std::vector<cudaEvent_t> ev_beg, ev_end;
@@ -341,6 +342,7 @@
     if (a.trace != nullptr && tn && m->trace_seen++ != atoi(tn)) a.trace = nullptr;
   }
   P2M_TRY(launch_umma_pack_weights(W, fin, fout, transposed, WPACK_ALL, 0.f, wpack, s));
+  a.conv_rows = m->conv_rows;
   if (!t1_given) P2M_TRY(launch_cheb_t1(g, a.x, a.in_unpool, a.batch, a.fin, T, s, elide ? &g.real_tiles : nullptr));
   a.t1 = T;
   a.wpack = wpack;
@@ -816,6 +818,27 @@
   out[0] = t.cols;
   out[1] = t.ns;
   out[2] = t.xs;
+  return P2M_OK;
+}
+
+int p2m_debug_set_conv_rows(p2m_model_t* m, int rows) {
+  if (!m || (rows != 0 && rows != 64 && rows != 128)) {
+    set_error("debug_set_conv_rows: rows must be 0, 64 or 128");
+    return P2M_ERR_INVALID;
+  }
+  m->conv_rows = rows;
+  return P2M_OK;
+}
+
+int p2m_debug_conv_rows(const p2m_model_t* m, int level, int fin, int fout, int res_identity, int32_t* out) {
+  if (!m || !out || level < 0 || level >= (int)m->levels.size() || fin <= 0 || fout <= 0) {
+    set_error("debug_conv_rows: bad argument");
+    return P2M_ERR_INVALID;
+  }
+  const DevLevel& g = m->levels[level];
+  *out = conv_route(m, level, fin, fout, 1, false).tc
+             ? umma_conv_tiling(g, fin, fout, false, res_identity != 0, m->conv_rows).rows
+             : 0;
   return P2M_OK;
 }
 
diff --git a/pose2mesh_release_b200/csrc/p2m_internal.h b/pose2mesh_release_b200/csrc/p2m_internal.h
--- a/pose2mesh_release_b200/csrc/p2m_internal.h
+++ b/pose2mesh_release_b200/csrc/p2m_internal.h
@@ -364,6 +364,7 @@
   float* head_z = nullptr;
   const TileSet* tiles = nullptr;
   long long* trace = nullptr;
+  int conv_rows = 0;
 };
 int build_umma_level_meta(const int* rowptr, const int* colidx, const float* val, int V, DevLevel* out,
                           std::vector<void*>* owned);
@@ -373,8 +374,10 @@
 int umma_conv_x_stages(const DevLevel& g, int fin, int fout, bool plain);
 struct UmmaConvTiling {
   int cols, ns, xs;
-};
-UmmaConvTiling umma_conv_tiling(const DevLevel& g, int fin, int fout, bool plain);
+  int rows;
+};
+UmmaConvTiling umma_conv_tiling(const DevLevel& g, int fin, int fout, bool plain, bool res_identity = false,
+                                int force_rows = 0);
 int umma_dw_x_stages(const DevLevel& g);
 bool umma_tma_rows(const DevLevel& g);
 constexpr int WPACK_ALL = -1, WPACK_COMBINED = -2;
diff --git a/pose2mesh_release_b200/meshnet.py b/pose2mesh_release_b200/meshnet.py
--- a/pose2mesh_release_b200/meshnet.py
+++ b/pose2mesh_release_b200/meshnet.py
@@ -84,8 +84,10 @@
         _lib.check(_lib.load().p2m_model_set_profiling(self.handle(device_index), int(enable)), "set_profiling")
 
     def set_debug(self, device_index: int, fuse_head: Optional[bool] = None, elide_padding: Optional[int] = None,
-                  dedup_padding: Optional[bool] = None):
+                  dedup_padding: Optional[bool] = None, conv_rows: Optional[int] = None):
         lib, h = _lib.load(), self.handle(device_index)
+        if conv_rows is not None:
+            _lib.check(lib.p2m_debug_set_conv_rows(h, int(conv_rows)), "set_conv_rows")
         if fuse_head is not None:
             _lib.check(lib.p2m_debug_set_fuse_head(h, int(fuse_head)), "set_fuse_head")
         if elide_padding is not None:
```

After: 13370 (median of 6 runs). 1.02x the previous value.
